# Kamino666/S2VT-video-caption

Measured on AMD Instinct MI355X. Metric: training frames/sec (whole node), higher is better.
Workload: dtype f32; 1 GPU; BASELINE configs[1]: S2VT train step, B=64 per GPU x 1 GPU, 80x4096 feats, hidden=embed=1000, vocab=12000, fp32, Adam; global_batch=64, frames=80, parallelism=dp1

## Files before the change

include/s2vt_hip.h:

```cpp
#ifndef S2VT_HIP_H
#define S2VT_HIP_H

#include <stddef.h>
#include <stdint.h>

#ifdef __cplusplus
extern "C" {
#endif

#define S2VT_ABI_VERSION 9

#define S2VT_ERR_ARG (-1)
#define S2VT_ERR_INDEX (-2)
#define S2VT_ERR_TIMEOUT (-3)

typedef struct s2vt_dims {
    int32_t B, L, F, H, E, V;
} s2vt_dims;

typedef struct s2vt_params {
    const float* vid_w_ih;
    const float* vid_w_hh;
    const float* vid_b_ih;
    const float* vid_b_hh;
// ... 127 lines not shown
                              float* dlogits, void* stream);

#define S2VT_CIDER_MAX_T 512
typedef struct s2vt_cider_table {
    const uint64_t* idf_keys; const double* idf_vals;
    const int32_t* clip_ref_off; const int32_t* ent_off;
    const uint64_t* ent_keys; const double* ent_w;
    const double* ref_norm; const int32_t* ref_len;
    const double* pen;
    double log_n;
    int64_t n_idf;
    int32_t n_clips, n_refs, n_pen;
} s2vt_cider_table;
int s2vt_cider_rewards(const s2vt_cider_table* table, const int32_t* clip_rows, const int64_t* ids, int32_t B, int32_t T, int64_t ld,
                       int32_t sos, int32_t eos, double* out, void* stream);
#define S2VT_CONSENSUS_MAX_K 64
size_t s2vt_cider_consensus_workspace_bytes(int32_t B, int32_t K, int32_t T);
int s2vt_cider_consensus(const s2vt_cider_table* table, const int64_t* ids, int32_t B, int32_t K, int32_t T, int64_t ld,
                         int32_t sos, int32_t eos, const uint8_t* valid, double* utility, int32_t* best,
                         void* workspace, size_t workspace_bytes, void* stream);
typedef struct s2vt_bleu_table {
    const int32_t* clip_key_off; const uint64_t* keys; const int32_t* max_count;
    const int32_t* clip_ref_off; const int32_t* ref_words;
    const double* bp;
    int64_t n_keys;
    int32_t n_clips, n_refs, n_rl;
} s2vt_bleu_table;
int s2vt_mixed_rewards(const s2vt_cider_table* table, const s2vt_bleu_table* bleu, const int32_t* clip_rows, const int64_t* ids,
                       int32_t B, int32_t T, int64_t ld, int32_t sos, int32_t eos, double w_cider, double w_bleu, double* out,
                       double* out_cider, double* out_bleu, void* stream);
size_t s2vt_mixed_consensus_workspace_bytes(int32_t B, int32_t K, int32_t T);
int s2vt_mixed_consensus(const s2vt_cider_table* table, const s2vt_bleu_table* bleu, const int64_t* ids, int32_t B, int32_t K, int32_t T,
                         int64_t ld, int32_t sos, int32_t eos, const uint8_t* valid, double w_cider, double w_bleu, double* utility,
                         int32_t* best, void* workspace, size_t workspace_bytes, void* stream);
int s2vt_sc_weights(const int64_t* sampled, const double* r_sample, const double* r_greedy, int32_t B, int32_t T, int32_t sos,
                    int32_t eos, int64_t* caps, float* weight, void* stream);
int s2vt_sc_weights_group(const int64_t* sampled, const double* r_sample, const double* r_greedy, int32_t B, int32_t K, int32_t T,
                          int32_t sos, int32_t eos, int64_t* caps, float* weight, double* baseline, void* stream);
#define S2VT_SWOR_MAX_K 8
int s2vt_sc_weights_swor(const int64_t* sampled, const float* logprob, const float* kappa, const double* r_sample,
                         const double* r_greedy, int32_t B, int32_t K, int32_t T, int32_t sos, int32_t eos, int64_t* caps,
                         float* weight, double* coef, double* baseline, void* stream);

int s2vt_mean_ce_backward_fused(const s2vt_dims* d, const float* logits, const int64_t* target, int64_t target_ld, const float* lse,
                                const float* gout, void* workspace, size_t workspace_bytes, void* stream);


int s2vt_gemm_f32(int32_t a_kmajor, int32_t b_kmajor, int32_t M, int32_t N, int32_t K, const float* A, int64_t lda,
                  const float* B, int64_t ldb, float* C, int64_t ldc, const float* bias, int32_t accumulate,
                  void* stream);

int s2vt_gemm_f32_splitk(int32_t a_kmajor, int32_t b_kmajor, int32_t M, int32_t N, int32_t K, const float* A,
                         int64_t lda, const float* B, int64_t ldb, float* C, int64_t ldc, const float* bias,
                         int32_t accumulate, float* ws, size_t ws_floats, void* stream);

int s2vt_split_planes(int32_t nplanes, int32_t transpose, const float* in, int64_t ld, int32_t rows, int32_t cols,
                      uint16_t* out, int64_t ldo, int32_t kpad, int32_t out_rows_pad, void* stream);
int s2vt_gemm_bf16_nt(int32_t nplanes, int32_t M, int32_t N, int32_t K, const uint16_t* A, int64_t lda, const uint16_t* B,
                      int64_t ldb, float* C, int64_t ldc, const float* bias, int32_t accumulate, float* ws,
                      size_t ws_floats, void* stream);
int s2vt_gemm_bf16_tt(int32_t nplanes, int32_t M, int32_t N, int32_t K, const uint16_t* A, int64_t lda, const uint16_t* B,
                      int64_t ldb, float* C, int64_t ldc, const float* bias, int32_t accumulate, float* ws, size_t ws_floats,
                      void* stream);

int s2vt_gemm_tune(int32_t nplanes, int32_t tile_rows, int32_t nsplit);

int s2vt_feat_proj_fwd(const s2vt_dims* d, const float* feats, const float* w, const float* bias, float* x1,
                       void* stream);
int s2vt_feat_proj_bwd(const s2vt_dims* d, const float* feats, const float* w, const float* dx1, float* dw,
                       float* dbias, float* dfeats, float* colsum_ws, void* stream);
size_t s2vt_colsum_ws_floats(int64_t rows, int32_t cols);


int s2vt_gemm_f32_mapped(int32_t a_kmajor, int32_t b_kmajor, int32_t M, int32_t N, int32_t K, const float* A, int64_t lda,
                         const int32_t* a_idx, int32_t a_inner, int32_t a_outer, const float* B, int64_t ldb, const int32_t* b_idx,
                         int32_t b_inner, int32_t b_outer, float* C, int64_t ldc, const int32_t* c_idx, int32_t c_inner,
                         int32_t c_outer, const float* bias, int32_t accumulate, float* ws, size_t ws_floats, int32_t splitk_cap,
                         void* stream);
size_t s2vt_embedding_grad_ws_ints(int64_t rows, int32_t V);
int s2vt_embedding_grad(const float* d_rows, int64_t rows, int32_t E, const int32_t* tok, int32_t V, float* d_emb, int32_t* ws,
                        size_t ws_ints, void* stream);
int s2vt_gather_rows(const float* src, int64_t ld, const int32_t* idx, int64_t rows, int32_t cols, float* out, void* stream);
int s2vt_group_sum_rows(const float* in, int64_t ld_in, float* out, int64_t ld_out, int64_t groups, int32_t K, int32_t cols, void* stream);
int s2vt_transpose_f32(const float* in, int32_t rows, int32_t cols, float* out, void* stream);
int s2vt_colsum(const float* x, int64_t rows, int32_t cols, int64_t ld, float* ws, size_t ws_floats, float* out, int32_t accumulate,
                void* stream);
int s2vt_colsum_finish(const float* partial, int32_t nchunks, int32_t cols, float* out, int32_t accumulate, void* stream);
int s2vt_split_planes_dual(int32_t nplanes, const float* in, int64_t ld, const int32_t* idx, int32_t inner, int32_t outer, int32_t rows,
                           int32_t cols, uint16_t* out_r, int64_t ldo_r, int32_t kpad_r, uint16_t* out_t, int64_t ldo_t, int32_t kpad_t,
                           float* colpart, const float* lse, const int64_t* target, int64_t target_ld, int32_t Lm1, const float* gout,
                           float* alpha_out, void* stream);

int s2vt_lstm_step_fwd(int32_t B, int32_t H, const float* gx, const float* bias, const float* w_hh,
                       const float* h_prev, const float* c_prev, float* h_out, float* c_out, float* stash,
                       void* stream);
int s2vt_lstm_step_fwd_token(int32_t B, int32_t H, int32_t E, int32_t V, const float* gx, const float* w_hh, const float* h_prev,
                             const float* c_prev, const float* emb, const float* w_e, int64_t ldw_e, const int32_t* tok,
                             const unsigned long long* tok_packed, int32_t tok_const, float* h_out, float* c_out, void* stream);

int s2vt_lstm_step_fwd_table(int32_t B, int32_t H, int32_t V, const float* gx, const int32_t* gx_idx, const float* bias, const float* gtab,
                             int64_t ldtab, const int32_t* tok, const unsigned long long* tok_packed, int32_t tok_const, const float* w_hh,
                             const float* h_prev, const float* c_prev, float* h_out, float* c_out, float* stash, uint16_t* h_planes,
                             int64_t ldhp, int32_t hp_rows, float* z_out, int64_t ldz, int32_t contract_only, void* stream);
int s2vt_lstm_cell_pointwise(int32_t B, int32_t H, int32_t V, const float* gx, const int32_t* gx_idx, const float* bias, const float* gtab,
                             int64_t ldtab, const int32_t* tok, const unsigned long long* tok_packed, int32_t tok_const, const float* z,
                             int64_t ldz, const float* c_prev, float* h_out, float* c_out, float* stash, uint16_t* h_planes, int64_t ldhp,
                             int32_t hp_rows, void* stream);
int s2vt_argmax_x3_planes(int32_t B, int32_t V, int32_t K, const uint16_t* W, int64_t ldw, int32_t w_rows, const uint16_t* Hp, int64_t ldh,
                          int32_t kpad_h, int32_t hp_rows, const float* bias, unsigned long long* packed, const uint16_t* W2, int64_t ldw2,
                          int32_t kpad_w2, int32_t w2_rows, int32_t M2, float* z, int64_t ldz, int32_t with_logits, int32_t sample,
                          float temperature, uint64_t seed, int32_t step, int32_t row0, void* stream);

int s2vt_lstm_step_bwd(int32_t B, int32_t H, const float* dg_next, const float* w_hh_t, const float* dh_out,
                       const float* stash, const float* c, const float* c_prev, float* dc, int32_t dc_is_zero,
                       float* dg, void* stream);

int s2vt_lstm_seq_fwd(int32_t T, int32_t B, int32_t H, const float* gx, int32_t n_gx, const float* bias,
                      const float* w_hh, float* h_all, float* c_all, float* stash, void* stream);
int s2vt_lstm_seq_bwd(int32_t T, int32_t B, int32_t H, const float* w_hh, const float* dh_out, int32_t dh_first,
                      const float* c_all, float* stash_dg, float* w_hh_t, float* dc, void* stream);

int s2vt_gru_step_fwd(int32_t B, int32_t H, const float* gx, const float* b_ih, const float* w_hh, const float* b_hh,
                      const float* h_prev, float* h_out, float* stash, void* stream);
int s2vt_gru_step_fwd_token(int32_t B, int32_t H, int32_t E, int32_t V, const float* gx, const float* w_hh, const float* b_hh,
                            const float* h_prev, const float* emb, const float* w_e, int64_t ldw_e, const int32_t* tok,
                            const unsigned long long* tok_packed, int32_t tok_const, float* h_out, void* stream);
int s2vt_gru_step_fwd_token_ss(int32_t B, int32_t H, int32_t E, int32_t V, const float* gx, const float* w_hh, const float* b_hh,
                               const float* h_prev, const float* emb, const float* w_e, int64_t ldw_e,
                               const unsigned long long* tok_packed, const int64_t* targets, int64_t targets_ld, float ss_prob,
                               uint64_t seed, int32_t step, int32_t row0, float* h_out, void* stream);
int s2vt_gru_step_bwd(int32_t B, int32_t H, const float* dgh_next, const float* w_hh_t, const float* stash_next, const float* dh_out,
                      const float* stash, const float* h_prev, float* dh, float* dgx, float* dgh, void* stream);
int s2vt_gru_seq_fwd(int32_t T, int32_t B, int32_t H, const float* gx, int32_t n_gx, const float* b_ih, const float* w_hh,
                     const float* b_hh, float* h_all, float* stash, void* stream);
int s2vt_gru_seq_bwd(int32_t T, int32_t B, int32_t H, const float* w_hh, const float* dh_out, int32_t dh_first, const float* h_all,
                     const float* stash, float* w_hh_t, float* dh, float* dgx, float* dgh, void* stream);
int s2vt_tokens_time_major(int32_t B, int32_t Lm1, int32_t V, const int64_t* targets, int64_t targets_ld, int32_t* tok, void* stream);

typedef struct s2vt_lstm_layer {
    const float* w_hh;
    const float* w_in;
    int64_t ldw_in;
    const float* x_in;
    const float* gx;
    int32_t gx_t0, n_gx;
    const float* bias;
    const float* h0; const float* c0;
    const float* mask;
    const float* emb; const float* w_e; int64_t ldw_e; int32_t E, V;
    const unsigned long long* tok_packed; int32_t tok_const;
    float* h; float* c;
    float* stash;
    float* hm;
    const float* dh_ext; int32_t dh_t0;
    float* dg;
    const int64_t* ss_targets; int64_t ss_ld; uint64_t ss_seed; float ss_prob; int32_t ss_step, ss_row0;
} s2vt_lstm_layer;
int s2vt_lstm_chain_fwd(int32_t T, int32_t B, int32_t H, int32_t n, const s2vt_lstm_layer* layers, void* stream);
size_t s2vt_lstm_chain_bwd_workspace_bytes(int32_t B, int32_t H, int32_t n);
int s2vt_lstm_chain_bwd(int32_t T, int32_t B, int32_t H, int32_t n, const s2vt_lstm_layer* layers, void* workspace,
                        size_t workspace_bytes, void* stream);

size_t s2vt_lstm_seq_bf16_workspace_bytes(int32_t T, int32_t B, int32_t H);
int s2vt_lstm_seq_fwd_bf16(int32_t T, int32_t B, int32_t H, float* gx_stash, int32_t n_gx, const float* bias,
                           const float* w_hh, float* h_all, float* c_all, void* workspace, size_t workspace_bytes,
                           int32_t persistent, int32_t block, void* stream);
// ... 174 lines not shown
```

s2vt-video-caption_amd/capi.py:

```python
import ctypes
import os
from ctypes import POINTER, c_char_p, c_double, c_float, c_int32, c_int64, c_size_t, c_uint64, c_void_p

_HERE = os.path.dirname(os.path.abspath(__file__))
LIB_PATH = os.environ.get("S2VT_LIB") or os.path.join(_HERE, "libs2vt_hip.so")


class Dims(ctypes.Structure):
    _fields_ = [(n, c_int32) for n in ("B", "L", "F", "H", "E", "V")]


PARAM_FIELDS = ("vid_w_ih", "vid_w_hh", "vid_b_ih", "vid_b_hh", "word_w_ih", "word_w_hh", "word_b_ih", "word_b_hh",
                "feat_w", "feat_b", "out_w", "out_b", "emb_w")
PARAM_KEYS = ("vid_rnn.weight_ih_l0", "vid_rnn.weight_hh_l0", "vid_rnn.bias_ih_l0", "vid_rnn.bias_hh_l0",
              "word_rnn.weight_ih_l0", "word_rnn.weight_hh_l0", "word_rnn.bias_ih_l0", "word_rnn.bias_hh_l0",
              "feat_linear.weight", "feat_linear.bias", "out_linear.weight", "out_linear.bias", "embedding.weight")


class Params(ctypes.Structure):
    _fields_ = [(n, c_void_p) for n in PARAM_FIELDS]


class Grads(ctypes.Structure):
    _fields_ = [(n, c_void_p) for n in PARAM_FIELDS]
# ... 59 lines not shown
                                      c_void_p, c_size_t, c_void_p]),
    "s2vt_backward_wait_grads": (c_int32, [c_int32, c_void_p]),
    "s2vt_backward_order": (c_int32, [POINTER(c_int32), POINTER(c_int32)]),
    "s2vt_beam_workspace_bytes": (c_size_t, [POINTER(Dims), c_int32]),
    "s2vt_beam_step": (c_int32, [POINTER(Dims), POINTER(Params), c_int32] + [c_void_p] * 14 + [c_size_t, c_void_p]),
    "s2vt_beam_step_cached": (c_int32, [POINTER(Dims), POINTER(Params), c_int32] + [c_void_p] * 14 + [c_size_t, c_void_p, c_size_t,
                                                                                                     c_void_p]),
    "s2vt_decode_workspace_bytes": (c_size_t, [POINTER(Dims)]),
    "s2vt_greedy_decode": (c_int32, [POINTER(Dims), POINTER(Params), c_void_p, c_int32, c_void_p, c_void_p, c_size_t,
                                     c_void_p]),
    "s2vt_decode_cache_bytes": (c_size_t, [POINTER(Dims)]),
    "s2vt_decode_uses_cache": (c_int32, [POINTER(Dims)]),
    "s2vt_greedy_decode_cached": (c_int32, [POINTER(Dims), POINTER(Params), c_void_p, c_int32, c_void_p, c_void_p, c_size_t,
                                            c_void_p, c_size_t, c_int32, c_void_p]),
    "s2vt_adam_step": (c_int32, [c_void_p, c_void_p, c_void_p, c_void_p, c_int64, c_double, c_double, c_double, c_double, c_int64, c_void_p]),
    "s2vt_grad_norm_workspace_bytes": (c_size_t, [c_int64]),
    "s2vt_grad_norm": (c_int32, [c_void_p, c_int64, c_double, c_int32, c_void_p, c_size_t, c_void_p, c_void_p]),
    "s2vt_adam_step_clipped": (c_int32, [c_void_p, c_void_p, c_void_p, c_void_p, c_int64, c_double, c_double, c_double, c_double, c_int64,
                                         c_double, c_int32, POINTER(c_int64), POINTER(c_int32), c_int32, c_int32, c_void_p, c_void_p]),
    "s2vt_mean_ce_forward": (c_int32, [c_int32, c_int32, c_int32, c_void_p, c_void_p, c_int64, c_void_p, c_void_p,
                                       c_void_p, c_void_p]),
    "s2vt_mean_ce_backward": (c_int32, [c_int32, c_int32, c_int32, c_void_p, c_void_p, c_int64, c_void_p, c_void_p,
                                        c_void_p, c_void_p]),
    "s2vt_mask_criterion_forward": (c_int32, [c_int32, c_int32, c_int32, c_void_p, c_void_p, c_int64, c_void_p, c_int64, c_void_p,
                                              c_void_p, c_void_p, c_void_p]),
    "s2vt_mask_criterion_backward": (c_int32, [c_int32, c_int32, c_void_p, c_int64, c_void_p, c_void_p, c_void_p, c_void_p]),
    "s2vt_gemm_f32": (c_int32, [c_int32, c_int32, c_int32, c_int32, c_int32, c_void_p, c_int64, c_void_p, c_int64,
                                c_void_p, c_int64, c_void_p, c_int32, c_void_p]),
    "s2vt_gemm_f32_splitk": (c_int32, [c_int32, c_int32, c_int32, c_int32, c_int32, c_void_p, c_int64, c_void_p, c_int64,
                                       c_void_p, c_int64, c_void_p, c_int32, c_void_p, c_size_t, c_void_p]),
    "s2vt_split_planes": (c_int32, [c_int32, c_int32, c_void_p, c_int64, c_int32, c_int32, c_void_p, c_int64, c_int32,
                                    c_int32, c_void_p]),
    "s2vt_gemm_bf16_nt": (c_int32, [c_int32, c_int32, c_int32, c_int32, c_void_p, c_int64, c_void_p, c_int64, c_void_p,
                                    c_int64, c_void_p, c_int32, c_void_p, c_size_t, c_void_p]),
    "s2vt_gemm_bf16_tt": (c_int32, [c_int32, c_int32, c_int32, c_int32, c_void_p, c_int64, c_void_p, c_int64, c_void_p,
                                    c_int64, c_void_p, c_int32, c_void_p, c_size_t, c_void_p]),
    "s2vt_gemm_tune": (c_int32, [c_int32, c_int32, c_int32]),
    "s2vt_beam_queue_bytes": (c_size_t, [c_int32, c_int32, c_int32]),
    "s2vt_beam_queue_step": (c_int32, [c_int32] * 6 + [c_void_p, c_size_t] + [c_void_p] * 6),
    "s2vt_beam_queue_result": (c_int32, [c_int32, c_int32, c_int32, c_void_p, c_size_t, c_void_p, c_int32, c_void_p, c_void_p]),
    "s2vt_beam_cum_bytes": (c_size_t, [c_int32, c_int32, c_int32]),
    "s2vt_beam_cum_step": (c_int32, [c_int32] * 5 + [c_double, c_int32, c_void_p, c_size_t] + [c_void_p] * 6),
    "s2vt_beam_cum_result": (c_int32, [c_int32] * 5 + [c_void_p, c_size_t] + [c_void_p] * 4),
    "s2vt_beam_cum_hist_bytes": (c_size_t, [c_int32, c_int32, c_int32]),
    "s2vt_beam_cum_hist_step": (c_int32, [c_int32] * 5 + [c_double, c_int32, c_void_p, c_size_t] + [c_void_p] * 5 +
                                [POINTER(c_void_p), POINTER(c_int64), c_void_p]),
    "s2vt_top20_logprob_constrained": (c_int32, [c_void_p, c_int64, c_int64, c_int32, c_void_p, c_int64, c_int32, POINTER(Constraints),
                                                 c_void_p, c_void_p, c_void_p]),
    "s2vt_beam_step_constrained": (c_int32, [POINTER(Dims), POINTER(Params), c_int32] + [c_void_p] * 15 + [c_size_t, c_void_p, c_size_t,
                                                                                                          POINTER(Constraints), c_void_p,
                                                                                                          c_int64, c_int32, c_void_p]),
    "s2vt_ensemble_top20": (c_int32, [c_void_p, c_int64, c_int64, c_int32, c_int64, c_int32, c_void_p, c_void_p, c_void_p, c_void_p]),
    "s2vt_ensemble_top20_constrained": (c_int32, [c_void_p, c_int64, c_int64, c_int32, c_int64, c_int32, c_void_p, c_void_p, c_int64,
                                                  c_int32, POINTER(Constraints), c_void_p, c_void_p, c_void_p]),
    "s2vt_beam_step_logits": (c_int32, [POINTER(Dims), POINTER(Params), c_int32] + [c_void_p] * 13 + [c_int64, c_void_p, c_size_t,
                                                                                                     c_void_p, c_size_t, c_void_p]),
    "s2vt_beam_div_bytes": (c_size_t, [c_int32] * 5),
    "s2vt_beam_div_step": (c_int32, [c_int32] * 6 + [c_double, c_double, c_int32, c_void_p, c_size_t] + [c_void_p] * 5 +
                           [POINTER(c_void_p), POINTER(c_int64), c_void_p]),
    "s2vt_beam_div_result": (c_int32, [c_int32] * 6 + [c_void_p, c_size_t] + [c_void_p] * 4),
    "s2vt_top20_gumbel": (c_int32, [c_void_p, c_int64, c_int64, c_int32, c_float, c_uint64, c_int32, c_int32, c_void_p, c_void_p, c_void_p,
                                    c_void_p]),
    "s2vt_beam_step_gumbel": (c_int32, [POINTER(Dims), POINTER(Params), c_int32] + [c_void_p] * 16 + [c_size_t, c_void_p, c_size_t, c_float,
                                                                                                     c_uint64, c_int32, c_void_p]),
    "s2vt_sbs_bytes": (c_size_t, [c_int32, c_int32, c_int32]),
    "s2vt_sbs_step": (c_int32, [c_int32] * 6 + [c_void_p, c_size_t] + [c_void_p] * 7),
    "s2vt_sbs_result": (c_int32, [c_int32] * 4 + [c_void_p, c_size_t] + [c_void_p] * 6),
    "s2vt_score_workspace_bytes": (c_size_t, [POINTER(Dims), c_int32, c_int32]),
    "s2vt_score_captions": (c_int32, [POINTER(Dims), POINTER(Params), c_void_p, c_void_p, c_int64, c_int64, c_int32, c_int32, c_int32,
                                      c_double, c_void_p, c_void_p, c_void_p, c_void_p, c_size_t, c_void_p, c_size_t, c_int32,
                                      c_void_p]),
    "s2vt_pick_logprob": (c_int32, [c_void_p, c_int64, c_int64, c_int32, c_void_p, c_void_p, c_void_p, c_void_p]),
    "s2vt_feat_proj_fwd": (c_int32, [POINTER(Dims), c_void_p, c_void_p, c_void_p, c_void_p, c_void_p]),
    "s2vt_feat_proj_bwd": (c_int32, [POINTER(Dims), c_void_p, c_void_p, c_void_p, c_void_p, c_void_p, c_void_p,
                                     c_void_p, c_void_p]),
    "s2vt_colsum_ws_floats": (c_size_t, [c_int64, c_int32]),
    "s2vt_gemm_f32_mapped": (c_int32, [c_int32] * 5 + [c_void_p, c_int64, c_void_p, c_int32, c_int32] * 3 +
                             [c_void_p, c_int32, c_void_p, c_size_t, c_int32, c_void_p]),
    "s2vt_embedding_grad_ws_ints": (c_size_t, [c_int64, c_int32]),
    "s2vt_embedding_grad": (c_int32, [c_void_p, c_int64, c_int32, c_void_p, c_int32, c_void_p, c_void_p, c_size_t, c_void_p]),
    "s2vt_gather_rows": (c_int32, [c_void_p, c_int64, c_void_p, c_int64, c_int32, c_void_p, c_void_p]),
    "s2vt_group_sum_rows": (c_int32, [c_void_p, c_int64, c_void_p, c_int64, c_int64, c_int32, c_int32, c_void_p]),
    "s2vt_transpose_f32": (c_int32, [c_void_p, c_int32, c_int32, c_void_p, c_void_p]),
    "s2vt_colsum": (c_int32, [c_void_p, c_int64, c_int32, c_int64, c_void_p, c_size_t, c_void_p, c_int32, c_void_p]),
    "s2vt_colsum_finish": (c_int32, [c_void_p, c_int32, c_int32, c_void_p, c_int32, c_void_p]),
    "s2vt_split_planes_dual": (c_int32, [c_int32, c_void_p, c_int64, c_void_p, c_int32, c_int32, c_int32, c_int32,
                                         c_void_p, c_int64, c_int32, c_void_p, c_int64, c_int32, c_void_p, c_void_p, c_void_p,
                                         c_int64, c_int32, c_void_p, c_void_p, c_void_p]),
    "s2vt_lstm_step_fwd": (c_int32, [c_int32, c_int32] + [c_void_p] * 9),
    "s2vt_lstm_step_fwd_token": (c_int32, [c_int32, c_int32, c_int32, c_int32] + [c_void_p] * 6 + [c_int64, c_void_p, c_void_p,
                                                                                            c_int32, c_void_p, c_void_p, c_void_p]),
    "s2vt_lstm_step_fwd_table": (c_int32, [c_int32] * 3 + [c_void_p] * 4 + [c_int64, c_void_p, c_void_p, c_int32] + [c_void_p] * 7 +
                                 [c_int64, c_int32, c_void_p, c_int64, c_int32, c_void_p]),
    "s2vt_lstm_cell_pointwise": (c_int32, [c_int32] * 3 + [c_void_p] * 4 + [c_int64, c_void_p, c_void_p, c_int32, c_void_p, c_int64] +
                                 [c_void_p] * 5 + [c_int64, c_int32, c_void_p]),
    "s2vt_argmax_x3_planes": (c_int32, [c_int32] * 3 + [c_void_p, c_int64, c_int32, c_void_p, c_int64, c_int32, c_int32, c_void_p, c_void_p,
                                                        c_void_p, c_int64, c_int32, c_int32, c_int32, c_void_p, c_int64, c_int32, c_int32,
                                                        c_float, c_uint64, c_int32, c_int32, c_void_p]),
    "s2vt_lstm_step_bwd": (c_int32, [c_int32, c_int32] + [c_void_p] * 7 + [c_int32, c_void_p, c_void_p]),
    "s2vt_lstm_seq_fwd": (c_int32, [c_int32, c_int32, c_int32, c_void_p, c_int32] + [c_void_p] * 6),
    "s2vt_lstm_seq_bwd": (c_int32, [c_int32, c_int32, c_int32, c_void_p, c_void_p, c_int32] + [c_void_p] * 5),
    "s2vt_gru_step_fwd": (c_int32, [c_int32, c_int32] + [c_void_p] * 8),
    "s2vt_gru_step_fwd_token": (c_int32, [c_int32, c_int32, c_int32, c_int32] + [c_void_p] * 6 + [c_int64, c_void_p, c_void_p,
                                                                                           c_int32, c_void_p, c_void_p]),
    "s2vt_gru_step_bwd": (c_int32, [c_int32, c_int32] + [c_void_p] * 10),
    "s2vt_lstm_chain_fwd": (c_int32, [c_int32, c_int32, c_int32, c_int32, POINTER(LstmLayer), c_void_p]),
    "s2vt_lstm_chain_bwd_workspace_bytes": (c_size_t, [c_int32, c_int32, c_int32]),
    "s2vt_lstm_chain_bwd": (c_int32, [c_int32, c_int32, c_int32, c_int32, POINTER(LstmLayer), c_void_p, c_size_t, c_void_p]),
    "s2vt_gru_seq_fwd": (c_int32, [c_int32, c_int32, c_int32, c_void_p, c_int32] + [c_void_p] * 6),
    "s2vt_gru_seq_bwd": (c_int32, [c_int32, c_int32, c_int32, c_void_p, c_void_p, c_int32] + [c_void_p] * 7),
    "s2vt_tokens_time_major": (c_int32, [c_int32, c_int32, c_int32, c_void_p, c_int64, c_void_p, c_void_p]),
    "s2vt_lstm_seq_bf16_workspace_bytes": (c_size_t, [c_int32, c_int32, c_int32]),
    "s2vt_lstm_seq_fwd_bf16": (c_int32, [c_int32, c_int32, c_int32, c_void_p, c_int32, c_void_p, c_void_p, c_void_p,
                                         c_void_p, c_void_p, c_size_t, c_int32, c_int32, c_void_p]),
    "s2vt_lstm_seq_fwd_bf16_pair": (c_int32, [c_int32, c_int32, c_int32, c_void_p, c_void_p, c_int32] + [c_void_p] * 9 +
                                    [c_size_t, c_int32, c_void_p]),
    "s2vt_lstm_seq_bwd_bf16_workspace_bytes": (c_size_t, [c_int32, c_int32, c_int32]),
    "s2vt_lstm_seq_bwd_bf16": (c_int32, [c_int32, c_int32, c_int32, c_void_p, c_void_p, c_int32, c_void_p, c_void_p, c_void_p,
                                         c_size_t, c_int32, c_int32, c_void_p]),
    "s2vt_lstm_seq_bwd_bf16_pair": (c_int32, [c_int32, c_int32, c_int32, c_void_p, c_void_p, c_void_p, c_void_p, c_int32,
                                              c_void_p, c_void_p, c_void_p, c_void_p, c_void_p, c_size_t, c_int32, c_void_p]),
    "s2vt_lstm_seq_bf16_layout": (c_int32, [c_int32, c_int32, c_int32, c_int32, c_void_p]),
    "s2vt_lstm_seq_x3_workspace_bytes": (c_size_t, [c_int32, c_int32, c_int32]),
    "s2vt_lstm_seq_fwd_x3_persist": (c_int32, [c_int32, c_int32, c_int32, c_void_p, c_void_p, c_int32] + [c_void_p] * 8 +
                                  [c_int32, c_void_p, c_size_t, c_void_p]),
    "s2vt_lstm_seq_bwd_x3_workspace_bytes": (c_size_t, [c_int32, c_int32, c_int32, c_int32]),
    "s2vt_lstm_seq_bwd_x3_persist": (c_int32, [c_int32, c_int32, c_int32, c_void_p, c_void_p, c_void_p, c_void_p, c_int32] +
                                     [c_void_p] * 4 + [c_int32, c_void_p, c_size_t, c_void_p]),
    "s2vt_lstm_seq_fwd_x3_persist_emit": (c_int32, [c_int32, c_int32, c_int32, c_void_p, c_void_p, c_int32] + [c_void_p] * 8 +
                                          [c_void_p, c_int64, c_void_p, c_int64, c_int32, c_int32, c_void_p, c_size_t, c_void_p]),
    "s2vt_lstm_seq_bwd_x3_persist_emit": (c_int32, [c_int32, c_int32, c_int32, c_void_p, c_void_p, c_void_p, c_void_p, c_int32] +
                                          [c_void_p] * 4 + [c_void_p, c_int64, c_void_p, c_int64, c_void_p, c_void_p, c_int32, c_int32,
                                                            c_void_p, c_size_t, c_void_p]),
    "s2vt_set_recurrence_mode": (c_int32, [c_int32]),
    "s2vt_recurrence_plan": (c_int32, [c_int32, c_int32, POINTER(c_int32), POINTER(c_int32)]),
    "s2vt_decode_plan": (c_int32, [POINTER(Dims), c_int32, POINTER(c_int32), POINTER(c_int32), POINTER(c_int32)]),
    "s2vt_decode_step_argmax": (c_int32, [c_int32, c_int32, c_int32] + [c_void_p] * 5),
    "s2vt_decode_step_argmax_x3_workspace_bytes": (c_size_t, [c_int32, c_int32, c_int32]),
    "s2vt_decode_step_argmax_x3": (c_int32, [c_int32, c_int32, c_int32] + [c_void_p] * 5 + [c_size_t, c_void_p]),
    "s2vt_decode_step_sample": (c_int32, [c_int32, c_int32, c_int32, c_void_p, c_void_p, c_void_p, c_float, c_uint64, c_int32, c_int32,
                                          c_void_p, c_void_p]),
    "s2vt_decode_step_sample_x3_workspace_bytes": (c_size_t, [c_int32, c_int32, c_int32]),
    "s2vt_decode_step_sample_x3": (c_int32, [c_int32, c_int32, c_int32, c_void_p, c_void_p, c_void_p, c_float, c_uint64, c_int32,
                                             c_int32, c_void_p, c_void_p, c_size_t, c_void_p]),
    "s2vt_sample_decode": (c_int32, [POINTER(Dims), POINTER(Params), c_void_p, c_int32, c_float, c_uint64, c_void_p, c_void_p,
                                     c_size_t, c_void_p]),
    "s2vt_sample_decode_cached": (c_int32, [POINTER(Dims), POINTER(Params), c_void_p, c_int32, c_float, c_uint64, c_void_p, c_void_p,
                                            c_size_t, c_void_p, c_size_t, c_int32, c_void_p]),
    "s2vt_sample_rows_workspace_bytes": (c_size_t, [POINTER(Dims), c_int32]),
    "s2vt_sample_decode_rows": (c_int32, [POINTER(Dims), POINTER(Params), c_void_p, c_int32, c_int32, c_float, c_uint64, c_void_p,
                                          c_void_p, c_size_t, c_void_p, c_size_t, c_int32, c_void_p]),
    "s2vt_truncated_draw": (c_int32, [c_void_p, c_int64, c_int64, c_int32, c_float, c_int32, c_float, c_uint64, c_int32, c_int32, c_void_p,
                                      c_void_p, c_void_p]),
    "s2vt_top20_logprob": (c_int32, [c_void_p, c_int64, c_int64, c_int32, c_void_p, c_void_p, c_void_p]),
    "s2vt_sample_rows_trunc_workspace_bytes": (c_size_t, [POINTER(Dims), c_int32]),
    "s2vt_sample_decode_rows_trunc": (c_int32, [POINTER(Dims), POINTER(Params), c_void_p, c_int32, c_int32, c_float, c_uint64, c_int32,
                                                c_float, c_void_p, c_void_p, c_size_t, c_void_p, c_size_t, c_int32, c_void_p]),
    "s2vt_constrained_draw": (c_int32, [c_void_p, c_int64, c_int64, c_int32, c_void_p, c_int64, c_int32, POINTER(Constraints), c_int32, c_float,
                                        c_int32, c_float, c_uint64, c_int32, c_int32, c_void_p, c_void_p, c_void_p]),
    "s2vt_decode_rows_constrained_workspace_bytes": (c_size_t, [POINTER(Dims), c_int32]),
    "s2vt_decode_rows_constrained": (c_int32, [POINTER(Dims), POINTER(Params), c_void_p, c_int32, c_int32, c_int32, c_float, c_uint64, c_int32,
                                               c_float, POINTER(Constraints), c_void_p, c_void_p, c_size_t, c_void_p, c_size_t, c_int32,
                                               c_void_p]),
    "s2vt_scheduled_decode": (c_int32, [POINTER(Dims), POINTER(Params), c_void_p, c_void_p, c_int64, c_float, c_int32, c_float, c_uint64,
                                        c_void_p, c_void_p, c_void_p, c_size_t, c_void_p]),
    "s2vt_scheduled_decode_cached": (c_int32, [POINTER(Dims), POINTER(Params), c_void_p, c_void_p, c_int64, c_float, c_int32, c_float,
# ... 119 lines not shown
```

s2vt-video-caption_amd/csrc/api_internal.h:

```cpp
#pragma once
#include <stdarg.h>
#include <stdlib.h>
#include <string.h>

#include <algorithm>
#include <functional>
#include <map>
#include <mutex>
#include <vector>

#include "../../include/s2vt_hip.h"
#include "common.h"
#include "kernels.h"

namespace s2vt {

#ifdef S2VT_EXPERIMENT_STAMPS
extern unsigned long long* g_xstamps;
extern int g_xstamp_block;
#endif
const char* last_error_text();

int poll_async_error(bool wait);
int post_async_error(hipStream_t st, const int* dev_flags, int kind = 0);
// ... 63 lines not shown
    const int m = option(O_PERSIST_X3_BWD);
    if (m == 0 || !persist_on()) return false;
    return m == 1 || lstm_seq_bwd_x3_persist_supported(B, H) == 1;
}
enum RecKind { REC_PER_STEP = 0, REC_BF16_PERSIST = 1, REC_X3_PERSIST = 3 };
struct RecurrencePlan { RecKind fwd, bwd; };
static inline RecurrencePlan train_recurrence_plan(int B, int H) {
    RecurrencePlan pl = {REC_PER_STEP, REC_PER_STEP};
    const int gm = gemm_mode();
    if (pipe_block() <= 0 || gm == 0 || B % 64 != 0) return pl;
    if (gm == 1) {
        if (persist_on() && lstm_seq_fwd_bf16_persist_supported(B, H, pad64(H))) pl.fwd = REC_BF16_PERSIST;
        if (persist_on() && lstm_seq_bwd_bf16_persist_supported(B, H, pad64(4 * H))) pl.bwd = REC_BF16_PERSIST;
    } else if (H <= 1024) {
        if (persist_x3_fwd_on() && lstm_seq_fwd_x3_persist_supported(B, H)) pl.fwd = REC_X3_PERSIST;
        if (persist_x3_bwd_on(B, H) && lstm_seq_bwd_x3_persist_supported(B, H)) pl.bwd = REC_X3_PERSIST;
    }
    return pl;
}
enum DecSchedule { DEC_PER_STEP = 0, DEC_TWO_CHAINS = 1, DEC_FUSED = 2 };
struct DecodePlan { bool padded; int B; bool planes, persist_encode; DecSchedule schedule; int nh; };
static inline DecodePlan decode_plan(const s2vt_dims& d, bool encode_only, bool device = true) {
    DecodePlan pl;
    pl.padded = encode_only ? (gemm_mode() != 0 && d.B % 64 != 0) : batch_pads(d.B, true);
    pl.B = pl.padded ? padded_dims(d).B : d.B;
    pl.planes = gemm_mode() != 0 && pl.B % 64 == 0;
    pl.persist_encode = pl.planes && d.H <= 1024 && pipe_block() > 0 && persist_x3_fwd_on() &&
                        (!device || lstm_seq_fwd_x3_persist_supported(pl.B, d.H));
    pl.schedule = !pl.persist_encode ? DEC_PER_STEP : option(O_DECODE_FUSED) == 1 ? DEC_FUSED : DEC_TWO_CHAINS;
    pl.nh = (pl.persist_encode && pl.B % 128 == 0) ? 2 : 1;
    return pl;
}
static inline int persist_bits() { return persist_mode() | (persist_x3_fwd_on() ? 2 : 0) | (option(O_PERSIST_X3_BWD) << 2); }

struct Lane {
    hipStream_t s;
    float* gws;
    size_t gws_floats;
    float* colsum;
};
int side_stream(hipStream_t caller, hipStream_t* out);
int side_stream_overlaps();
int get_event(size_t i, hipEvent_t* out);
int handoff(hipStream_t from, hipStream_t to, size_t ev_index);
int lgemm(const Lane& ln, bool ak, bool bk, int M, int N, int K, const float* A, int64_t lda, RowMap am, const float* B, int64_t ldb,
          RowMap bm, float* C, int64_t ldc, RowMap cm, const float* bias, bool acc);
struct Lanes {
    hipStream_t st = nullptr, sx = nullptr;
    Lane la{}, lb{};
    size_t ev = 0;
    int open(hipStream_t caller, float* gws_a, float* gws_b, size_t gws_floats, float* colsum_a, float* colsum_b);
    int hand(hipStream_t from, hipStream_t to) { return handoff(from, to, ev++); }
    int record(hipStream_t s, long* idx);
    int wait(hipStream_t s, long idx);
};

int seq_fwd(hipStream_t st, int t0, int t1, int B, int H, float* gx_stash, int n_gx, const float* bias, const float* w_hh, float* h_all,
            float* c_all, bool write_stash);
int seq_bwd(hipStream_t st, int T, int t0, int t1, int B, int H, const float* w_hh_t, const float* dh_out, int dh_first,
            const float* c_all, float* stash_dg, float* dc);
int balanced_block(int L, int blk);
std::vector<int> pipe_bounds(int T, int L, int blk);

struct PB { unsigned short* p = nullptr; int64_t ld = 0; int kpad = 0; int planes = 0; };
static constexpr size_t K16_HALF_ELEMS = 64 * 8;
static constexpr size_t K16_REC_ELEMS = 3 * 2 * K16_HALF_ELEMS;
static inline int64_t koff(const PB& b, int k0) { return b.planes == 3 ? (int64_t)k0 * 192 : (int64_t)k0 * b.planes; }
static inline size_t rows64(size_t r) { return (r + 63) / 64 * 64; }
static inline PB take_planes(Carver& c, size_t rows, size_t k, int planes) {
    const int kpad = pad64((int)k);
    return PB{c.take<unsigned short>(rows64(rows) * (size_t)planes * kpad), (int64_t)planes * kpad, kpad, planes};
}
int zero_k16_tail(hipStream_t st, const PB& img, int H, size_t rows);
int psplit(const Lane& ln, const PB& dst, int r0, const float* in, int64_t ld, RowMap imap, int rows, int cols);
int pdual(const Lane& ln, const float* in, int64_t ld, RowMap imap, int rows, int cols, const PB* r, int r0, const PB* t, int k0,
          float* colpart);
int pcolpart(const Lane& ln, int planes, const float* in, int64_t ld, RowMap imap, int rows, int cols, float* colpart);
int pgemm(const Lane& ln, int M, int N, int K, const PB& A, int a0, int ka, const PB& B, int b0, int kb, float* C, int64_t ldc,
          RowMap cm, const float* bias, bool acc);
int pgemm_tt(const Lane& ln, int M, int N, int K, const PB& A, int a_row0, const PB& B, int b_row0, float* C, int64_t ldc, RowMap cm,
             const float* bias, bool acc);
int lcolsum_finish(const Lane& ln, const float* partial, int nchunks, int cols, float* out, bool accumulate);
int bias_sums(hipStream_t st, const s2vt_params* p, int H, float* bsum1, float* bsum2);
int project_features_f32(const Lane& ln, const s2vt_dims& d, const s2vt_params* p, const float* feats, float* x1, float* gx1, const float* bsum1);
extern int g_lane_delay_lanes;
extern long long g_lane_delay_us;
struct LaneDelayScope {
    explicit LaneDelayScope(hipStream_t caller);
    ~LaneDelayScope();
};
int lane_delay(hipStream_t s);

int seq_fwd_bf16(hipStream_t st, int t0, int t1, int B, int H, float* gx_stash, int n_gx, const float* bias, const PB& wb, const PB& hb,
                 float* h_all, float* c_all);
int seq_bwd_bf16(hipStream_t st, int T, int t0, int t1, int B, int H, const PB& wt, const float* dh_out, int dh_first,
                 const float* c_all, float* stash_dg, const PB& dgb, float* dc);
SeqBwdX3Args persist_bwd_x3_args(int T, int t0, int t1, int B, int H, int64_t Kp, int64_t Hp, const unsigned short* wtp,
                                 const float* dh_out, int dh_first, const float* c_all, float* stash_dg, float* dc, float* part,
                                 int64_t part_slot, int nslots, unsigned int* sync, int* err);
SeqFwdX3Args persist_fwd_x3_args(int t0, int t1, int B, int H, int T, int64_t Kp, float* gx_stash, int n_gx, const float* bias,
                                 const unsigned short* wp, unsigned short* hp, float* h_all, float* c_all, unsigned int* sync, int* err);
bool persist_fwd_ok(int B, int H, const PB& wb, const PB& hb);
SeqFwdBf16Args persist_fwd_args(int t0, int t1, int B, int H, float* gx_stash, int n_gx, const float* bias, const PB& wb, const PB& hb,
                                float* h_all, float* c_all, unsigned int* sync, int* err);
SeqBwdBf16Args seq_bwd_bf16_args(int T, int t0, int t1, int B, int H, const PB& wt, const PB& dgb, const float* dh_out, int dh_first,
                                 const float* c_all, float* stash_dg, float* dc, unsigned int* sync, int* err);

int grads_ready(int group, hipStream_t s);
void backward_order_reset();
struct BackwardScope {
    BackwardScope() { backward_order_reset(); cu_reserve_window(false); }
    ~BackwardScope() { cu_reserve_window(false); }
};

template <typename Rec> class RecordTable {
    struct Slot { Rec rec; unsigned long long seq; };
    std::map<const void*, Slot> slots;
    std::mutex mutex;
    unsigned long long seq = 0;
public:
    void put(const void* ws, const Rec& rec) {
        std::lock_guard<std::mutex> lock(mutex);
        if (slots.size() >= 64 && !slots.count(ws)) {
            auto oldest = slots.begin();
            for (auto it = slots.begin(); it != slots.end(); ++it)
                if (it->second.seq < oldest->second.seq) oldest = it;
            slots.erase(oldest);
        }
        slots[ws] = Slot{rec, ++seq};
    }
    bool take(const void* ws, Rec* out) {
        std::lock_guard<std::mutex> lock(mutex);
        auto it = slots.find(ws);
        if (it == slots.end()) return false;
        *out = it->second.rec;
        slots.erase(it);
        return true;
    }
    template <typename F> bool with(const void* ws, F f) {
        std::lock_guard<std::mutex> lock(mutex);
        auto it = slots.find(ws);
        return it != slots.end() && f(it->second.rec);
    }
};

struct TrainBufs {
    float *bsum1, *bsum2, *x1, *s1, *h1, *c1, *s2, *h2, *c2;
    float *wt1, *wt2, *dh1, *dh2dec, *dx1, *de, *dc1, *dc2, *colsum_a, *colsum_b, *gws_a, *gws_b;
    size_t gws_floats;
    int32_t* tok;
    int* embws;
    int* err;
};

int train_forward_f32(const s2vt_dims* d, const s2vt_params* p, const float* feats, const int64_t* targets, int64_t targets_ld,
                      float* logits, const TrainBufs& w, hipStream_t st, const float* out_mask);
int train_backward_f32(const s2vt_dims* d, const s2vt_params* p, const float* feats, const float* dlogits, const s2vt_grads* g,
                       float* dfeats, const TrainBufs& w, hipStream_t st, const float* out_mask);

static inline bool temperature_ok(float t) { const float r = 1.0f / t; return t > 0.f && r > 0.f && r <= 3.4028234e38f; }
static inline GumbelArgs gumbel_args(float temperature, uint64_t seed, uint32_t step, uint32_t row0, uint32_t rows) {
    return GumbelArgs{1.0f / temperature, (uint32_t)(seed & 0xFFFFFFFFull), (uint32_t)(seed >> 32), step, row0, rows};
}

struct DecodeConst { PB wf, wih1, wv, wo; float* gtab; unsigned short *xw1, *xw2; PB whh; size_t bytes; };
DecodeConst carve_decode_const(const s2vt_dims& d, void* base);
// ... 18 lines not shown
```

s2vt-video-caption_amd/csrc/api_ops.hip:

```cpp
#include "api_internal.h"

using namespace s2vt;

extern "C" {

int s2vt_adam_step(float* params, const float* grads, float* exp_avg, float* exp_avg_sq, int64_t n, double lr, double beta1, double beta2,
                   double eps, int64_t step, void* stream) {
    return adam_flat((hipStream_t)stream, params, grads, exp_avg, exp_avg_sq, n, lr, beta1, beta2, eps, step);
}

size_t s2vt_grad_norm_workspace_bytes(int64_t n) { return grad_norm_workspace_bytes(n); }
int s2vt_grad_norm(const float* grads, int64_t n, double max_norm, int32_t skip_nonfinite, void* workspace, size_t workspace_bytes,
                   void* record, void* stream) {
    static_assert(sizeof(ClipRecord) == sizeof(s2vt_clip_record) && GN_CHUNK == S2VT_GRAD_NORM_CHUNK && ADAM_MAX_SEGS == S2VT_ADAM_MAX_SEGMENTS,
                  "kernels.h and s2vt_hip.h state the same record and constants");
    return grad_norm((hipStream_t)stream, grads, n, max_norm, skip_nonfinite, workspace, workspace_bytes, static_cast<ClipRecord*>(record));
}
int s2vt_adam_step_clipped(float* params, const float* grads, float* exp_avg, float* exp_avg_sq, int64_t n, double lr, double beta1,
                           double beta2, double eps, int64_t step, double weight_decay, int32_t decoupled, const int64_t* seg_end,
                           const int32_t* seg_decay, int32_t n_seg, int32_t skip_nonfinite, const void* record, void* stream) {
    return adam_flat_clipped((hipStream_t)stream, params, grads, exp_avg, exp_avg_sq, n, lr, beta1, beta2, eps, step, weight_decay, decoupled,
                             seg_end, seg_decay, n_seg, skip_nonfinite, static_cast<const ClipRecord*>(record));
}

// ... 74 lines not shown
                         int64_t lda, const float* B, int64_t ldb, float* C, int64_t ldc, const float* bias,
                         int32_t accumulate, float* ws, size_t ws_floats, void* stream) {
    GemmWsScope gscope(ws, ws_floats);
    return gemm((hipStream_t)stream, a_kmajor != 0, b_kmajor != 0, M, N, K, A, lda, ID, B, ldb, ID, C, ldc, ID, bias,
                accumulate != 0);
}

int s2vt_split_planes(int32_t nplanes, int32_t transpose, const float* in, int64_t ld, int32_t rows, int32_t cols,
                      uint16_t* out, int64_t ldo, int32_t kpad, int32_t out_rows_pad, void* stream) {
    return split_planes((hipStream_t)stream, nplanes, transpose != 0, in, ld, ID, rows, cols, out, ldo, kpad, out_rows_pad);
}

int s2vt_gemm_bf16_nt(int32_t nplanes, int32_t M, int32_t N, int32_t K, const uint16_t* A, int64_t lda, const uint16_t* B,
                      int64_t ldb, float* C, int64_t ldc, const float* bias, int32_t accumulate, float* ws,
                      size_t ws_floats, void* stream) {
    ProfScope ps((hipStream_t)stream, K_GEMM, 1);
    return gemm_bf16_nt((hipStream_t)stream, nplanes, M, N, K, A, lda, B, ldb, C, ldc, ID, bias, accumulate != 0, ws,
                        ws_floats);
}

int s2vt_gemm_bf16_tt(int32_t nplanes, int32_t M, int32_t N, int32_t K, const uint16_t* A, int64_t lda, const uint16_t* B,
                      int64_t ldb, float* C, int64_t ldc, const float* bias, int32_t accumulate, float* ws, size_t ws_floats,
                      void* stream) {
    S2VT_REQUIRE(nplanes == 3 || nplanes == 1, "s2vt_gemm_bf16_tt: planes must be 1 or 3");
    ProfScope ps((hipStream_t)stream, K_GEMM, 1);
    if (nplanes == 1) return gemm_b1_tt((hipStream_t)stream, M, N, K, A, lda, B, ldb, C, ldc, ID, bias, accumulate != 0, ws, ws_floats);
    return gemm_x3_tt((hipStream_t)stream, M, N, K, A, lda, B, ldb, C, ldc, ID, bias, accumulate != 0, ws, ws_floats);
}

int s2vt_feat_proj_fwd(const s2vt_dims* d, const float* feats, const float* w, const float* bias, float* x1,
                       void* stream) {
    S2VT_REQUIRE(dims_ok(d) && feats && w && x1, "s2vt_feat_proj_fwd: null/invalid argument");
    return gemm((hipStream_t)stream, true, true, d->B * d->L, d->H, d->F, feats, d->F, ID, w, d->F, ID, x1, d->H,
                perm(d->L, d->B), bias, false);
}

size_t s2vt_colsum_ws_floats(int64_t rows, int32_t cols) { return colsum_partial_floats(rows, cols); }

static bool rowmap_ok(const int32_t* idx, int32_t inner, int32_t outer, int64_t mapped_rows) {
    if (inner < 0 || outer < 0) return false;
    if (inner == 0) return outer == 0;
    return idx == nullptr && (int64_t)inner * outer == mapped_rows;
}
static RowMap rowmap(const int32_t* idx, int32_t inner, int32_t outer) { return RowMap{idx, inner, outer}; }

int s2vt_gemm_f32_mapped(int32_t a_kmajor, int32_t b_kmajor, int32_t M, int32_t N, int32_t K, const float* A, int64_t lda,
                         const int32_t* a_idx, int32_t a_inner, int32_t a_outer, const float* B, int64_t ldb, const int32_t* b_idx,
                         int32_t b_inner, int32_t b_outer, float* C, int64_t ldc, const int32_t* c_idx, int32_t c_inner,
                         int32_t c_outer, const float* bias, int32_t accumulate, float* ws, size_t ws_floats, int32_t splitk_cap,
                         void* stream) {
    S2VT_REQUIRE(M > 0 && N > 0 && K > 0 && A && B && C, "s2vt_gemm_f32_mapped: null operand or non-positive size (M=%d N=%d K=%d)", M, N, K);
    S2VT_REQUIRE(lda >= (a_kmajor ? K : M) && ldb >= (b_kmajor ? K : N) && ldc >= N,
                 "s2vt_gemm_f32_mapped: a row stride is shorter than the row it strides over");
    S2VT_REQUIRE(rowmap_ok(a_idx, a_inner, a_outer, a_kmajor ? M : K) && rowmap_ok(b_idx, b_inner, b_outer, b_kmajor ? N : K) &&
                     rowmap_ok(c_idx, c_inner, c_outer, M),
                 "s2vt_gemm_f32_mapped: bad row map (an index and a permutation together, or inner * outer != the mapped rows)");
    S2VT_REQUIRE(splitk_cap >= 0 && (ws != nullptr || ws_floats == 0), "s2vt_gemm_f32_mapped: bad split-K scratch or cap");
    size_t planned = ws ? ws_floats : 0;
    if (splitk_cap > 0 && (size_t)splitk_cap * M * N < planned) planned = (size_t)splitk_cap * M * N;
    ProfScope ps((hipStream_t)stream, K_GEMM, 1);
    return gemm_f32((hipStream_t)stream, a_kmajor != 0, b_kmajor != 0, M, N, K, A, lda, rowmap(a_idx, a_inner, a_outer), B, ldb,
                    rowmap(b_idx, b_inner, b_outer), C, ldc, rowmap(c_idx, c_inner, c_outer), bias, accumulate != 0, ws, planned);
}

size_t s2vt_embedding_grad_ws_ints(int64_t rows, int32_t V) {
    if (rows < 0 || V <= 0) return 0;
    return embedding_grad_ws_ints(rows, V);
}
int s2vt_embedding_grad(const float* d_rows, int64_t rows, int32_t E, const int32_t* tok, int32_t V, float* d_emb, int32_t* ws,
                        size_t ws_ints, void* stream) {
    S2VT_REQUIRE(rows >= 0 && rows <= 0x7fffffff && E > 0 && V > 0 && d_emb && ws && (rows == 0 || (d_rows && tok)),
                 "s2vt_embedding_grad: null argument or bad size (rows=%lld E=%d V=%d)", (long long)rows, E, V);
    S2VT_REQUIRE(ws_ints >= embedding_grad_ws_ints(rows, V), "s2vt_embedding_grad: scratch %zu < %zu ints", ws_ints,
                 embedding_grad_ws_ints(rows, V));
    return embedding_grad((hipStream_t)stream, d_rows, rows, E, tok, V, d_emb, ws);
}

int s2vt_gather_rows(const float* src, int64_t ld, const int32_t* idx, int64_t rows, int32_t cols, float* out, void* stream) {
    S2VT_REQUIRE(src && idx && out && rows > 0 && rows <= 65535 && cols > 0 && ld >= cols,
                 "s2vt_gather_rows: null argument or bad geometry (rows=%lld cols=%d ld=%lld)", (long long)rows, cols, (long long)ld);
    return gather_rows_f32((hipStream_t)stream, src, ld, idx, rows, cols, out);
}

int s2vt_transpose_f32(const float* in, int32_t rows, int32_t cols, float* out, void* stream) {
    S2VT_REQUIRE(in && out && in != out && rows > 0 && cols > 0 && (rows + 63) / 64 <= 65535,
                 "s2vt_transpose_f32: null argument or bad geometry (rows=%d cols=%d)", rows, cols);
    return transpose_f32((hipStream_t)stream, in, rows, cols, out);
}

int s2vt_colsum(const float* x, int64_t rows, int32_t cols, int64_t ld, float* ws, size_t ws_floats, float* out, int32_t accumulate,
                void* stream) {
    S2VT_REQUIRE(x && ws && out && rows > 0 && rows <= 64 * (int64_t)65535 && cols > 0 && ld >= cols,
                 "s2vt_colsum: null argument or bad geometry (rows=%lld cols=%d ld=%lld)", (long long)rows, cols, (long long)ld);
    S2VT_REQUIRE(ws_floats >= colsum_partial_floats(rows, cols), "s2vt_colsum: scratch %zu < %zu floats", ws_floats,
                 colsum_partial_floats(rows, cols));
    return colsum_f32((hipStream_t)stream, x, rows, cols, ld, ws, out, accumulate != 0);
}
int s2vt_colsum_finish(const float* partial, int32_t nchunks, int32_t cols, float* out, int32_t accumulate, void* stream) {
    S2VT_REQUIRE(partial && out && nchunks > 0 && cols > 0, "s2vt_colsum_finish: null argument or bad geometry (nchunks=%d cols=%d)",
                 nchunks, cols);
    return colsum_finish((hipStream_t)stream, partial, nchunks, cols, out, accumulate != 0);
}

int s2vt_split_planes_dual(int32_t nplanes, const float* in, int64_t ld, const int32_t* idx, int32_t inner, int32_t outer, int32_t rows,
                           int32_t cols, uint16_t* out_r, int64_t ldo_r, int32_t kpad_r, uint16_t* out_t, int64_t ldo_t, int32_t kpad_t,
                           float* colpart, const float* lse, const int64_t* target, int64_t target_ld, int32_t Lm1, const float* gout,
                           float* alpha_out, void* stream) {
    S2VT_REQUIRE((nplanes == 1 || nplanes == 3) && in && rows > 0 && cols > 0 && ld >= cols && (out_r || out_t || colpart),
                 "s2vt_split_planes_dual: null input, no output, or bad size (planes=%d rows=%d cols=%d)", nplanes, rows, cols);
    S2VT_REQUIRE(rowmap_ok(idx, inner, outer, rows), "s2vt_split_planes_dual: bad row map");
    auto image_ok = [&](const uint16_t* p, int64_t ldo, int kpad, int k) {
        return !p || (kpad % 64 == 0 && kpad >= k && kpad <= 64 * cdiv(k, 64) && ldo % 8 == 0 && ldo >= (int64_t)nplanes * kpad &&
                      (reinterpret_cast<uintptr_t>(p) & 15) == 0);
    };
    S2VT_REQUIRE(image_ok(out_r, ldo_r, kpad_r, cols) && image_ok(out_t, ldo_t, kpad_t, rows),
                 "s2vt_split_planes_dual: bad plane geometry (kpad = the k extent rounded up to 64, ldo >= planes * kpad, 16-byte aligned)");
    const bool with_ce = lse || target || gout || alpha_out;
    if (!with_ce) return split_planes_dual((hipStream_t)stream, nplanes, in, ld, rowmap(idx, inner, outer), rows, cols, out_r, ldo_r,
                                            kpad_r, out_t, ldo_t, kpad_t, colpart, nullptr);
    S2VT_REQUIRE(lse && target && gout && Lm1 > 0 && rows % Lm1 == 0 && target_ld >= Lm1 + 1 && !idx && inner == 0,
                 "s2vt_split_planes_dual: bad CE-gradient arguments (lse, target and gout together, rows = B * Lm1, no row map)");
    const CeGradArgs ce = {lse, target, gout, Lm1, target_ld, alpha_out};
    return split_planes_dual((hipStream_t)stream, nplanes, in, ld, ID, rows, cols, out_r, ldo_r, kpad_r, out_t, ldo_t, kpad_t, colpart, &ce);
}

int s2vt_feat_proj_bwd(const s2vt_dims* d, const float* feats, const float* w, const float* dx1, float* dw,
                       float* dbias, float* dfeats, float* colsum_ws, void* stream) {
    S2VT_REQUIRE(dims_ok(d) && feats && w && dx1 && dw && dbias && colsum_ws, "s2vt_feat_proj_bwd: null/invalid argument");
    hipStream_t st = (hipStream_t)stream;
    int rc;
    if ((rc = gemm(st, false, false, d->H, d->F, d->L * d->B, dx1, d->H, ID, feats, d->F, perm(d->B, d->L), dw, d->F, ID,
                   nullptr, false)))
        return rc;
    if ((rc = colsum_f32(st, dx1, (int64_t)d->L * d->B, d->H, d->H, colsum_ws, dbias, false))) return rc;
    if (dfeats)
        return gemm(st, true, false, d->L * d->B, d->F, d->H, dx1, d->H, ID, w, d->F, ID, dfeats, d->F, perm(d->B, d->L),
                    nullptr, false);
    return 0;
}

int s2vt_lstm_step_fwd(int32_t B, int32_t H, const float* gx, const float* bias, const float* w_hh,
                       const float* h_prev, const float* c_prev, float* h_out, float* c_out, float* stash,
                       void* stream) {
    StepFwdArgs a;
    memset(&a, 0, sizeof(a));
    a.B = B; a.H = H;
    a.h_prev = h_prev; a.ldh = H; a.w_hh = w_hh; a.ldw = H;
    a.gx = gx; a.ldgx = 4 * (int64_t)H; a.bias = bias;
    a.c_prev = c_prev; a.ldc = H;
    a.h_out = h_out; a.ldho = H; a.c_out = c_out; a.ldco = H;
    a.stash = stash; a.ldst = 4 * (int64_t)H;
    ProfScope ps((hipStream_t)stream, K_STEP_FWD, 1);
    return lstm_step_fwd((hipStream_t)stream, a);
}

int s2vt_lstm_step_fwd_token(int32_t B, int32_t H, int32_t E, int32_t V, const float* gx, const float* w_hh, const float* h_prev,
                             const float* c_prev, const float* emb, const float* w_e, int64_t ldw_e, const int32_t* tok,
                             const unsigned long long* tok_packed, int32_t tok_const, float* h_out, float* c_out, void* stream) {
    S2VT_REQUIRE(B > 0 && H > 0 && E > 0 && V > 0 && gx && w_hh && emb && w_e && h_out && c_out && ldw_e >= E,
                 "s2vt_lstm_step_fwd_token: null/invalid argument");
    hipStream_t st = (hipStream_t)stream;
    PostedFlags flags;
    int rc;
    if ((rc = flags.open(st))) return rc;
    StepFwdArgs a;
    memset(&a, 0, sizeof(a));
// ... 509 lines not shown
```

s2vt-video-caption_amd/csrc/api_shared.hip:

```cpp
#include "api_internal.h"

namespace s2vt {

int seq_fwd(hipStream_t st, int t0, int t1, int B, int H, float* gx_stash, int n_gx, const float* bias,
                   const float* w_hh, float* h_all, float* c_all, bool write_stash) {
    if (t1 <= t0) return 0;
    ProfScope ps(st, K_STEP_FWD, t1 - t0);
    const int64_t BH = (int64_t)B * H, B4H = 4 * BH;
    for (int t = t0; t < t1; ++t) {
        StepFwdArgs a;
        memset(&a, 0, sizeof(a));
        a.B = B; a.H = H;
        a.h_prev = t ? h_all + (t - 1) * BH : nullptr; a.ldh = H;
        a.w_hh = w_hh; a.ldw = H;
        a.gx = (t < n_gx) ? gx_stash + t * B4H : nullptr; a.ldgx = 4 * (int64_t)H;
        a.bias = bias;
        a.c_prev = t ? c_all + (t - 1) * BH : nullptr; a.ldc = H;
        a.h_out = h_all + t * BH; a.ldho = H;
        a.c_out = c_all + t * BH; a.ldco = H;
        a.stash = write_stash ? gx_stash + t * B4H : nullptr; a.ldst = 4 * (int64_t)H;
        int rc = lstm_step_fwd(st, a);
        if (rc) return rc;
    }
    return 0;
// ... 47 lines not shown
}
int Lanes::record(hipStream_t s, long* idx) {
    hipEvent_t e;
    *idx = (long)ev++;
    if (const int r = get_event((size_t)*idx, &e)) return r;
    S2VT_HIP(hipEventRecord(e, s));
    return 0;
}
int Lanes::wait(hipStream_t s, long idx) {
    hipEvent_t e;
    if (const int r = get_event((size_t)idx, &e)) return r;
    S2VT_HIP(hipStreamWaitEvent(s, e, 0));
    return 0;
}

int bias_sums(hipStream_t st, const s2vt_params* p, int H, float* bsum1, float* bsum2) {
    if (const int rc = add_vectors(st, p->vid_b_ih, p->vid_b_hh, bsum1, 4 * H)) return rc;
    return add_vectors(st, p->word_b_ih, p->word_b_hh, bsum2, 4 * H);
}
int project_features_f32(const Lane& ln, const s2vt_dims& d, const s2vt_params* p, const float* feats, float* x1, float* gx1, const float* bsum1) {
    const int B = d.B, L = d.L, F = d.F, H = d.H;
    if (const int rc = lgemm(ln, true, true, B * L, H, F, feats, F, ID, p->feat_w, F, ID, x1, H, perm(L, B), p->feat_b, false)) return rc;
    return lgemm(ln, true, true, L * B, 4 * H, H, x1, H, ID, p->vid_w_ih, H, ID, gx1, 4 * H, ID, bsum1, false);
}
int zero_k16_tail(hipStream_t st, const PB& img, int H, size_t rows) {
    const size_t kc0 = (size_t)cdiv(H, 16), kc1 = (size_t)(img.kpad / 16);
    if (kc1 <= kc0) return 0;
    S2VT_HIP(hipMemset2DAsync(img.p + kc0 * K16_REC_ELEMS, (size_t)64 * img.ld * 2, 0, (kc1 - kc0) * K16_REC_ELEMS * 2, rows / 64, st));
    return 0;
}

int g_lane_delay_lanes = 0;
long long g_lane_delay_us = 0;
static thread_local hipStream_t t_delay_caller = nullptr;
static thread_local bool t_delay_active = false;
LaneDelayScope::LaneDelayScope(hipStream_t caller) { t_delay_caller = caller; t_delay_active = true; }
LaneDelayScope::~LaneDelayScope() { t_delay_active = false; t_delay_caller = nullptr; }
int lane_delay(hipStream_t s) {
    if (g_lane_delay_us <= 0 || !t_delay_active) return 0;
    if (!(g_lane_delay_lanes & (s == t_delay_caller ? 1 : 2))) return 0;
    return occupy_cus(s, 1, 0, g_lane_delay_us);
}

int psplit(const Lane& ln, const PB& dst, int r0, const float* in, int64_t ld, RowMap imap, int rows, int cols) {
    if (int rc = lane_delay(ln.s)) return rc;
    return split_planes(ln.s, dst.planes, false, in, ld, imap, rows, cols, dst.p + (int64_t)r0 * dst.ld, dst.ld, dst.kpad, rows);
}
int pdual(const Lane& ln, const float* in, int64_t ld, RowMap imap, int rows, int cols, const PB* r, int r0,
                 const PB* t, int k0, float* colpart) {
    if (!r && !t && !colpart) return 0;
    S2VT_REQUIRE(r || t, "pdual: column sums alone name no plane count (pcolpart)");
    S2VT_REQUIRE(!r || !t || r->planes == t->planes, "pdual: row image of %d planes, transposed image of %d", r->planes, t->planes);
    if (int rc = lane_delay(ln.s)) return rc;
    return split_planes_dual(ln.s, (r ? r : t)->planes, in, ld, imap, rows, cols, r ? r->p + (int64_t)r0 * r->ld : nullptr, r ? r->ld : 0,
                             r ? r->kpad : 0, t ? t->p + koff(*t, k0) : nullptr, t ? t->ld : 0, t ? pad64(rows) : 0, colpart);
}
int pcolpart(const Lane& ln, int planes, const float* in, int64_t ld, RowMap imap, int rows, int cols, float* colpart) {
    if (int rc = lane_delay(ln.s)) return rc;
    return split_planes_dual(ln.s, planes, in, ld, imap, rows, cols, nullptr, 0, 0, nullptr, 0, 0, colpart);
}
int pgemm(const Lane& ln, int M, int N, int K, const PB& A, int a0, int ka, const PB& B, int b0, int kb, float* C,
                 int64_t ldc, RowMap cm, const float* bias, bool acc) {
    S2VT_REQUIRE(A.planes == B.planes, "pgemm: A of %d planes, B of %d", A.planes, B.planes);
    if (int rc = lane_delay(ln.s)) return rc;
    ProfScope ps(ln.s, cu_plan_cap_current() ? K_GEMM_CORUN : K_GEMM, 1);
    return gemm_bf16_nt(ln.s, A.planes, M, N, pad64(K), A.p + (int64_t)a0 * A.ld + koff(A, ka), A.ld,
                        B.p + (int64_t)b0 * B.ld + koff(B, kb), B.ld, C, ldc, cm, bias, acc, ln.gws, ln.gws_floats);
}

int pgemm_tt(const Lane& ln, int M, int N, int K, const PB& A, int a_row0, const PB& B, int b_row0, float* C, int64_t ldc,
                    RowMap cm, const float* bias, bool acc) {
    S2VT_REQUIRE(A.planes == B.planes, "pgemm_tt: A of %d planes, B of %d", A.planes, B.planes);
    if (int rc = lane_delay(ln.s)) return rc;
    ProfScope ps(ln.s, cu_plan_cap_current() ? K_GEMM_CORUN : K_GEMM, 1);
    if (A.planes == 1)
        return gemm_b1_tt(ln.s, M, N, K, A.p + (int64_t)a_row0 * A.ld, A.ld, B.p + (int64_t)b_row0 * B.ld, B.ld, C, ldc, cm, bias, acc,
                          ln.gws, ln.gws_floats);
    return gemm_x3_tt(ln.s, M, N, K, A.p + (int64_t)a_row0 * A.ld, A.ld, B.p + (int64_t)b_row0 * B.ld, B.ld, C, ldc, cm, bias, acc,
                      ln.gws, ln.gws_floats);
}
int lcolsum_finish(const Lane& ln, const float* partial, int nchunks, int cols, float* out, bool accumulate) {
    if (int rc = lane_delay(ln.s)) return rc;
    return colsum_finish(ln.s, partial, nchunks, cols, out, accumulate);
}

int seq_fwd_bf16(hipStream_t st, int t0, int t1, int B, int H, float* gx_stash, int n_gx, const float* bias,
                        const PB& wb, const PB& hb, float* h_all, float* c_all) {
    if (t1 <= t0) return 0;
    ProfScope ps(st, K_STEP_FWD, t1 - t0);
    const int64_t BH = (int64_t)B * H, B4H = 4 * BH;
    for (int t = t0; t < t1; ++t) {
        StepFwdBf16Args a;
        memset(&a, 0, sizeof(a));
        a.B = B; a.H = H; a.Kp = hb.kpad;
        a.hb_prev = t ? hb.p + (int64_t)(t - 1) * B * hb.ld : nullptr; a.ldhb = hb.ld;
        a.wb = wb.p; a.ldwb = wb.ld;
        a.gx = (t < n_gx) ? gx_stash + t * B4H : nullptr; a.ldgx = 4 * (int64_t)H;
        a.bias = bias;
        a.c_prev = t ? c_all + (t - 1) * BH : nullptr; a.ldc = H;
        a.h_out = h_all + t * BH; a.ldho = H;
        a.hb_out = hb.p + (int64_t)t * B * hb.ld; a.ldhbo = hb.ld;
        a.c_out = c_all + t * BH; a.ldco = H;
        a.stash = gx_stash + t * B4H; a.ldst = 4 * (int64_t)H;
        int rc = lstm_step_fwd_bf16(st, a);
        if (rc) return rc;
    }
    return 0;
}
int seq_bwd_bf16(hipStream_t st, int T, int t0, int t1, int B, int H, const PB& wt, const float* dh_out,
                        int dh_first, const float* c_all, float* stash_dg, const PB& dgb, float* dc) {
    if (t1 <= t0) return 0;
    ProfScope ps(st, K_STEP_BWD, t1 - t0);
    const int64_t BH = (int64_t)B * H, B4H = 4 * BH;
    for (int t = t1 - 1; t >= t0; --t) {
        StepBwdBf16Args a;
        memset(&a, 0, sizeof(a));
        a.B = B; a.H = H; a.Kp = dgb.kpad;
        a.dgb_next = (t < T - 1) ? dgb.p + (int64_t)(t + 1) * B * dgb.ld : nullptr; a.lddgb = dgb.ld;
        a.wtb = wt.p; a.ldwtb = wt.ld;
        a.dh_out = (dh_out && t >= dh_first) ? dh_out + (int64_t)(t - dh_first) * BH : nullptr; a.lddho = H;
        a.stash = stash_dg + t * B4H; a.ldst = 4 * (int64_t)H;
        a.c = c_all + t * BH; a.ldc = H;
        a.c_prev = t ? c_all + (t - 1) * BH : nullptr; a.ldcp = H;
        a.dc = dc; a.lddc = H;
        a.dc_is_zero = (t == T - 1) ? 1 : 0;
        a.dg = stash_dg + t * B4H; a.lddg = 4 * (int64_t)H;
        a.dgb = dgb.p + (int64_t)t * B * dgb.ld; a.lddgbo = dgb.ld;
        int rc = lstm_step_bwd_bf16(st, a);
        if (rc) return rc;
    }
    return 0;
}

SeqBwdX3Args persist_bwd_x3_args(int T, int t0, int t1, int B, int H, int64_t Kp, int64_t Hp, const unsigned short* wtp,
                                        const float* dh_out, int dh_first, const float* c_all, float* stash_dg, float* dc,
                                        float* part, int64_t part_slot, int nslots, unsigned int* sync, int* err) {
    SeqBwdX3Args a;
    memset(&a, 0, sizeof(a));
    a.B = B; a.H = H; a.Kp = (int)Kp; a.Hp = (int)Hp; a.T = T; a.t0 = t0; a.t1 = t1;
    a.wtp = wtp; a.wplane = Kp * 4 * Hp; a.ldw = 4 * Hp;
    a.dh_out = dh_out; a.dh_first = dh_first;
    a.stash_dg = stash_dg; a.c_all = c_all; a.dc = dc;
    a.part = part; a.part_slot = part_slot; a.nslots = nslots;
    a.sync = sync; a.err = err;
#ifdef S2VT_EXPERIMENT_STAMPS
    a.stamps = g_xstamps; a.stamp_block = g_xstamp_block;
#endif
    return a;
}
SeqFwdX3Args persist_fwd_x3_args(int t0, int t1, int B, int H, int T, int64_t Kp, float* gx_stash, int n_gx, const float* bias,
                                        const unsigned short* wp, unsigned short* hp, float* h_all, float* c_all,
                                        unsigned int* sync, int* err) {
    SeqFwdX3Args a;
    memset(&a, 0, sizeof(a));
    a.B = B; a.H = H; a.Kp = (int)Kp; a.t0 = t0; a.t1 = t1; a.n_gx = n_gx;
    a.wp = wp; a.wplane = 4 * (int64_t)H * Kp; a.ldw = Kp;
    a.hp = hp; a.hplane = (int64_t)T * B * Kp; a.ldh = Kp;
    a.h_all = h_all; a.gx_stash = gx_stash; a.bias = bias; a.c_all = c_all;
    a.sync = sync; a.err = err;
#ifdef S2VT_EXPERIMENT_STAMPS
    a.stamps = g_xstamps; a.stamp_block = g_xstamp_block;
#endif
    return a;
}
bool persist_fwd_ok(int B, int H, const PB& wb, const PB& hb) {
    return persist_on() && lstm_seq_fwd_bf16_persist_supported(B, H, hb.kpad) && hb.kpad == wb.kpad;
// ... 33 lines not shown
```

s2vt-video-caption_amd/csrc/api_train.hip:

```cpp
#include "api_internal.h"

namespace s2vt {

struct TrainWS : TrainBufs {
    float* colsum_c;
    float* ce_alpha;
    unsigned int *psync_a, *psync_b;
    unsigned short *xw1, *xw2, *xh1, *xh2;
    int64_t xkp;
    bool xfwd;
    unsigned short *xwt1, *xwt2;
    float *xpart1, *xpart2;
    int xnslots; int64_t xpslot, xhp;
    size_t bytes;
};

static TrainWS carve_train(const s2vt_dims& d, void* base) {
    const size_t B = d.B, L = d.L, H = d.H, E = d.E, V = d.V, T = 2 * L - 1;
    Carver c{reinterpret_cast<char*>(base), 0, 0};
    TrainWS w;
    w.bsum1 = c.take<float>(4 * H);
    w.bsum2 = c.take<float>(4 * H);
    w.x1 = c.take<float>(L * B * H);
    w.s1 = c.take<float>(T * B * 4 * H);
// ... 56 lines not shown
    if (group == 0) {
        g_bwd_group0_after = g_bwd_persist_launches;
        cu_reserve_window(true);
    }
    if (!g_grad_ev[group]) S2VT_HIP(hipEventCreateWithFlags(&g_grad_ev[group], hipEventDisableTiming));
    if (!graph_capturing()) S2VT_HIP(hipEventRecord(g_grad_ev[group], s));
    g_grad_ev_set[group] = true;
    return 0;
}

struct PlaneWS {
    PB feats, wf, x1, wih1, h1, we, wv, emb, h2r, wo, whh1, whh2;
    PB dlog, woT, wvT, weT, wih1T, dg2, dg1, whh1T, whh2T;
    PB h2decB;
    size_t bytes;
};

static PlaneWS carve_planes(const s2vt_dims& d, int planes, void* base) {
    const size_t B = d.B, L = d.L, F = d.F, H = d.H, E = d.E, V = d.V, T = 2 * L - 1, R = (L - 1) * B;
    Carver c{reinterpret_cast<char*>(base), 0, 0};
    auto mk = [&](size_t rows, size_t k) { return take_planes(c, rows, k, planes); };
    PlaneWS w;
    w.feats = mk(B * L, F);   w.wf = mk(H, F);       w.x1 = mk(L * B, H);    w.wih1 = mk(4 * H, H);
    w.h1 = mk(T * B, H);      w.we = mk(4 * H, E);   w.wv = mk(4 * H, H);    w.emb = mk(R, E);
    w.h2r = mk(T * B, H);     w.wo = mk(V, H);
    if (planes == 1) {
        w.whh1 = mk(4 * H, H); w.whh2 = mk(4 * H, H); w.whh1T = mk(H, 4 * H); w.whh2T = mk(H, 4 * H);
    }
    w.dlog = mk(R, V);        w.woT = mk(H, V);
    w.wvT = mk(H, 4 * H);     w.weT = mk(E, 4 * H);  w.wih1T = mk(H, 4 * H);
    w.dg2 = mk(T * B, 4 * H); w.dg1 = mk(T * B, 4 * H);
    w.h2decB = mk(R, H);
    w.bytes = align_up(c.off, 256);
    return w;
}

struct FwdRecord { s2vt_dims d; int gemm_mode, planes, persist, blk; bool dlog_ready; };
static RecordTable<FwdRecord> g_fwd_records;
static void record_forward(const void* ws, const s2vt_dims& d, bool planes) {
    g_fwd_records.put(ws, FwdRecord{d, gemm_mode(), planes ? train_planes() : 0, persist_bits(), pipe_block(), false});
}
static int check_forward_record(const void* ws, const s2vt_dims& d, bool planes, bool* dlog_ready = nullptr) {
    FwdRecord r;
    S2VT_REQUIRE(g_fwd_records.take(ws, &r), "s2vt_train_backward: no s2vt_train_forward has run on this workspace");
    if (dlog_ready) *dlog_ready = r.dlog_ready;
    S2VT_REQUIRE(memcmp(&r.d, &d, sizeof(d)) == 0, "s2vt_train_backward: dims differ from the forward that filled this workspace");
    S2VT_REQUIRE(r.gemm_mode == gemm_mode() && r.planes == (planes ? train_planes() : 0) && r.persist == persist_bits() && r.blk == pipe_block(),
                 "s2vt_train_backward: the forward ran with gemm mode %d / recurrence options %d / pipeline block %d, now %d / %d / %d: the "
                 "workspace layout differs (do not change gemm_mode / persist / persist_x3_fwd / persist_x3_bwd / pipe_block "
                 "between a forward and its backward)", r.gemm_mode, r.persist, r.blk, gemm_mode(), persist_bits(), pipe_block());
    return 0;
}

static void key_options(std::vector<uint64_t>& key) {
    for (int i = 0; i < O_COUNT; ++i) key.push_back((uint64_t)(uint32_t)option(i));
    key.push_back((uint64_t)(uint32_t)cu_plan_cap_current());
    key.push_back((uint64_t)g_lane_delay_lanes);
    key.push_back((uint64_t)g_lane_delay_us);
}

struct BpttDone {
    int bias_chunk = 64;
    int hh1_t0 = 0;
    long word_grads_ev = -1;
    long demb_ev = -1;
};

struct TrainDriver : Lanes {
    const s2vt_params* p; const s2vt_grads* g; const TrainWS& w; const PlaneWS& q;
    const float* out_mask; float* logits;
    const int B, L, F, H, E, V, T, R, blk;
    const int64_t BH, B4H;
    const bool bf;
    const bool emit;
    std::vector<int> bd;
    TrainDriver(const s2vt_dims* d, const s2vt_params* p_, const s2vt_grads* g_, const TrainWS& w_, const PlaneWS& q_,
                const float* out_mask_, float* logits_)
        : p(p_), g(g_), w(w_), q(q_), out_mask(out_mask_), logits(logits_), B(d->B), L(d->L), F(d->F), H(d->H), E(d->E), V(d->V),
          T(2 * d->L - 1), R((d->L - 1) * d->B), blk(pipe_block()), BH((int64_t)d->B * d->H), B4H(4 * (int64_t)d->B * d->H),
          bf(q_.h1.planes == 1), emit(d->H % 8 == 0) {}
    int open_lanes(hipStream_t caller) { return open(caller, w.gws_a, w.gws_b, w.gws_floats, w.colsum_a, w.colsum_b); }
    void set_bounds(bool persistent) { bd = pipe_bounds(T, L, persistent ? balanced_block(L, blk) : blk); }

    int zero_k16(const PB& img, size_t first, size_t elems) {
        S2VT_HIP(hipMemset2DAsync(img.p + first, (size_t)64 * img.ld * 2, 0, elems * 2, (size_t)(T * B / 64), st));
        return 0;
    }
    int vid_half_gemm(const Lane& ln, int t0, int t1) {
        const bool cap = t0 >= L;
        return pgemm(ln, (t1 - t0) * B, 4 * H, H, q.h1, t0 * B, 0, q.wv, 0, 0, w.s2 + t0 * B4H, 4 * H, ID, cap ? nullptr : w.bsum2, cap);
    }
    int logits_gemm(const Lane& ln, int first_step) {
        const PB* a = &q.h2r;
        int a0 = L * B, rc;
        if (out_mask) {
            if ((rc = mul_vectors(ln.s, w.h2 + (int64_t)L * B * H, out_mask, w.dh2dec, (int64_t)R * H))) return rc;
            a = &q.h2decB; a0 = 0;
            if ((rc = psplit(ln, *a, a0, w.dh2dec, H, ID, R, H))) return rc;
        }
        return pgemm(ln, R - first_step * B, V, H, *a, a0 + first_step * B, 0, q.wo, 0, 0, logits + (int64_t)first_step * V, V, perm(B, L - 1),
                     p->out_b, false);
    }
    int fwd_x3_persistent(int f_cus, int tenths, int gxe_c);
    int fwd_bf16_persistent();
    int fwd_two_lanes();

    int split_dg_block(const Lane& ln, int layer, int t0, int t1, bool want_planes) {
        const PB& dg = layer == 2 ? q.dg2 : q.dg1;
        const float* in = (layer == 2 ? w.s2 : w.s1) + t0 * B4H;
        float* colpart = (layer == 2 ? w.colsum_a : w.colsum_b) + (int64_t)(t0 * B / 64) * 4 * H;
        return want_planes ? pdual(ln, in, 4 * H, ID, (t1 - t0) * B, 4 * H, &dg, t0 * B, nullptr, t0 * B, colpart)
                           : pcolpart(ln, dg.planes, in, 4 * H, ID, (t1 - t0) * B, 4 * H, colpart);
    }
    int dh1_gemm(const Lane& ln, int t0, int t1) {
        return pgemm(ln, (t1 - t0) * B, H, 4 * H, q.dg2, t0 * B, 0, q.wvT, 0, 0, w.dh1 + t0 * BH, H, ID, nullptr, false);
    }
    int word_weight_grads(const Lane& ln) {
        int rc;
        if ((rc = pgemm_tt(ln, 4 * H, H, (T - 1) * B, q.dg2, B, q.h2r, 0, g->word_w_hh, H, ID, nullptr, false))) return rc;
        if ((rc = pgemm_tt(ln, 4 * H, H, T * B, q.dg2, 0, q.h1, 0, g->word_w_ih + E, E + H, ID, nullptr, false))) return rc;
        return pgemm_tt(ln, 4 * H, E, R, q.dg2, L * B, q.emb, 0, g->word_w_ih, E + H, ID, nullptr, false);
    }
    int demb_gemm(const Lane& ln) { return pgemm(ln, R, E, 4 * H, q.dg2, L * B, 0, q.weT, 0, 0, w.de, E, ID, nullptr, false); }
    SeqBwdX3Args bwd_x3_args(int layer, int t0, int t1) {
        const bool word = layer == 2;
        SeqBwdX3Args a = word ? persist_bwd_x3_args(T, t0, t1, B, H, w.xkp, w.xhp, w.xwt2, w.dh2dec, L, w.c2, w.s2, w.dc2, w.xpart2, w.xpslot,
                                                    w.xnslots, w.psync_a, w.err + 1)
                              : persist_bwd_x3_args(T, t0, t1, B, H, w.xkp, w.xhp, w.xwt1, w.dh1, 0, w.c1, w.s1, w.dc1, w.xpart1, w.xpslot,
                                                    w.xnslots, w.psync_b, w.err + 1);
        if (emit) {
            a.dgp = word ? q.dg2.p : q.dg1.p; a.lddgp = word ? q.dg2.ld : q.dg1.ld;
            a.colpart = word ? w.colsum_a : w.colsum_b; a.skip_dg = 1;
        }
        return a;
    }
    int x3_bptt_begin();
    int bptt_x3_one_layer(int corun_cus, int corun_k, BpttDone* done);
    int bptt_x3_two_layer(int corun_cus, int corun_k, BpttDone* done);
    int bptt_bf16_persistent();
    int bptt_two_lanes();
};

int TrainDriver::fwd_x3_persistent(int f_cus, int tenths, int gxe_c) {
    int rc;
    if ((rc = hand(sx, st))) return rc;
    const int nb = (int)bd.size() - 1;
    for (const PB* img : {&q.h1, &q.h2r})
        if ((rc = zero_k16_tail(st, *img, H, (size_t)T * B))) return rc;
    int lg_c = (nb >= 2 && !out_mask) ? (L - 1) * ((2 * tenths + 1) / 3) / 10 : 0;
    if (lg_c > bd[nb - 1] - L) lg_c = bd[nb - 1] - L > 0 ? bd[nb - 1] - L : 0;
    for (int k = 0; k <= nb; ++k) {
        const bool hv = k < nb, hw = k >= 1;
        const bool co_first = k == 0 && nb >= 2 && gxe_c > 0, co_last = k == nb && lg_c > 0;
        if ((co_first || co_last) && (rc = hand(st, sx))) return rc;
        {
        ProfScope ps(st, K_STEP_FWD, (hv ? bd[k + 1] - bd[k] : 0) + (hw ? bd[k] - bd[k - 1] : 0));
        SeqFwdX3Args av, aw;
        if (hv) av = persist_fwd_x3_args(bd[k], bd[k + 1], B, H, T, w.xkp, w.s1, L, w.bsum1, w.xw1, w.xh1, w.h1, w.c1, w.psync_a, w.err + 1);
        if (hw) aw = persist_fwd_x3_args(bd[k - 1], bd[k], B, H, T, w.xkp, w.s2, T, w.bsum2, w.xw2, w.xh2, w.h2, w.c2, w.psync_b, w.err + 1);
        av.hblk = q.h1.p; av.ldhblk = q.h1.ld;
        aw.hblk = q.h2r.p; aw.ldhblk = q.h2r.ld;
        if (hv && hw) rc = lstm_seq_fwd_x3_persist2(st, av, &aw);
        else rc = lstm_seq_fwd_x3_persist2(st, hv ? av : aw, nullptr);
        }
        if (rc) return rc;
        if (co_first || co_last) {
            {
                CuPlanCap cap(f_cus);
                if (co_first)
                    rc = pgemm(lb, gxe_c, 4 * H, E, q.emb, R - gxe_c, 0, q.we, 0, 0, w.s2 + (int64_t)L * B4H + (int64_t)(R - gxe_c) * 4 * H, 4 * H,
                               ID, w.bsum2, false);
                else
                    rc = pgemm(lb, lg_c * B, V, H, q.h2r, L * B, 0, q.wo, 0, 0, logits, V, perm(B, L - 1), p->out_b, false);
            }
            if (rc || (rc = hand(sx, st))) return rc;
        }
        if (hv && (rc = vid_half_gemm(la, bd[k], bd[k + 1]))) return rc;
    }
    return logits_gemm(la, lg_c);
}

int TrainDriver::fwd_bf16_persistent() {
    int rc;
    if ((rc = hand(sx, st))) return rc;
    const int nb = (int)bd.size() - 1;
    for (int k = 0; k <= nb; ++k) {
        const bool hv = k < nb, hw = k >= 1;
        SeqFwdBf16Args av, aw;
        if (hv) av = persist_fwd_args(bd[k], bd[k + 1], B, H, w.s1, L, w.bsum1, q.whh1, q.h1, w.h1, w.c1, w.psync_a, w.err + 1);
        if (hw) aw = persist_fwd_args(bd[k - 1], bd[k], B, H, w.s2, T, w.bsum2, q.whh2, q.h2r, w.h2, w.c2, w.psync_b, w.err + 1);
        {
            ProfScope ps(st, K_STEP_FWD, (hv ? bd[k + 1] - bd[k] : 0) + (hw ? bd[k] - bd[k - 1] : 0));
            if (hv && hw) rc = lstm_seq_fwd_bf16_persist2(st, av, &aw);
            else rc = lstm_seq_fwd_bf16_persist2(st, hv ? av : aw, nullptr);
            if (rc) return rc;
        }
        if (hv && (rc = vid_half_gemm(la, bd[k], bd[k + 1]))) return rc;
    }
    return logits_gemm(la, 0);
}

int TrainDriver::fwd_two_lanes() {
    int rc;
    for (size_t k = 0; k + 1 < bd.size(); ++k) {
        const int t0 = bd[k], t1 = bd[k + 1];
        rc = bf ? seq_fwd_bf16(st, t0, t1, B, H, w.s1, L, w.bsum1, q.whh1, q.h1, w.h1, w.c1)
                : seq_fwd(st, t0, t1, B, H, w.s1, L, w.bsum1, p->vid_w_hh, w.h1, w.c1, true);
        if (rc) return rc;
        if ((rc = hand(st, sx))) return rc;
        if ((rc = pdual(lb, w.h1 + t0 * BH, H, ID, (t1 - t0) * B, H, bf ? nullptr : &q.h1, t0 * B, nullptr, t0 * B, nullptr))) return rc;
        if ((rc = vid_half_gemm(lb, t0, t1))) return rc;
        rc = bf ? seq_fwd_bf16(sx, t0, t1, B, H, w.s2, T, w.bsum2, q.whh2, q.h2r, w.h2, w.c2)
                : seq_fwd(sx, t0, t1, B, H, w.s2, T, w.bsum2, p->word_w_hh, w.h2, w.c2, true);
        if (rc) return rc;
        if ((rc = pdual(lb, w.h2 + t0 * BH, H, ID, (t1 - t0) * B, H, bf ? nullptr : &q.h2r, t0 * B, nullptr, t0 * B, nullptr))) return rc;
    }
    if ((rc = logits_gemm(lb, 0))) return rc;
    return hand(sx, st);
}

static int train_forward_x3(const s2vt_dims* d, const s2vt_params* p, const float* feats, const int64_t* targets,
                            int64_t targets_ld, float* logits, const TrainWS& w, const PlaneWS& q, hipStream_t st,
                            const float* out_mask) {
    TrainDriver x(d, p, nullptr, w, q, out_mask, logits);
    const int B = x.B, L = x.L, F = x.F, H = x.H, E = x.E, V = x.V, T = x.T, R = x.R;
    const int64_t B4H = x.B4H;
    int rc;
    if ((rc = x.open_lanes(st))) return rc;
    const hipStream_t sx = x.sx;
    const Lane &la = x.la, &lb = x.lb;
    const bool bf = x.bf;
    if ((rc = bias_sums(st, p, H, w.bsum1, w.bsum2))) return rc;
    if ((rc = fill_zero(st, w.err, 4 * sizeof(int)))) return rc;
    if ((rc = targets_to_time_major(st, targets, B, L - 1, targets_ld, V, w.tok, w.err))) return rc;
    if (bf) {
        if ((rc = zero_pad_cols_u16(st, q.h1.p, (int64_t)T * B, q.h1.ld, H, q.h1.kpad))) return rc;
        if ((rc = zero_pad_cols_u16(st, q.h2r.p, (int64_t)T * B, q.h2r.ld, H, q.h2r.kpad))) return rc;
        if ((rc = pdual(la, p->vid_w_hh, H, ID, 4 * H, H, &q.whh1, 0, &q.whh1T, 0, nullptr))) return rc;
    }
    if ((rc = x.hand(st, sx))) return rc;
    if (bf && (rc = pdual(lb, p->word_w_hh, H, ID, 4 * H, H, &q.whh2, 0, &q.whh2T, 0, nullptr))) return rc;
    RecKind kind = train_recurrence_plan(B, H).fwd;
    if (kind == REC_X3_PERSIST && !w.xfwd) kind = REC_PER_STEP;
    if (kind == REC_BF16_PERSIST && !persist_fwd_ok(B, H, q.whh1, q.h1)) kind = REC_PER_STEP;
    const bool px3_fwd = kind == REC_X3_PERSIST;
    if (px3_fwd) {
        if ((rc = split3_rows(sx, p->vid_w_hh, H, 4 * H, H, (int)w.xkp, w.xw1, 4 * (int64_t)H * w.xkp))) return rc;
        if ((rc = split3_rows(sx, p->word_w_hh, H, 4 * H, H, (int)w.xkp, w.xw2, 4 * (int64_t)H * w.xkp))) return rc;
    }
    if ((rc = pdual(lb, p->word_w_ih, E + H, ID, 4 * H, E, &q.we, 0, &q.weT, 0, nullptr))) return rc;
    if ((rc = pdual(lb, p->word_w_ih + E, E + H, ID, 4 * H, H, &q.wv, 0, &q.wvT, 0, nullptr))) return rc;
    if ((rc = pdual(lb, p->out_w, H, ID, V, H, &q.wo, 0, &q.woT, 0, nullptr))) return rc;
    if ((rc = pdual(lb, p->emb_w, E, gather(w.tok), R, E, &q.emb, 0, nullptr, 0, nullptr))) return rc;
    const int f_wgs = px3_fwd ? lstm_seq_fwd_x3_persist_single_workgroups(B, H) : 0;
    const int f_cus = f_wgs > 0 ? (planned_compute_units() - f_wgs - 2) / 8 * 8 : 0;
    const bool stages3 = px3_fwd && pipe_bounds(T, L, balanced_block(L, x.blk)).size() >= 3;
    const int tenths = (stages3 && sx != st && f_cus >= 64 && R >= 2560 && B % 64 == 0) ? option(O_CORUN) : 0;
    const int gxe_c = (R / 64 * (2 * tenths < 8 ? 2 * tenths : 8) / 10) * 64;
    if ((rc = pgemm(lb, R - gxe_c, 4 * H, E, q.emb, 0, 0, q.we, 0, 0, w.s2 + (int64_t)L * B4H, 4 * H, ID, w.bsum2, false))) return rc;
    if ((rc = psplit(la, q.feats, 0, feats, F, ID, B * L, F))) return rc;
    if ((rc = psplit(la, q.wf, 0, p->feat_w, F, ID, H, F))) return rc;
    if ((rc = pdual(la, p->vid_w_ih, H, ID, 4 * H, H, &q.wih1, 0, &q.wih1T, 0, nullptr))) return rc;
    if ((rc = pgemm(la, B * L, H, F, q.feats, 0, 0, q.wf, 0, 0, w.x1, H, perm(L, B), p->feat_b, false))) return rc;
    if ((rc = pdual(la, w.x1, H, ID, L * B, H, &q.x1, 0, nullptr, 0, nullptr))) return rc;
    if ((rc = pgemm(la, L * B, 4 * H, H, q.x1, 0, 0, q.wih1, 0, 0, w.s1, 4 * H, ID, w.bsum1, false))) return rc;
    x.set_bounds(kind != REC_PER_STEP);
    switch (kind) {
    case REC_X3_PERSIST: return x.fwd_x3_persistent(f_cus, tenths, gxe_c);
    case REC_BF16_PERSIST: return x.fwd_bf16_persistent();
    default: return x.fwd_two_lanes();
    }
}

int TrainDriver::x3_bptt_begin() {
    int rc;
    if ((rc = split3_wt(st, w.wt2, H, (int)w.xkp, (int)w.xhp, w.xwt2, w.xkp * 4 * w.xhp))) return rc;
    if ((rc = split3_wt(sx, w.wt1, H, (int)w.xkp, (int)w.xhp, w.xwt1, w.xkp * 4 * w.xhp))) return rc;
    if ((rc = hand(sx, st))) return rc;
    if (emit && q.dg2.kpad > 4 * H) {
        const size_t kc0 = (size_t)(4 * H / 16);
        for (const PB* img : {&q.dg2, &q.dg1}) {
            if ((rc = zero_k16_tail(st, *img, 4 * H, (size_t)T * B))) return rc;
            if (4 * H % 16)
                for (int pl = 0; pl < 3; ++pl)
                    if ((rc = zero_k16(*img, kc0 * K16_REC_ELEMS + (pl * 2 + 1) * K16_HALF_ELEMS, K16_HALF_ELEMS))) return rc;
        }
    }
    return 0;
}

int TrainDriver::bptt_x3_one_layer(int corun_cus, int corun_k, BpttDone* done) {
    int rc;
    const int nb = (int)bd.size() - 1;
    if ((rc = hand(st, sx))) return rc;
    int wo_r = 0;
    auto wo_part = [&]() -> int {
        if (wo_r >= R) return 0;
        int kk = corun_k < R - wo_r ? corun_k : R - wo_r;
        if (R - wo_r - kk < 512) kk = R - wo_r;
        const int r = pgemm_tt(lb, V, H, kk, q.dlog, wo_r, q.h2decB, wo_r, g->out_w, H, ID, nullptr, wo_r > 0);
        wo_r += kk;
        return r;
    };
    std::vector<long> dh1_done((size_t)nb);
    long wo_done = 0;
    {
        CuPlanCap cap(corun_cus);
        for (int k = nb - 1; k >= 0; --k) {
            const int t0 = bd[k], t1 = bd[k + 1];
            {
                ProfScope ps(st, K_STEP_BWD, t1 - t0);
                if ((rc = lstm_seq_bwd_x3_persist2(st, bwd_x3_args(2, t0, t1), nullptr))) return rc;
                ++g_bwd_persist_launches;
            }
            if ((rc = wo_part())) return rc;
            if ((rc = hand(st, sx))) return rc;
            if (!emit && (rc = split_dg_block(lb, 2, t0, t1, true))) return rc;
            if ((rc = dh1_gemm(lb, t0, t1))) return rc;
            if ((rc = record(sx, &dh1_done[(size_t)k]))) return rc;
        }
        while (wo_r < R)
            if ((rc = wo_part())) return rc;
        if ((rc = record(sx, &wo_done))) return rc;
        if ((rc = word_weight_grads(lb))) return rc;
        if ((rc = record(sx, &done->word_grads_ev))) return rc;
        if ((rc = demb_gemm(lb))) return rc;
        if ((rc = record(sx, &done->demb_ev))) return rc;
    }
    const int kc = nb / 2;
    const int hh1_t0 = nb >= 4 ? bd[kc] : 0;
    for (int k = nb - 1; k >= 0; --k) {
        const int t0 = bd[k], t1 = bd[k + 1];
        if ((rc = wait(st, dh1_done[(size_t)k]))) return rc;
        ProfScope ps(st, K_STEP_BWD, t1 - t0);
        if ((rc = lstm_seq_bwd_x3_persist2(st, bwd_x3_args(1, t0, t1), nullptr))) return rc;
        ++g_bwd_persist_launches;
        if (!emit && (rc = split_dg_block(la, 1, t0, t1, true))) return rc;
        if (hh1_t0 > 0 && k == kc) {
            if ((rc = hand(st, sx))) return rc;
            CuPlanCap cap(corun_cus);
            if ((rc = pgemm_tt(lb, 4 * H, H, (T - hh1_t0) * B, q.dg1, hh1_t0 * B, q.h1, (hh1_t0 - 1) * B, g->vid_w_hh, H, ID, nullptr, false))) return rc;
        }
    }
    done->bias_chunk = emit ? 32 : 64;
    done->hh1_t0 = hh1_t0;
    if ((rc = wait(st, wo_done))) return rc;
    if ((rc = grads_ready(0, st))) return rc;
    return hand(st, sx);
}

int TrainDriver::bptt_x3_two_layer(int corun_cus, int corun_k, BpttDone* done) {
    int rc;
    const int nb = (int)bd.size() - 1;
    for (int k = nb - 1; k >= -1; --k) {
        const bool hw = k >= 0, hv = k + 1 <= nb - 1;
        const bool solo = corun_k && nb >= 2 && (k == nb - 1 || k == -1);
        if (solo && (rc = hand(st, sx))) return rc;
        {
            ProfScope ps(st, K_STEP_BWD, (hw ? bd[k + 1] - bd[k] : 0) + (hv ? bd[k + 2] - bd[k + 1] : 0));
            SeqBwdX3Args aw, av;
            if (hw) aw = bwd_x3_args(2, bd[k], bd[k + 1]);
            if (hv) av = bwd_x3_args(1, bd[k + 1], bd[k + 2]);
            if (hw && hv) rc = lstm_seq_bwd_x3_persist2(st, aw, &av);
            else rc = lstm_seq_bwd_x3_persist2(st, hw ? aw : av, nullptr);
            ++g_bwd_persist_launches;
            if (rc) return rc;
        }
        if (solo) {
            const int r0 = (k == nb - 1) ? 0 : corun_k;
            {
                CuPlanCap cap(corun_cus);
                if ((rc = pgemm_tt(lb, V, H, corun_k, q.dlog, r0, q.h2decB, r0, g->out_w, H, ID, nullptr, r0 > 0))) return rc;
            }
            if ((rc = hand(sx, st))) return rc;
        }
        if (hw) {
            if (!emit && (rc = split_dg_block(la, 2, bd[k], bd[k + 1], true))) return rc;
            if ((rc = dh1_gemm(la, bd[k], bd[k + 1]))) return rc;
        }
        if (hv && !emit && (rc = split_dg_block(la, 1, bd[k + 1], bd[k + 2], true))) return rc;
    }
    done->bias_chunk = emit ? 32 : 64;
    if (!corun_k && (rc = grads_ready(0, st))) return rc;
    if ((rc = hand(st, sx))) return rc;
    if (corun_k) {
        const bool two = nb >= 2;
        const int r0 = two ? 2 * corun_k : 0;
        if ((rc = pgemm_tt(lb, V, H, R - r0, q.dlog, r0, q.h2decB, r0, g->out_w, H, ID, nullptr, two))) return rc;
        if ((rc = grads_ready(0, sx))) return rc;
    }
    return 0;
}

int TrainDriver::bptt_bf16_persistent() {
    int rc;
    if ((rc = hand(sx, st))) return rc;
    const int nb = (int)bd.size() - 1;
    for (int k = nb - 1; k >= -1; --k) {
        const bool hw = k >= 0, hv = k + 1 <= nb - 1;
        SeqBwdBf16Args aw, av;
        if (hw) aw = seq_bwd_bf16_args(T, bd[k], bd[k + 1], B, H, q.whh2T, q.dg2, w.dh2dec, L, w.c2, w.s2, w.dc2, w.psync_a, w.err + 1);
        if (hv) av = seq_bwd_bf16_args(T, bd[k + 1], bd[k + 2], B, H, q.whh1T, q.dg1, w.dh1, 0, w.c1, w.s1, w.dc1, w.psync_b, w.err + 1);
        {
            ProfScope ps(st, K_STEP_BWD, (hw ? bd[k + 1] - bd[k] : 0) + (hv ? bd[k + 2] - bd[k + 1] : 0));
            if (hw && hv) rc = lstm_seq_bwd_bf16_persist2(st, aw, &av);
            else rc = lstm_seq_bwd_bf16_persist2(st, hw ? aw : av, nullptr);
            ++g_bwd_persist_launches;
            if (rc) return rc;
        }
        if (hw) {
            if ((rc = split_dg_block(la, 2, bd[k], bd[k + 1], false))) return rc;
            if ((rc = dh1_gemm(la, bd[k], bd[k + 1]))) return rc;
        }
        if (hv && (rc = split_dg_block(la, 1, bd[k + 1], bd[k + 2], false))) return rc;
    }
    if ((rc = grads_ready(0, st))) return rc;
    return hand(st, sx);
}

int TrainDriver::bptt_two_lanes() {
    int rc;
    for (size_t k = bd.size() - 1; k >= 1; --k) {
        const int t0 = bd[k - 1], t1 = bd[k];
        rc = bf ? seq_bwd_bf16(st, T, t0, t1, B, H, q.whh2T, w.dh2dec, L, w.c2, w.s2, q.dg2, w.dc2)
                : seq_bwd(st, T, t0, t1, B, H, w.wt2, w.dh2dec, L, w.c2, w.s2, w.dc2);
        if (rc) return rc;
        if ((rc = split_dg_block(la, 2, t0, t1, !bf))) return rc;
        if ((rc = dh1_gemm(la, t0, t1))) return rc;
        if ((rc = hand(st, sx))) return rc;
        rc = bf ? seq_bwd_bf16(sx, T, t0, t1, B, H, q.whh1T, w.dh1, 0, w.c1, w.s1, q.dg1, w.dc1)
                : seq_bwd(sx, T, t0, t1, B, H, w.wt1, w.dh1, 0, w.c1, w.s1, w.dc1);
        if (rc) return rc;
        if ((rc = split_dg_block(lb, 1, t0, t1, !bf))) return rc;
    }
    return 0;
}

static int train_backward_x3(const s2vt_dims* d, const s2vt_params* p, const float* feats, const float* dlogits,
                             const s2vt_grads* g, float* dfeats, const TrainWS& w, const PlaneWS& q, hipStream_t st,
                             const float* out_mask, bool dlog_ready) {
    TrainDriver x(d, p, g, w, q, out_mask, nullptr);
    const int B = x.B, L = x.L, F = x.F, H = x.H, E = x.E, V = x.V, T = x.T, R = x.R;
    const int64_t BH = x.BH;
    int rc;
    if ((rc = x.open_lanes(st))) return rc;
    const hipStream_t sx = x.sx;
    const Lane &la = x.la, &lb = x.lb;
    const bool bf = x.bf;
    if (bf) {
        if ((rc = zero_pad_cols_u16(st, q.dg2.p, (int64_t)T * B, q.dg2.ld, 4 * H, q.dg2.kpad))) return rc;
        if ((rc = zero_pad_cols_u16(st, q.dg1.p, (int64_t)T * B, q.dg1.ld, 4 * H, q.dg1.kpad))) return rc;
    }
    if ((rc = x.hand(st, sx))) return rc;
    if (!dlog_ready && (rc = pdual(la, dlogits, V, ID, R, V, &q.dlog, 0, nullptr, 0, w.colsum_c))) return rc;
    if ((rc = x.hand(st, sx))) return rc;
    if ((rc = pgemm(la, R, H, V, q.dlog, 0, 0, q.woT, 0, 0, w.dh2dec, H, perm(L - 1, B), nullptr, false))) return rc;
    const bool ce_pow2 = dlog_ready && bf;
    if (ce_pow2 && (rc = scale_by_device_scalar(st, w.dh2dec, (int64_t)R * H, w.ce_alpha))) return rc;
    if (out_mask && (rc = mul_vectors(st, w.dh2dec, out_mask, w.dh2dec, (int64_t)R * H))) return rc;
    if (!bf && (rc = transpose_f32(st, p->word_w_hh, 4 * H, H, w.wt2))) return rc;
    RecKind kind = train_recurrence_plan(B, H).bwd;
    if (kind == REC_BF16_PERSIST && q.dg2.kpad != q.whh2T.kpad) kind = REC_PER_STEP;
    if (kind == REC_X3_PERSIST && !(w.xnslots > (x.blk < T ? x.blk : T))) kind = REC_PER_STEP;
    const bool px3_bwd = kind == REC_X3_PERSIST;
    const int x3_ns = px3_bwd ? lstm_seq_bwd_x3_persist_supported(B, H) : 0;
    const int one_layer_wgs = x3_ns > 0 ? (B / (32 * x3_ns)) * cdiv(H, 16) : 1 << 20;
    const int corun_cus = (planned_compute_units() - one_layer_wgs - 2) / 8 * 8;
    const int corun_k = (px3_bwd && option(O_CORUN) && sx != st && corun_cus >= 64 && R >= 2560) ? (R / 64 * option(O_CORUN) / 10) * 64 : 0;
    {
        const float* h2dec = w.h2 + L * BH;
        if (out_mask) {
            if ((rc = mul_vectors(sx, w.h2 + L * BH, out_mask, w.dx1, (int64_t)R * H))) return rc;
            h2dec = w.dx1;
        }
        if ((rc = psplit(lb, q.h2decB, 0, h2dec, H, perm(L - 1, B), R, H))) return rc;
        if (!corun_k && (rc = pgemm_tt(lb, V, H, R, q.dlog, 0, q.h2decB, 0, g->out_w, H, ID, nullptr, false))) return rc;
        if (!corun_k && ce_pow2 && (rc = scale_by_device_scalar(sx, g->out_w, (int64_t)V * H, w.ce_alpha))) return rc;
    }
    if ((rc = lcolsum_finish(lb, w.colsum_c, cdiv(R, 64), V, g->out_b, false))) return rc;
    if (kind == REC_PER_STEP && (rc = grads_ready(0, sx))) return rc;
    if (!bf && (rc = transpose_f32(sx, p->vid_w_hh, 4 * H, H, w.wt1))) return rc;
    x.set_bounds(kind != REC_PER_STEP);
    BpttDone done;
    switch (kind) {
    case REC_X3_PERSIST:
        if ((rc = x.x3_bptt_begin())) return rc;
        if (corun_k > 0 && x.bd.size() >= 3 && option(O_BPTT_SOLO) != 0) rc = x.bptt_x3_one_layer(corun_cus, corun_k, &done);
        else rc = x.bptt_x3_two_layer(corun_cus, corun_k, &done);
        break;
    case REC_BF16_PERSIST: rc = x.bptt_bf16_persistent(); break;
    default: rc = x.bptt_two_lanes(); break;
    }
    if (rc) return rc;
    if (done.word_grads_ev < 0 && (rc = x.word_weight_grads(la))) return rc;
    if ((rc = lcolsum_finish(la, w.colsum_a, T * B / done.bias_chunk, 4 * H, g->word_b_ih, false))) return rc;
    S2VT_HIP(hipMemcpyAsync(g->word_b_hh, g->word_b_ih, sizeof(float) * 4 * H, hipMemcpyDeviceToDevice, st));
    if ((rc = done.demb_ev >= 0 ? x.wait(st, done.demb_ev) : x.demb_gemm(la))) return rc;
    if ((rc = embedding_grad(st, w.de, R, E, w.tok, V, g->emb_w, w.embws))) return rc;
    if (done.word_grads_ev >= 0 && (rc = x.wait(st, done.word_grads_ev))) return rc;
    if ((rc = grads_ready(1, st))) return rc;
    const int hh1_rows = ((done.hh1_t0 > 0 ? done.hh1_t0 : T) - 1) * B;
    if ((rc = pgemm_tt(lb, 4 * H, H, hh1_rows, q.dg1, B, q.h1, 0, g->vid_w_hh, H, ID, nullptr, done.hh1_t0 > 0))) return rc;
    if ((rc = pgemm_tt(lb, 4 * H, H, L * B, q.dg1, 0, q.x1, 0, g->vid_w_ih, H, ID, nullptr, false))) return rc;
    if ((rc = lcolsum_finish(lb, w.colsum_b, T * B / done.bias_chunk, 4 * H, g->vid_b_ih, false))) return rc;
    S2VT_HIP(hipMemcpyAsync(g->vid_b_hh, g->vid_b_ih, sizeof(float) * 4 * H, hipMemcpyDeviceToDevice, sx));
    if ((rc = pgemm(lb, L * B, H, 4 * H, q.dg1, 0, 0, q.wih1T, 0, 0, w.dx1, H, perm(B, L), nullptr, false))) return rc;
    if ((rc = pdual(lb, w.dx1, H, ID, L * B, H, &q.x1, 0, nullptr, 0, w.colsum_b))) return rc;
    if ((rc = pgemm_tt(lb, H, F, L * B, q.x1, 0, q.feats, 0, g->feat_w, F, ID, nullptr, false))) return rc;
    if ((rc = lcolsum_finish(lb, w.colsum_b, L * B / 64, H, g->feat_b, false))) return rc;
    if (dfeats && (rc = lgemm(lb, true, false, L * B, F, H, w.dx1, H, ID, p->feat_w, F, ID, dfeats, F, ID, nullptr, false))) return rc;
    return x.hand(sx, st);
}

}

using namespace s2vt;

extern "C" {

struct PadWS { float* feats; int64_t* targets; float* logits; float* mask; float* dfeats; size_t bytes; };
static PadWS carve_pad(const s2vt_dims& d, const s2vt_dims& dp, void* base) {
    const size_t Bp = dp.B, L = d.L, F = d.F, H = d.H, V = d.V;
    Carver c{reinterpret_cast<char*>(base), 0, 0};
    PadWS w;
    w.feats = c.take<float>(Bp * L * F);
    w.targets = c.take<int64_t>(Bp * (L - 1));
    w.logits = c.take<float>(Bp * (L - 1) * V);
    w.mask = c.take<float>((L - 1) * Bp * H);
    w.dfeats = c.take<float>(Bp * L * F);
    w.bytes = align_up(c.off, 256);
    return w;
}
static size_t train_core_bytes(const s2vt_dims& d) {
    size_t n = carve_train(d, nullptr).bytes;
    if (planes_ok(d)) n += carve_planes(d, train_planes(), nullptr).bytes;
    return n;
}

int32_t s2vt_padded_batch(int32_t B) {
    if (B <= 0) return 0;
    s2vt_dims d = {B, 2, 1, 1, 1, 1};
    return batch_padded(d) ? padded_dims(d).B : B;
}

size_t s2vt_train_workspace_bytes(const s2vt_dims* d) {
    if (!dims_ok(d)) return 0;
    if (batch_padded(*d)) {
        const s2vt_dims dp = padded_dims(*d);
        return align_up(train_core_bytes(dp), 256) + carve_pad(*d, dp, nullptr).bytes;
    }
    return train_core_bytes(*d);
}

static inline uint64_t kw(const void* p) { return (uint64_t)(uintptr_t)p; }
static std::vector<uint64_t> graph_key(uint64_t tag, const s2vt_dims* d, const s2vt_params* p, const s2vt_grads* g, std::initializer_list<uint64_t> words) {
    std::vector<uint64_t> key;
    if (!graph_on()) return key;
    key.reserve(80);
    key.push_back(tag);
    for (int v : {d->B, d->L, d->F, d->H, d->E, d->V}) key.push_back((uint64_t)v);
    key_options(key);
    const float* const* pp = reinterpret_cast<const float* const*>(p);
    for (size_t i = 0; i < sizeof(s2vt_params) / sizeof(void*); ++i) key_ptr(key, pp[i]);
    float* const* gp = reinterpret_cast<float* const*>(g);
    for (size_t i = 0; g && i < sizeof(s2vt_grads) / sizeof(void*); ++i) key_ptr(key, gp[i]);
    key.insert(key.end(), words);
    return key;
}

static int train_forward_core(const s2vt_dims* d, const s2vt_params* p, const float* feats, const int64_t* targets,
                              int64_t targets_ld, float* logits, void* workspace, size_t workspace_bytes, void* stream,
                              const float* out_mask) {
    const TrainWS w = carve_train(*d, workspace);
    S2VT_REQUIRE(workspace_bytes >= w.bytes, "s2vt_train_forward: workspace %zu < %zu bytes", workspace_bytes, w.bytes);
    hipStream_t st = (hipStream_t)stream;
    int rc0 = poll_async_error(false);
    if (rc0) return rc0;
    record_forward(workspace, *d, planes_ok(*d));
    if (planes_ok(*d)) {
        const PlaneWS q = carve_planes(*d, train_planes(), reinterpret_cast<char*>(workspace) + w.bytes);
        S2VT_REQUIRE(workspace_bytes >= w.bytes + q.bytes, "s2vt_train_forward: workspace %zu < %zu bytes", workspace_bytes, w.bytes + q.bytes);
        const std::vector<uint64_t> key = graph_key(0xF0, d, p, nullptr, {kw(feats), kw(targets), (uint64_t)targets_ld, kw(logits), kw(workspace),
                                                                           kw(out_mask), kw(st)});
        rc0 = run_graphed(st, key, [&](hipStream_t s_) { return train_forward_x3(d, p, feats, targets, targets_ld, logits, w, q, s_, out_mask); });
    } else {
        rc0 = train_forward_f32(d, p, feats, targets, targets_ld, logits, w, st, out_mask);
    }
    return rc0 ? rc0 : post_async_error(st, w.err);
}
static int train_forward_impl(const s2vt_dims* d, const s2vt_params* p, const float* feats, const int64_t* targets,
                              int64_t targets_ld, float* logits, void* workspace, size_t workspace_bytes, void* stream,
                              const float* out_mask) {
    S2VT_REQUIRE(dims_ok(d) && p && feats && targets && logits && workspace, "s2vt_train_forward: null/invalid argument");
    if (!batch_padded(*d)) return train_forward_core(d, p, feats, targets, targets_ld, logits, workspace, workspace_bytes, stream, out_mask);
    const s2vt_dims dp = padded_dims(*d);
    const size_t core = align_up(train_core_bytes(dp), 256);
    const PadWS s = carve_pad(*d, dp, reinterpret_cast<char*>(workspace) + core);
    S2VT_REQUIRE(workspace_bytes >= core + s.bytes, "s2vt_train_forward: workspace %zu < %zu bytes", workspace_bytes, core + s.bytes);
    hipStream_t st = (hipStream_t)stream;
    const size_t B = d->B, Bp = dp.B, L = d->L, F = d->F, H = d->H, V = d->V;
    int rc;
    S2VT_HIP(hipMemcpyAsync(s.feats, feats, B * L * F * sizeof(float), hipMemcpyDeviceToDevice, st));
    if ((rc = fill_zero(st, s.feats + B * L * F, (Bp - B) * L * F * sizeof(float)))) return rc;
    if ((rc = fill_zero(st, s.targets, Bp * (L - 1) * sizeof(int64_t)))) return rc;
    S2VT_HIP(hipMemcpy2DAsync(s.targets, (L - 1) * sizeof(int64_t), targets, (size_t)targets_ld * sizeof(int64_t), (L - 1) * sizeof(int64_t), B,
                              hipMemcpyDeviceToDevice, st));
    if (out_mask) {
        if ((rc = fill_zero(st, s.mask, (L - 1) * Bp * H * sizeof(float)))) return rc;
        S2VT_HIP(hipMemcpy2DAsync(s.mask, Bp * H * sizeof(float), out_mask, B * H * sizeof(float), B * H * sizeof(float), L - 1,
                                  hipMemcpyDeviceToDevice, st));
    }
    if ((rc = train_forward_core(&dp, p, s.feats, s.targets, (int64_t)(L - 1), s.logits, workspace, core, stream, out_mask ? s.mask : nullptr))) return rc;
    S2VT_HIP(hipMemcpyAsync(logits, s.logits, B * (L - 1) * V * sizeof(float), hipMemcpyDeviceToDevice, st));
    return 0;
}

int s2vt_train_forward(const s2vt_dims* d, const s2vt_params* p, const float* feats, const int64_t* targets,
                       int64_t targets_ld, float* logits, void* workspace, size_t workspace_bytes, void* stream) {
    return train_forward_impl(d, p, feats, targets, targets_ld, logits, workspace, workspace_bytes, stream, nullptr);
}
int s2vt_train_forward_dropout(const s2vt_dims* d, const s2vt_params* p, const float* feats, const int64_t* targets,
                               int64_t targets_ld, const float* out_mask, float* logits, void* workspace,
                               size_t workspace_bytes, void* stream) {
    return train_forward_impl(d, p, feats, targets, targets_ld, logits, workspace, workspace_bytes, stream, out_mask);
}

static int train_backward_core(const s2vt_dims* d, const s2vt_params* p, const float* feats, const float* dlogits,
                               const s2vt_grads* g, float* dfeats, void* workspace, size_t workspace_bytes, void* stream,
                               const float* out_mask) {
    BackwardScope scope;
    const TrainWS w = carve_train(*d, workspace);
    S2VT_REQUIRE(workspace_bytes >= w.bytes, "s2vt_train_backward: workspace %zu < %zu bytes", workspace_bytes, w.bytes);
    hipStream_t st = (hipStream_t)stream;
    bool dlog_ready = false;
    int rc0 = poll_async_error(false);
    if (rc0 || (rc0 = check_forward_record(workspace, *d, planes_ok(*d), &dlog_ready))) return rc0;
    S2VT_REQUIRE(dlogits || dlog_ready, "s2vt_train_backward: dlogits is null and s2vt_mean_ce_backward_fused has not run on this workspace");
    if (planes_ok(*d)) {
        const PlaneWS q = carve_planes(*d, train_planes(), reinterpret_cast<char*>(workspace) + w.bytes);
        S2VT_REQUIRE(workspace_bytes >= w.bytes + q.bytes, "s2vt_train_backward: workspace %zu < %zu bytes", workspace_bytes, w.bytes + q.bytes);
        const std::vector<uint64_t> key = graph_key(0xB0 + (dlog_ready ? 1 : 0), d, p, g, {kw(feats), kw(dlogits), kw(dfeats), kw(workspace),
                                                                                            kw(out_mask), kw(st)});
        bool graphed = false;
        rc0 = run_graphed(st, key, [&](hipStream_t s_) {
                LaneDelayScope delay(s_);
                return train_backward_x3(d, p, feats, dlogits, g, dfeats, w, q, s_, out_mask, dlog_ready);
            }, &graphed);
        if (!rc0 && graphed) {
            if ((rc0 = grads_ready(0, st))) return rc0;
            if ((rc0 = grads_ready(1, st))) return rc0;
        }
        return rc0 ? rc0 : post_async_error(st, w.err, 1);
    }
    return train_backward_f32(d, p, feats, dlogits, g, dfeats, w, st, out_mask);
}
static int train_backward_impl(const s2vt_dims* d, const s2vt_params* p, const float* feats, const float* dlogits,
                               const s2vt_grads* g, float* dfeats, void* workspace, size_t workspace_bytes, void* stream,
                               const float* out_mask) {
    S2VT_REQUIRE(dims_ok(d) && p && feats && g && workspace, "s2vt_train_backward: null/invalid argument");
    if (!batch_padded(*d)) return train_backward_core(d, p, feats, dlogits, g, dfeats, workspace, workspace_bytes, stream, out_mask);
    S2VT_REQUIRE(dlogits, "s2vt_train_backward: dlogits is null (the fused criterion backward needs a batch that is a multiple of 64)");
    const s2vt_dims dp = padded_dims(*d);
    const size_t core = align_up(train_core_bytes(dp), 256);
    const PadWS s = carve_pad(*d, dp, reinterpret_cast<char*>(workspace) + core);
    S2VT_REQUIRE(workspace_bytes >= core + s.bytes, "s2vt_train_backward: workspace %zu < %zu bytes", workspace_bytes, core + s.bytes);
    hipStream_t st = (hipStream_t)stream;
    const size_t B = d->B, Bp = dp.B, L = d->L, F = d->F, V = d->V;
// ... 58 lines not shown
```

s2vt-video-caption_amd/csrc/kernels.h:

```cpp
#pragma once
#include "common.h"
#include "philox.h"

namespace s2vt {

int gemm_f32(hipStream_t stream, bool a_kmajor, bool b_kmajor, int M, int N, int K,
             const float* A, int64_t lda, RowMap amap, const float* B, int64_t ldb, RowMap bmap,
             float* C, int64_t ldc, RowMap cmap, const float* bias, bool accumulate,
             float* splitk_ws = nullptr, size_t splitk_ws_floats = 0);

int gemm_bf16_nt(hipStream_t stream, int nplanes, int M, int N, int K, const unsigned short* A, int64_t lda,
                 const unsigned short* B, int64_t ldb, float* C, int64_t ldc, RowMap cmap, const float* bias,
                 bool accumulate, float* splitk_ws, size_t splitk_ws_floats);
int gemm_x3(hipStream_t stream, int M, int N, int K, const unsigned short* A, int64_t lda, const unsigned short* B,
            int64_t ldb, float* C, int64_t ldc, RowMap cmap, const float* bias, bool accumulate, float* splitk_ws,
            size_t splitk_ws_floats);
int gemm_x3_tt(hipStream_t stream, int M, int N, int K, const unsigned short* A, int64_t lda, const unsigned short* B,
               int64_t ldb, float* C, int64_t ldc, RowMap cmap, const float* bias, bool accumulate, float* splitk_ws,
               size_t splitk_ws_floats);
int gemm_b1(hipStream_t stream, int M, int N, int K, const unsigned short* A, int64_t lda, const unsigned short* B,
            int64_t ldb, float* C, int64_t ldc, RowMap cmap, const float* bias, bool accumulate, float* splitk_ws,
            size_t splitk_ws_floats);
int gemm_b1_tt(hipStream_t stream, int M, int N, int K, const unsigned short* A, int64_t lda, const unsigned short* B,
               int64_t ldb, float* C, int64_t ldc, RowMap cmap, const float* bias, bool accumulate, float* splitk_ws,
// ... 115 lines not shown
struct ChainBwdLaunch { int B, H, n, tiles; ChainBwdStep s[CHAIN_MAX]; };
int lstm_chain_fwd_launch(hipStream_t stream, const ChainFwdLaunch& a);
int lstm_chain_bwd_launch(hipStream_t stream, const ChainBwdLaunch& a);

struct StepFwdBf16Args {
    int B, H, Kp;
    const unsigned short* hb_prev; int64_t ldhb;
    const unsigned short* wb; int64_t ldwb;
    const float* gx; int64_t ldgx;
    const float* bias;
    const float* c_prev; int64_t ldc;
    float* h_out; int64_t ldho;
    unsigned short* hb_out; int64_t ldhbo;
    float* c_out; int64_t ldco;
    float* stash; int64_t ldst;
};
int lstm_step_fwd_bf16(hipStream_t stream, const StepFwdBf16Args& a);

struct StepBwdBf16Args {
    int B, H, Kp;
    const unsigned short* dgb_next; int64_t lddgb;
    const unsigned short* wtb; int64_t ldwtb;
    const float* dh_out; int64_t lddho;
    const float* stash; int64_t ldst;
    const float* c; int64_t ldc;
    const float* c_prev; int64_t ldcp;
    float* dc; int64_t lddc;
    int dc_is_zero;
    float* dg; int64_t lddg;
    unsigned short* dgb; int64_t lddgbo;
};
int lstm_step_bwd_bf16(hipStream_t stream, const StepBwdBf16Args& a);

struct SeqFwdBf16Args {
    int B, H, Kp;
    int t0, t1, n_gx;
    const unsigned short* wb; int64_t ldwb;
    unsigned short* hb; int64_t ldhb;
    float* gx_stash;
    const float* bias;
    float* h_all;
    float* c_all;
    unsigned int* sync;
    int* err;
    int RB, NS;
    unsigned long long* stamps; int stamp_block;
};
int lstm_seq_fwd_bf16_persist_supported(int B, int H, int Kp);
size_t lstm_persist_sync_bytes();
int lstm_seq_fwd_bf16_persist(hipStream_t stream, SeqFwdBf16Args a);
int lstm_seq_fwd_bf16_persist2(hipStream_t stream, SeqFwdBf16Args a, const SeqFwdBf16Args* b);

struct SeqBwdBf16Args {
    int B, H, Kp;
    int T, t0, t1;
    const unsigned short* wtb; int64_t ldwtb;
    unsigned short* dgb; int64_t lddgb;
    const float* dh_out; int dh_first;
    float* stash_dg;
    const float* c_all;
    float* dc;
    unsigned int* sync; int* err;
    int RB, NS;
    unsigned long long* stamps; int stamp_block;
};
int lstm_seq_bwd_bf16_persist_supported(int B, int H, int Kp4);
int lstm_seq_bwd_bf16_persist2(hipStream_t stream, SeqBwdBf16Args a, const SeqBwdBf16Args* b);

struct SeqFwdX3Args {
    int B, H, Kp;
    int t0, t1, n_gx;
    const unsigned short* wp; int64_t wplane, ldw;
    unsigned short* hp; int64_t hplane, ldh;
    float* h_all;
    float* gx_stash; const float* bias; float* c_all;
    int no_stash;
    unsigned int* sync; int* err;
    unsigned short* hblk; int64_t ldhblk;
    int RB, NS;
    unsigned long long* stamps; int stamp_block;
};
int lstm_seq_fwd_x3_persist_supported(int B, int H);
int lstm_seq_fwd_x3_persist_single_workgroups(int B, int H);
int lstm_seq_fwd_x3_persist2(hipStream_t stream, SeqFwdX3Args a, const SeqFwdX3Args* b);
int split3_rows(hipStream_t stream, const float* src, int64_t ld, int R, int C, int Cp, unsigned short* dst, int64_t plane);
struct SeqBwdX3Args {
    int B, H, Kp, Hp;
    int T, t0, t1;
    const unsigned short* wtp; int64_t wplane, ldw;
    const float* dh_out; int dh_first;
    float* stash_dg;
    const float* c_all;
    float* dc;
    float* part; int64_t part_slot; int nslots;
    unsigned int* sync; int* err;
    unsigned short* dgp; int64_t lddgp;
    float* colpart;
    int skip_dg;
    int RB, NS;
    unsigned long long* stamps; int stamp_block;
};
int lstm_seq_bwd_x3_persist_supported(int B, int H);
size_t lstm_seq_bwd_x3_part_slot_floats(int B, int H);
int lstm_seq_bwd_x3_persist2(hipStream_t stream, SeqBwdX3Args a, const SeqBwdX3Args* b);
int split3_wt(hipStream_t stream, const float* wt, int H, int Kp, int Hp, unsigned short* dst, int64_t plane);

struct LogitsArgmaxArgs {
    int B, H, V;
    const float* h; int64_t ldh;
    const float* w_out; int64_t ldw;
    const float* b_out;
    unsigned long long* packed;
    unsigned long long* stamps;
};
int logits_argmax(hipStream_t stream, const LogitsArgmaxArgs& a, const GumbelArgs* sample = nullptr);

struct ArgmaxX3Args {
    int B, V, K;
    const unsigned short* W; int64_t ldw;
    const unsigned short* Hp; int64_t ldh;
    const float* bias;
    unsigned long long* packed;
    const unsigned short* W2; int64_t ldw2; int M2;
    float* z; int64_t ldz;
    int v_off;
    int dbg;
    unsigned long long* stamps;
};
int logits_argmax_x3(hipStream_t stream, const ArgmaxX3Args& a, const GumbelArgs* sample = nullptr);

int add_vectors(hipStream_t s, const float* a, const float* b, float* out, int n);
int adam_flat(hipStream_t s, float* p, const float* g, float* m, float* v, int64_t n, double lr, double beta1, double beta2, double eps,
              int64_t step);
constexpr int GN_CHUNK = 16384;
constexpr int ADAM_MAX_SEGS = 16;
struct ClipRecord {
    float grad_norm, scale;
    int32_t nonfinite, pad;
    int64_t skipped_total;
};
size_t grad_norm_workspace_bytes(int64_t n);
int grad_norm(hipStream_t s, const float* g, int64_t n, double max_norm, int skip_nonfinite, void* workspace, size_t workspace_bytes,
              ClipRecord* rec);
int adam_flat_clipped(hipStream_t s, float* p, const float* g, float* m, float* v, int64_t n, double lr, double beta1, double beta2,
                      double eps, int64_t step, double weight_decay, int decoupled, const int64_t* seg_end, const int32_t* seg_decay,
                      int n_seg, int skip_nonfinite, const ClipRecord* rec);
int mul_vectors(hipStream_t s, const float* a, const float* b, float* out, int64_t n);
int transpose_f32(hipStream_t s, const float* in, int rows, int cols, float* out);
int colsum_f32(hipStream_t s, const float* x, int64_t rows, int cols, int64_t ld, float* partial, float* out,
               bool accumulate);
size_t colsum_partial_floats(int64_t rows, int cols);
int targets_to_time_major(hipStream_t s, const int64_t* targets, int B, int Lm1, int64_t ld, int V, int32_t* out,
                          int* err_flag);
int top20_logprob(hipStream_t s, const float* logits, int64_t ld, int64_t rows, int V, int32_t* top_ix, float* top_lp);
int top20_gumbel(hipStream_t s, const float* logits, int64_t ld, int64_t rows, int V, const GumbelArgs& ga, int32_t* top_ix,
                 float* top_lp, float* top_g);
int gather_rows_f32(hipStream_t s, const float* src, int64_t ld, const int32_t* idx, int64_t rows, int cols, float* out);
size_t embedding_grad_ws_ints(int64_t rows, int V);
int embedding_grad(hipStream_t s, const float* d_rows, int64_t rows, int E, const int32_t* tok, int V, float* d_emb, int* ws);
int unpack_tokens(hipStream_t s, const unsigned long long* packed, int steps, int B, int64_t* out_ids);
int rows_clip(hipStream_t s, int R, int K, int Rp, int32_t* row_b);
int unpack_rows(hipStream_t s, const unsigned long long* packed, int steps, int ldp, int R, int64_t* out_ids);
int unpack_scheduled(hipStream_t s, const unsigned long long* packed, int steps, int ldp, int B, const SsArgs& ss, int64_t* used,
                     int64_t* draws);
int ss_mix(hipStream_t s, const int64_t* draw_tokens, int B, const SsArgs& ss, int64_t* out);
int fill_zero(hipStream_t s, void* p, size_t bytes);
int occupy_cus(hipStream_t s, int workgroups, int lds_bytes, long long microseconds);
int zero_pad_cols_u16(hipStream_t s, unsigned short* p, int64_t rows, int64_t ld, int col0, int col1);

int group_sum_rows(hipStream_t s, const float* in, int64_t ld_in, float* out, int64_t ld_out, int64_t groups, int K, int cols);
int group_expand_rows(hipStream_t s, const float* in, int64_t ld_in, float* out, int64_t ld_out, int64_t groups, int K, int cols,
                      bool accumulate);
int group_tokens(hipStream_t s, const int64_t* caps, int64_t stride_b, int64_t stride_k, int B, int K, int S, int V, int32_t* tok,
                 int* err_flag);

int mean_ce_fwd(hipStream_t s, const float* logits, int64_t rows, int V, const int64_t* target, int Lm1, int64_t ldt,
                float* lse, float* rowloss, float* loss_out, int* err_flag);
int mean_ce_bwd(hipStream_t s, const float* logits, int64_t rows, int V, const int64_t* target, int Lm1, int64_t ldt,
                const float* lse, const float* gout, float* dlogits);
int mask_criterion_fwd(hipStream_t s, const float* logits, int64_t rows, int V, const int64_t* target, int Lm1, int64_t ldt,
                       const float* mask, int64_t ldm, float* lse, float* rowloss, float* out3, int* err_flag);
int mask_criterion_bwd(hipStream_t s, const float* mask, int64_t ldm, int64_t rows, int Lm1, const float* fwd_out, const float* gout,
                       float* g_ce);
int weighted_ce_fwd(hipStream_t s, const float* logits, int64_t rows, int V, const int64_t* target, int Lm1, int64_t ldt,
                    const float* weight, int64_t ldw, float* lse, float* rowloss, float* out2, int* err_flag);
int weighted_ce_bwd(hipStream_t s, const float* logits, int64_t rows, int V, const int64_t* target, int Lm1, int64_t ldt,
                    const float* weight, int64_t ldw, const float* lse, const float* fwd_out, const float* gout, float* dlogits);

// ... 32 lines not shown
```

s2vt-video-caption_amd/csrc/lstm_persist_frame.h:

```cpp
#pragma once
#include <mutex>

#include "common.h"
#include "kernels.h"

namespace s2vt {

constexpr int PF_SR = 32;
constexpr int PF_MAXNS = 4;
constexpr unsigned long long PF_SPIN_TICKS = 100000000ull;

typedef short bf16x8 __attribute__((ext_vector_type(8)));
typedef float f32x2 __attribute__((ext_vector_type(2)));
typedef unsigned int u32x4 __attribute__((ext_vector_type(4)));
typedef __attribute__((address_space(1))) unsigned int gu32;

__device__ __forceinline__ unsigned short f2bf_rn(float x) {
    unsigned int u = __float_as_uint(x);
    if ((u & 0x7fffffffu) > 0x7f800000u) return (unsigned short)((u >> 16) | 0x40);
    u += 0x7fffu + ((u >> 16) & 1u);
    return (unsigned short)(u >> 16);
}

#ifdef S2VT_EXPERIMENT_PLAIN_LOADS
// ... 68 lines not shown
};

struct ActFast {
    static __device__ __forceinline__ float sigmoid(float x) { return __builtin_amdgcn_rcpf(1.0f + __expf(-x)); }
    static __device__ __forceinline__ float tanh(float x) { return 2.0f * __builtin_amdgcn_rcpf(1.0f + __expf(-2.0f * x)) - 1.0f; }
};
struct ActExact {
    static __device__ __forceinline__ float sigmoid(float x) { return sigmoidf_(x); }
    static __device__ __forceinline__ float tanh(float x) { return tanhf_(x); }
};

template <class Act>
__device__ __forceinline__ void cell_forward(float pi, float pf, float pg, float po, float cprev, bool ok, float (&gate)[4], float& c, float& h) {
    gate[0] = Act::sigmoid(pi);
    gate[1] = Act::sigmoid(pf);
    gate[2] = Act::tanh(pg);
    gate[3] = Act::sigmoid(po);
    c = ok ? gate[1] * cprev + gate[0] * gate[2] : 0.f;
    h = gate[3] * Act::tanh(c);
}
template <class Act>
__device__ __forceinline__ void cell_backward(float dh, float ig, float fg, float gg, float og, float c, float cprev, float dcin,
                                              float (&dg)[4], float& dcn) {
    const float tc = Act::tanh(c);
    const float dc = dh * og * (1.0f - tc * tc) + dcin;
    const float d_o = dh * tc;
    dg[0] = dc * gg * ig * (1.0f - ig);
    dg[1] = dc * cprev * fg * (1.0f - fg);
    dg[2] = dc * ig * (1.0f - gg * gg);
    dg[3] = d_o * og * (1.0f - og);
    dcn = dc * fg;
}

inline int coresident_capacity(const void* kernel, int block) {
    struct Entry { int dev; const void* k; int cap; };
    static Entry cache[32];
    static int n = 0;
    static std::mutex mu;
    std::lock_guard<std::mutex> lock(mu);
    int dev = 0;
    if (hipGetDevice(&dev) != hipSuccess) return 0;
    for (int i = 0; i < n; ++i)
        if (cache[i].dev == dev && cache[i].k == kernel) return cache[i].cap;
    int cus = 0, occ = 0;
    if (hipDeviceGetAttribute(&cus, hipDeviceAttributeMultiprocessorCount, dev) != hipSuccess) cus = 0;
    if (hipOccupancyMaxActiveBlocksPerMultiprocessor(&occ, kernel, block, 0) != hipSuccess) occ = 0;
    (void)hipGetLastError();
    const int cap = (cus > 0 && occ > 0) ? cus * occ : 0;
    if (n < 32) cache[n++] = Entry{dev, kernel, cap};
    return cap;
}
template <class Kernel>
static int persist_capacity_of(Kernel* kernel, int block, int design) {
    const int cap = coresident_capacity(reinterpret_cast<const void*>(kernel), block);
    return cap < design ? cap : design;
}

static inline int plan_chains(int B, int nC, int lim, bool rg_bound) {
    int R = B / PF_SR, ns = 1;
    while (R * nC > lim && ns < PF_MAXNS && R % 2 == 0) { R /= 2; ns *= 2; }
    return (R * nC <= lim && (!rg_bound || R <= 64)) ? ns : 0;
}

enum XcdPolicy { XCD_NONE, XCD_EXACT, XCD_PADDED };
struct XcdPlan { int xg, grid; };
static inline XcdPlan plan_xcd(XcdPolicy policy, int na, int nb, int nC, bool same_shape, int cap) {
    XcdPlan plan = {0, na + nb};
    if (policy == XCD_NONE || !same_shape || nC <= 0) return plan;
    const int G = (na + nb) / nC;
    if (!(G > 0 && G <= 8 && 8 % G == 0)) return plan;
    if (policy == XCD_EXACT) {
        if (na % nC == 0 && nb % nC == 0 && (!nb || nb == na) && (na + nb) % 8 == 0) plan.xg = G;
    } else {
        const int padded = 8 * cdiv(nC, 8 / G);
        if (padded <= cap) { plan.xg = G; plan.grid = padded; }
    }
    return plan;
}

struct PersistLayer { int un, cap; };

template <bool BPTT, class Args, class Prep, class Pair, class Launch>
static int launch_persistent_layers(hipStream_t stream, Args a, const Args* b, XcdPolicy policy, const char* who, const char* counters_msg,
                                    const char* kernel_name, Prep prep, Pair pair, Launch launch) {
    int rc;
    PersistLayer la, lb;
    if ((rc = prep(a, b == nullptr, &la))) return rc;
    Args bb = b ? *b : a;
    lb = la;
    if (b) {
        if ((rc = prep(bb, false, &lb))) return rc;
        const char* why = (bb.sync == a.sync) ? counters_msg : pair(a, bb, la, lb);
        S2VT_REQUIRE(!why, "%s", why);
    }
    const int nC = cdiv(a.H, la.un);
    const int na = (a.B / a.RB) * nC, nb = b ? (bb.B / bb.RB) * cdiv(bb.H, lb.un) : 0;
    S2VT_REQUIRE(na + nb <= la.cap, "%s: %d workgroups would not be co-resident (device capacity %d)", who, na + nb, la.cap);
    auto first = [](const Args& x) {
        if constexpr (BPTT) return x.t1 == x.T;
        else return x.t0 == 0;
    };
    if (first(a)) S2VT_HIP(hipMemsetAsync(a.sync, 0, lstm_persist_sync_bytes(), stream));
    if (b && first(bb)) S2VT_HIP(hipMemsetAsync(bb.sync, 0, lstm_persist_sync_bytes(), stream));
    const XcdPlan x = plan_xcd(policy, na, nb, nC, !b || (bb.B == a.B && bb.H == a.H), la.cap);
    launch(dim3(x.grid), a, bb, na, x.xg, la);
    S2VT_LAUNCH_CHECK(kernel_name);
    return 0;
}

}
```

s2vt-video-caption_amd/csrc/lstm_persist_x3.hip:

```cpp
#include <stdlib.h>
#include "common.h"
#include "experiment.h"
#include "kernels.h"
#include "lstm_persist_frame.h"

namespace s2vt {

constexpr int X_UN = 16;
constexpr int X_NT = 256;
constexpr int X_PLANE = PF_SR * 128;
constexpr int X_CHUNK = 3 * X_PLANE;
constexpr int X_RING = 3 * X_CHUNK;
constexpr int X_RLD = 72;
constexpr int X_HSM = 4 * X_RING;
constexpr int X_CST = X_HSM + 3 * PF_SR * X_UN * 2;
constexpr int X_LDS = X_CST + PF_MAXNS * PF_SR * X_UN * 4;
constexpr int X_MAX_WG = 256;
__device__ __forceinline__ void seq_fwd_x3_body(const SeqFwdX3Args& p, const int bid, unsigned char* smem, int& s_flag) {
    const unsigned lbase = (unsigned)(uintptr_t)(__attribute__((address_space(3))) unsigned char*)smem;
    const int tid = threadIdx.x, lane = tid & 63;
    const int kq = __builtin_amdgcn_readfirstlane(tid >> 6);
    const int li = lane & 31, lh = lane >> 5;
    const int H = p.H, B = p.B, Kp = p.Kp;
    const int nC = (H + X_UN - 1) / X_UN;
// ... 192 lines not shown
                        for (int c = u0 + X_UN; c < Kp; c += X_UN) {
                            zd += X_UN;
#pragma unroll
                            for (int pl = 0; pl < 3; ++pl)
                                asm volatile("global_store_dwordx4 %0, %1, off sc1\n\ts_nop 1" ::"v"(zd + pl * p.hplane), "v"(z) : "memory");
                        }
                    }
                }
            }
            if (kq == 1 && p.hblk) {
                const int rl = lane >> 1, part = lane & 1;
                const int64_t r = (int64_t)t * B + rbase + rl;
                if (rbase + rl < B) {
                    unsigned short* dst = p.hblk + (r >> 6) * (64 * p.ldhblk) + (int64_t)(u0 >> 4) * 3072 + part * 512 + (r & 63) * 8;
#pragma unroll
                    for (int pl = 0; pl < 3; ++pl)
                        *reinterpret_cast<u32x4*>(dst + pl * 1024) = *reinterpret_cast<const u32x4*>(hsm + pl * (PF_SR * X_UN) + rl * X_UN + part * 8);
                }
            }
            XSTAMP(p.stamps, xrec, 7);
            if (kq == 0) {
                asm volatile("s_waitcnt vmcnt(0)" ::: "memory");
                XSTAMP(p.stamps, xrec, 8);
                if (lane == 0) __hip_atomic_fetch_add((gu32*)cnt, 1u, __ATOMIC_RELAXED, __HIP_MEMORY_SCOPE_AGENT);
            }
            XSTAMP(p.stamps, xrec, 9);
            if (rok) {
                const int64_t rowi = (int64_t)t * B + eb;
                float* cdst = p.c_all + rowi * H + e.unit;
                float* hdst = p.h_all + rowi * H + e.unit;
                float* st = p.gx_stash + rowi * H4 + e.unit;
                const bool stash = p.no_stash == 0;
                e.store(cdst, cv);
                e.store(hdst, hv);
                if (stash) {
#pragma unroll
                    for (int g = 0; g < 4; ++g) e.store(st + (int64_t)g * H, gate[g]);
                }
            }
            PF_BARRIER();
        }
    }
}

__global__ __launch_bounds__(X_NT, 1) void lstm_seq_fwd_x3_persist_kernel(SeqFwdX3Args pa, SeqFwdX3Args pb, int na, int xg) {
    __shared__ __attribute__((aligned(1024))) unsigned char smem[X_LDS];
    __shared__ int s_flag;
    bool lb;
    const int vb = persist_role((int)blockIdx.x, na, (pa.H + X_UN - 1) / X_UN, xg, lb);
    if (vb < 0) return;
    seq_fwd_x3_body(lb ? pb : pa, vb, smem, s_flag);
}

static int fwd_x3_capacity() { return persist_capacity_of(&lstm_seq_fwd_x3_persist_kernel, X_NT, X_MAX_WG); }
int lstm_seq_fwd_x3_persist_supported(int B, int H) {
    if (!(B > 0 && B % PF_SR == 0 && H >= 8 && H <= 1024)) return 0;
    return plan_chains(B, cdiv(H, X_UN), fwd_x3_capacity() / 2, true);
}

static int fwd_x3_single_ns(int B, int H) {
    if (!lstm_seq_fwd_x3_persist_supported(B, H)) return 0;
    return plan_chains(B, cdiv(H, X_UN), fwd_x3_capacity(), false);
}
int lstm_seq_fwd_x3_persist_single_workgroups(int B, int H) {
    const int ns = fwd_x3_single_ns(B, H);
    return ns > 0 ? (B / (ns * PF_SR)) * cdiv(H, X_UN) : 0;
}
static int prep_x(SeqFwdX3Args& a, bool single = false) {
    const int ns = single ? fwd_x3_single_ns(a.B, a.H) : lstm_seq_fwd_x3_persist_supported(a.B, a.H);
    S2VT_REQUIRE(ns > 0, "lstm_seq_fwd_x3_persist: unsupported shape (B %% 32, H <= 1024) or it does not fit the device's resident capacity");
    S2VT_REQUIRE(a.t1 > a.t0 && a.t0 >= 0 && a.wp && a.hp && a.h_all && a.gx_stash && a.c_all && a.sync && a.err && (a.bias || a.n_gx >= a.t1),
                 "lstm_seq_fwd_x3_persist: bad arguments");
    S2VT_REQUIRE(!a.hblk || (a.B % 64 == 0 && a.ldhblk >= 3 * (int64_t)a.Kp && a.ldhblk % 8 == 0 && (reinterpret_cast<uintptr_t>(a.hblk) & 15) == 0),
                 "lstm_seq_fwd_x3_persist: the h row image needs B %% 64 == 0 and rows of 3 * pad64(H) elements");
    S2VT_REQUIRE(a.Kp == (a.H + 63) / 64 * 64 && a.ldw >= a.Kp && a.ldh >= a.Kp && a.ldw % 8 == 0 && a.ldh % 8 == 0 &&
                     a.wplane % 8 == 0 && a.hplane % 8 == 0 && (reinterpret_cast<uintptr_t>(a.wp) & 15) == 0 &&
                     (reinterpret_cast<uintptr_t>(a.hp) & 15) == 0,
                 "lstm_seq_fwd_x3_persist: plane images must be 16-byte aligned with rows of Kp = H rounded up to 64");
    a.NS = ns;
    a.RB = ns * PF_SR;
    return 0;
}

int lstm_seq_fwd_x3_persist2(hipStream_t stream, SeqFwdX3Args a, const SeqFwdX3Args* b) {
    return launch_persistent_layers<false>(
        stream, a, b, XCD_PADDED, "lstm_seq_fwd_x3_persist", "lstm_seq_fwd_x3_persist: paired layers need their own counters",
        "lstm_seq_fwd_x3_persist_kernel",
        [](SeqFwdX3Args& x, bool single, PersistLayer* l) {
            *l = PersistLayer{X_UN, fwd_x3_capacity()};
            return prep_x(x, single);
        },
        [](const SeqFwdX3Args&, const SeqFwdX3Args&, const PersistLayer&, const PersistLayer&) -> const char* { return nullptr; },
        [&](dim3 grid, const SeqFwdX3Args& pa, const SeqFwdX3Args& pb, int na, int xg, const PersistLayer&) {
            hipLaunchKernelGGL(lstm_seq_fwd_x3_persist_kernel, grid, dim3(X_NT), 0, stream, pa, pb, na, xg);
        });
}

__global__ __launch_bounds__(256) void split3_rows_kernel(const float* __restrict__ src, int64_t ld, int R, int C, int Cp,
                                                          unsigned short* __restrict__ dst, int64_t plane) {
    const int64_t n = (int64_t)R * (Cp / 2);
    for (int64_t i = (int64_t)blockIdx.x * blockDim.x + threadIdx.x; i < n; i += (int64_t)gridDim.x * blockDim.x) {
        const int r = (int)(i / (Cp / 2)), c = (int)(i % (Cp / 2)) * 2;
        unsigned short a[3] = {0, 0, 0}, b[3] = {0, 0, 0};
        if (c < C) split3_bits(src[(int64_t)r * ld + c], a);
        if (c + 1 < C) split3_bits(src[(int64_t)r * ld + c + 1], b);
#pragma unroll
        for (int pl = 0; pl < 3; ++pl)
            *reinterpret_cast<unsigned int*>(dst + pl * plane + (int64_t)r * Cp + c) = (unsigned int)a[pl] | ((unsigned int)b[pl] << 16);
    }
}
int split3_rows(hipStream_t stream, const float* src, int64_t ld, int R, int C, int Cp, unsigned short* dst, int64_t plane) {
    S2VT_REQUIRE(src && dst && R > 0 && C > 0 && Cp >= C && Cp % 2 == 0 && plane >= (int64_t)R * Cp, "split3_rows: bad arguments");
    const int64_t n = (int64_t)R * (Cp / 2);
    const int grid = (int)((n + 255) / 256 < 2048 ? (n + 255) / 256 : 2048);
    hipLaunchKernelGGL(split3_rows_kernel, dim3(grid), dim3(256), 0, stream, src, ld, R, C, Cp, dst, plane);
    S2VT_LAUNCH_CHECK("split3_rows_kernel");
    return 0;
}


constexpr int Y_GBUF = 64 * 2048;
constexpr int Y_TILE = Y_GBUF;
constexpr int Y_DCST = Y_TILE + 3 * X_PLANE;
constexpr int Y_CSUM = Y_DCST + PF_MAXNS * PF_SR * X_UN * 4;
constexpr int Y_LDS = Y_CSUM + 4 * 64 * 4;

__device__ __forceinline__ void seq_bwd_x3_body(const SeqBwdX3Args& p, const int bid, unsigned char* smem, int& s_flag) {
    const unsigned lbase = (unsigned)(uintptr_t)(__attribute__((address_space(3))) unsigned char*)smem;
    const int tid = threadIdx.x, lane = tid & 63;
    const int kw = __builtin_amdgcn_readfirstlane(tid >> 6);
    const int li = lane & 31, lh = lane >> 5;
    const int H = p.H, B = p.B;
    const int nC = (H + X_UN - 1) / X_UN;
    const int cs = bid % nC, rg = bid / nC;
    const int u0 = cs * X_UN, row0 = rg * p.RB;
    const unsigned short* zero = reinterpret_cast<const unsigned short*>(g_zero4);

    const int l16 = lane & 15, kg = lane >> 4;
    bf16x8 wreg[96];
    {
#pragma unroll
        for (int pl = 0; pl < 3; ++pl)
#pragma unroll
            for (int ks = 0; ks < 2; ++ks)
#pragma unroll
                for (int jt = 0; jt < 16; ++jt) {
                    const int j = 256 * kw + 16 * jt + l16;
                    const unsigned short* q = (j < p.Kp) ? p.wtp + pl * p.wplane + (int64_t)j * p.ldw + (2 * ks + (kg >> 1)) * p.Hp + u0 + (kg & 1) * 8 : zero;
                    wreg[(pl * 2 + ks) * 16 + jt] = *reinterpret_cast<const bf16x8*>(q);
                }
#pragma unroll
        for (int i = 0; i < 32; ++i) asm volatile("" : "+v"(wreg[i]));
#pragma unroll
        for (int i = 32; i < 96; ++i) asm volatile("" : "+a"(wreg[i]));
    }
    unsigned fa[2][2];
#pragma unroll
    for (int bt = 0; bt < 2; ++bt)
#pragma unroll
        for (int ks = 0; ks < 2; ++ks) {
            const int b = 16 * bt + l16;
            fa[bt][ks] = lbase + (unsigned)(Y_TILE + b * 128 + (((4 * ks + kg) ^ ((b >> 1) & 7)) * 16));
        }

    const CellLane<X_UN> e(tid, u0, H);
    float* dcst = reinterpret_cast<float*>(smem + Y_DCST);
    const bool last_block = (p.t1 == p.T);
    for (int s = 0; s < p.NS; ++s) {
        const int b = row0 + s * PF_SR + e.row;
        f32x2 d0 = {0.f, 0.f};
        if (!last_block && b < B) d0 = e.carry(p.dc + (int64_t)b * H + e.unit);
        *reinterpret_cast<f32x2*>(dcst + (s * PF_SR + e.row) * X_UN + e.ul) = d0;
    }
    const int64_t H4 = 4 * (int64_t)H;
    const float* gbuf = reinterpret_cast<const float*>(smem);
    unsigned char* tile = smem + Y_TILE;
    unsigned tw[4];
#pragma unroll
// ... 138 lines not shown
                        for (int ks = 0; ks < 2; ++ks) asm volatile("" : "+v"(gfr[pl][bt][ks]));
#define Y_MF(W, G, ACC) ACC = __builtin_amdgcn_mfma_f32_16x16x32_bf16(W, G, ACC, 0, 0, 0);
#pragma unroll
                for (int jp = 0; jp < 8; ++jp) {
                    f32x4 acc[2][2];
#pragma unroll
                    for (int x = 0; x < 2; ++x)
#pragma unroll
                        for (int bt = 0; bt < 2; ++bt) acc[x][bt] = f32x4{0.f, 0.f, 0.f, 0.f};
#define Y_PROD(WP, GP)                                                                                          \
                    _Pragma("unroll") for (int ks = 0; ks < 2; ++ks)                                            \
                        _Pragma("unroll") for (int x = 0; x < 2; ++x)                                           \
                            _Pragma("unroll") for (int bt = 0; bt < 2; ++bt)                                    \
                                Y_MF(wreg[((WP) * 2 + ks) * 16 + 2 * jp + x], gfr[GP][bt][ks], acc[x][bt])
                    Y_PROD(2, 0) Y_PROD(0, 2) Y_PROD(1, 1) Y_PROD(1, 0) Y_PROD(0, 1) Y_PROD(0, 0)
#undef Y_PROD
#pragma unroll
                    for (int x = 0; x < 2; ++x) {
                        const int cons = 16 * kw + 2 * jp + x;
                        if (cons < nC) {
#pragma unroll
                            for (int bt = 0; bt < 2; ++bt) {
                                float* dst = pslot + cons * cstride + bt * (16 * X_UN);
                                asm volatile("global_store_dwordx4 %0, %1, off sc1\n\ts_nop 1" ::"v"(dst), "a"(acc[x][bt]) : "memory");
                            }
                        }
                    }
                }
#undef Y_MF
                XSTAMP(p.stamps, xrec, 6);
                asm volatile("s_waitcnt vmcnt(0)" ::: "memory");
                XSTAMP(p.stamps, xrec, 7);
                PF_BARRIER();
                if (tid == 0) __hip_atomic_fetch_add((gu32*)cnt, 1u, __ATOMIC_RELAXED, __HIP_MEMORY_SCOPE_AGENT);
                XSTAMP(p.stamps, xrec, 8);
                emit_planes();
                if (p.dgp || p.colpart) PF_BARRIER();
            } else {
                emit_planes();
                PF_BARRIER();
            }
        }
    }
}

__global__ __launch_bounds__(X_NT, 1) void lstm_seq_bwd_x3_persist_kernel(SeqBwdX3Args pa, SeqBwdX3Args pb, int na, int xg) {
    __shared__ __attribute__((aligned(1024))) unsigned char smem[Y_LDS];
    __shared__ int s_flag;
    bool lb;
    const int vb = persist_role((int)blockIdx.x, na, (pa.H + X_UN - 1) / X_UN, xg, lb);
    if (vb < 0) return;
    seq_bwd_x3_body(lb ? pb : pa, vb, smem, s_flag);
}

static int bwd_x3_capacity() { return persist_capacity_of(&lstm_seq_bwd_x3_persist_kernel, X_NT, X_MAX_WG); }
int lstm_seq_bwd_x3_persist_supported(int B, int H) {
    if (!(B > 0 && B % PF_SR == 0 && H >= 8 && H <= 1024)) return 0;
    return plan_chains(B, cdiv(H, X_UN), bwd_x3_capacity() / 2, true);
}
size_t lstm_seq_bwd_x3_part_slot_floats(int B, int H) {
    const size_t nC = (size_t)cdiv(H, X_UN);
    return (size_t)(B / PF_SR) * nC * nC * PF_SR * X_UN;
}

static int prep_y(SeqBwdX3Args& a) {
    const int ns = lstm_seq_bwd_x3_persist_supported(a.B, a.H);
    S2VT_REQUIRE(ns > 0, "lstm_seq_bwd_x3_persist: unsupported shape (B %% 32, H <= 1024) or it does not fit the device's resident capacity");
    S2VT_REQUIRE(a.t1 > a.t0 && a.t0 >= 0 && a.t1 <= a.T && a.wtp && a.stash_dg && a.c_all && a.dc && a.part && a.sync && a.err &&
                     a.dh_first >= 0, "lstm_seq_bwd_x3_persist: bad arguments");
    S2VT_REQUIRE(a.Kp == (a.H + 63) / 64 * 64 && a.Hp == cdiv(a.H, X_UN) * X_UN && a.ldw >= 4 * (int64_t)a.Hp && a.ldw % 8 == 0 &&
                     a.wplane % 8 == 0 && (reinterpret_cast<uintptr_t>(a.wtp) & 15) == 0 && (reinterpret_cast<uintptr_t>(a.part) & 15) == 0,
                 "lstm_seq_bwd_x3_persist: W_hh^T planes must be [3][Kp][4 Hp], 16-byte aligned");
    S2VT_REQUIRE(a.nslots > a.t1 - a.t0 && (size_t)a.part_slot >= lstm_seq_bwd_x3_part_slot_floats(a.B, a.H) && a.part_slot % 4 == 0,
                 "lstm_seq_bwd_x3_persist: the partial-sum ring needs more slots than the launch has timesteps");
    S2VT_REQUIRE(!a.dgp || (a.H % 8 == 0 && a.B % 64 == 0 && a.lddgp >= 3 * (int64_t)((4 * a.H + 63) / 64 * 64) && a.lddgp % 8 == 0 &&
                            (reinterpret_cast<uintptr_t>(a.dgp) & 15) == 0),
                 "lstm_seq_bwd_x3_persist: the dG row image needs H %% 8 == 0, B %% 64 == 0 and rows of 3 * pad64(4H) elements");
    S2VT_REQUIRE(!a.skip_dg || a.dgp, "lstm_seq_bwd_x3_persist: skip_dg without a plane image");
    a.NS = ns;
    a.RB = ns * PF_SR;
    return 0;
}

int lstm_seq_bwd_x3_persist2(hipStream_t stream, SeqBwdX3Args a, const SeqBwdX3Args* b) {
    static const char pair_msg[] = "lstm_seq_bwd_x3_persist: paired layers need their own counters and partial sums";
    return launch_persistent_layers<true>(
        stream, a, b, XCD_PADDED, "lstm_seq_bwd_x3_persist", pair_msg, "lstm_seq_bwd_x3_persist_kernel",
        [](SeqBwdX3Args& x, bool, PersistLayer* l) {
            *l = PersistLayer{X_UN, bwd_x3_capacity()};
            return prep_y(x);
        },
        [](const SeqBwdX3Args& pa, const SeqBwdX3Args& pb, const PersistLayer&, const PersistLayer&) -> const char* {
            return pb.part != pa.part ? nullptr : pair_msg;
        },
        [&](dim3 grid, const SeqBwdX3Args& pa, const SeqBwdX3Args& pb, int na, int xg, const PersistLayer&) {
            hipLaunchKernelGGL(lstm_seq_bwd_x3_persist_kernel, grid, dim3(X_NT), 0, stream, pa, pb, na, xg);
        });
}

__global__ __launch_bounds__(256) void split3_wt_kernel(const float* __restrict__ wt, int H, int Kp, int Hp,
                                                        unsigned short* __restrict__ dst, int64_t plane) {
    const int64_t n = (int64_t)Kp * (2 * Hp);
    for (int64_t i = (int64_t)blockIdx.x * blockDim.x + threadIdx.x; i < n; i += (int64_t)gridDim.x * blockDim.x) {
        const int j = (int)(i / (2 * Hp)), kp = (int)(i % (2 * Hp)) * 2;
        const int g = kp / Hp, u = kp % Hp;
        unsigned short a[3] = {0, 0, 0}, b[3] = {0, 0, 0};
        if (j < H && u < H) split3_bits(wt[(int64_t)j * 4 * H + (int64_t)g * H + u], a);
        if (j < H && u + 1 < H) split3_bits(wt[(int64_t)j * 4 * H + (int64_t)g * H + u + 1], b);
#pragma unroll
        for (int pl = 0; pl < 3; ++pl)
            *reinterpret_cast<unsigned int*>(dst + pl * plane + (int64_t)j * 4 * Hp + kp) = (unsigned int)a[pl] | ((unsigned int)b[pl] << 16);
    }
}
int split3_wt(hipStream_t stream, const float* wt, int H, int Kp, int Hp, unsigned short* dst, int64_t plane) {
    S2VT_REQUIRE(wt && dst && H > 0 && Kp >= H && Hp >= H && Hp % 2 == 0 && plane >= (int64_t)Kp * 4 * Hp, "split3_wt: bad arguments");
    const int64_t n = (int64_t)Kp * (2 * Hp);
    const int grid = (int)((n + 255) / 256 < 2048 ? (n + 255) / 256 : 2048);
    hipLaunchKernelGGL(split3_wt_kernel, dim3(grid), dim3(256), 0, stream, wt, H, Kp, Hp, dst, plane);
    S2VT_LAUNCH_CHECK("split3_wt_kernel");
    return 0;
}

}
```

Baseline: 517,400 frames/s.

## Fuse W_hh split3 images, move forward prep onto side lane, prezero counters

```diff
diff --git a/include/s2vt_hip.h b/include/s2vt_hip.h
--- a/include/s2vt_hip.h
+++ b/include/s2vt_hip.h
@@ -233,6 +233,7 @@
                         size_t ws_ints, void* stream);
 int s2vt_gather_rows(const float* src, int64_t ld, const int32_t* idx, int64_t rows, int32_t cols, float* out, void* stream);
 int s2vt_group_sum_rows(const float* in, int64_t ld_in, float* out, int64_t ld_out, int64_t groups, int32_t K, int32_t cols, void* stream);
+int s2vt_split3_whh(const float* w_hh, int32_t H, uint16_t* rows_out, uint16_t* wt_out, void* stream);
 int s2vt_transpose_f32(const float* in, int32_t rows, int32_t cols, float* out, void* stream);
 int s2vt_colsum(const float* x, int64_t rows, int32_t cols, int64_t ld, float* ws, size_t ws_floats, float* out, int32_t accumulate,
                 void* stream);
diff --git a/s2vt-video-caption_amd/capi.py b/s2vt-video-caption_amd/capi.py
--- a/s2vt-video-caption_amd/capi.py
+++ b/s2vt-video-caption_amd/capi.py
@@ -165,6 +165,7 @@
     "s2vt_gather_rows": (c_int32, [c_void_p, c_int64, c_void_p, c_int64, c_int32, c_void_p, c_void_p]),
     "s2vt_group_sum_rows": (c_int32, [c_void_p, c_int64, c_void_p, c_int64, c_int64, c_int32, c_int32, c_void_p]),
     "s2vt_transpose_f32": (c_int32, [c_void_p, c_int32, c_int32, c_void_p, c_void_p]),
+    "s2vt_split3_whh": (c_int32, [c_void_p, c_int32, c_void_p, c_void_p, c_void_p]),
     "s2vt_colsum": (c_int32, [c_void_p, c_int64, c_int32, c_int64, c_void_p, c_size_t, c_void_p, c_int32, c_void_p]),
     "s2vt_colsum_finish": (c_int32, [c_void_p, c_int32, c_int32, c_void_p, c_int32, c_void_p]),
     "s2vt_split_planes_dual": (c_int32, [c_int32, c_void_p, c_int64, c_void_p, c_int32, c_int32, c_int32, c_int32,
diff --git a/s2vt-video-caption_amd/csrc/api_internal.h b/s2vt-video-caption_amd/csrc/api_internal.h
--- a/s2vt-video-caption_amd/csrc/api_internal.h
+++ b/s2vt-video-caption_amd/csrc/api_internal.h
@@ -169,6 +169,11 @@
              const float* bias, bool acc);
 int lcolsum_finish(const Lane& ln, const float* partial, int nchunks, int cols, float* out, bool accumulate);
 int bias_sums(hipStream_t st, const s2vt_params* p, int H, float* bsum1, float* bsum2);
+int lfill_zero(const Lane& ln, void* p, size_t bytes);
+int lzero_k16_tail(const Lane& ln, const PB& img, int H, size_t rows);
+int lsplit3_whh(const Lane& ln, const float* w_hh, int H, int64_t Kp, int64_t Hp, unsigned short* rows_dst, unsigned short* wt_dst);
+int lbias_sums(const Lane& ln, const s2vt_params* p, int H, float* bsum1, float* bsum2);
+int ltargets_to_time_major(const Lane& ln, const int64_t* targets, int B, int Lm1, int64_t ld, int V, int32_t* out, int* err);
 int project_features_f32(const Lane& ln, const s2vt_dims& d, const s2vt_params* p, const float* feats, float* x1, float* gx1, const float* bsum1);
 extern int g_lane_delay_lanes;
 extern long long g_lane_delay_us;
diff --git a/s2vt-video-caption_amd/csrc/api_ops.hip b/s2vt-video-caption_amd/csrc/api_ops.hip
--- a/s2vt-video-caption_amd/csrc/api_ops.hip
+++ b/s2vt-video-caption_amd/csrc/api_ops.hip
@@ -180,6 +180,12 @@
     return gather_rows_f32((hipStream_t)stream, src, ld, idx, rows, cols, out);
 }
 
+int s2vt_split3_whh(const float* w_hh, int32_t H, uint16_t* rows_out, uint16_t* wt_out, void* stream) {
+    S2VT_REQUIRE(w_hh && wt_out && H >= 8 && H <= 1024, "s2vt_split3_whh: null argument or H = %d outside 8..1024", H);
+    S2VT_REQUIRE((reinterpret_cast<uintptr_t>(rows_out) & 15) == 0 && (reinterpret_cast<uintptr_t>(wt_out) & 15) == 0,
+                 "s2vt_split3_whh: the images must be 16-byte aligned");
+    return split3_whh((hipStream_t)stream, w_hh, H, (H + 63) / 64 * 64, (H + 15) / 16 * 16, rows_out, wt_out);
+}
 int s2vt_transpose_f32(const float* in, int32_t rows, int32_t cols, float* out, void* stream) {
     S2VT_REQUIRE(in && out && in != out && rows > 0 && cols > 0 && (rows + 63) / 64 <= 65535,
                  "s2vt_transpose_f32: null argument or bad geometry (rows=%d cols=%d)", rows, cols);
diff --git a/s2vt-video-caption_amd/csrc/api_shared.hip b/s2vt-video-caption_amd/csrc/api_shared.hip
--- a/s2vt-video-caption_amd/csrc/api_shared.hip
+++ b/s2vt-video-caption_amd/csrc/api_shared.hip
@@ -153,6 +153,26 @@
 int lcolsum_finish(const Lane& ln, const float* partial, int nchunks, int cols, float* out, bool accumulate) {
     if (int rc = lane_delay(ln.s)) return rc;
     return colsum_finish(ln.s, partial, nchunks, cols, out, accumulate);
+}
+int lfill_zero(const Lane& ln, void* p, size_t bytes) {
+    if (int rc = lane_delay(ln.s)) return rc;
+    return fill_zero(ln.s, p, bytes);
+}
+int lzero_k16_tail(const Lane& ln, const PB& img, int H, size_t rows) {
+    if (int rc = lane_delay(ln.s)) return rc;
+    return zero_k16_tail(ln.s, img, H, rows);
+}
+int lsplit3_whh(const Lane& ln, const float* w_hh, int H, int64_t Kp, int64_t Hp, unsigned short* rows_dst, unsigned short* wt_dst) {
+    if (int rc = lane_delay(ln.s)) return rc;
+    return split3_whh(ln.s, w_hh, H, (int)Kp, (int)Hp, rows_dst, wt_dst);
+}
+int lbias_sums(const Lane& ln, const s2vt_params* p, int H, float* bsum1, float* bsum2) {
+    if (int rc = lane_delay(ln.s)) return rc;
+    return bias_sums(ln.s, p, H, bsum1, bsum2);
+}
+int ltargets_to_time_major(const Lane& ln, const int64_t* targets, int B, int Lm1, int64_t ld, int V, int32_t* out, int* err) {
+    if (int rc = lane_delay(ln.s)) return rc;
+    return targets_to_time_major(ln.s, targets, B, Lm1, ld, V, out, err);
 }
 
 int seq_fwd_bf16(hipStream_t st, int t0, int t1, int B, int H, float* gx_stash, int n_gx, const float* bias,
diff --git a/s2vt-video-caption_amd/csrc/api_train.hip b/s2vt-video-caption_amd/csrc/api_train.hip
--- a/s2vt-video-caption_amd/csrc/api_train.hip
+++ b/s2vt-video-caption_amd/csrc/api_train.hip
@@ -162,9 +162,10 @@
     int open_lanes(hipStream_t caller) { return open(caller, w.gws_a, w.gws_b, w.gws_floats, w.colsum_a, w.colsum_b); }
     void set_bounds(bool persistent) { bd = pipe_bounds(T, L, persistent ? balanced_block(L, blk) : blk); }
 
-    int zero_k16(const PB& img, size_t first, size_t elems) {
-        S2VT_HIP(hipMemset2DAsync(img.p + first, (size_t)64 * img.ld * 2, 0, elems * 2, (size_t)(T * B / 64), st));
-        return 0;
+    bool x3_bwd_planned() const { return train_recurrence_plan(B, H).bwd == REC_X3_PERSIST && w.xnslots > (blk < T ? blk : T); }
+    int zero_counters(const Lane& ln) {
+        const size_t span = (size_t)(reinterpret_cast<char*>(w.psync_b) - reinterpret_cast<char*>(w.psync_a)) + lstm_persist_sync_bytes();
+        return lfill_zero(ln, w.psync_a, span);
     }
     int vid_half_gemm(const Lane& ln, int t0, int t1) {
         const bool cap = t0 >= L;
@@ -214,7 +215,8 @@
         }
         return a;
     }
-    int x3_bptt_begin();
+    int x3_bptt_prep(long* ev);
+    int x3_bptt_begin(long prep_ev, bool one_layer);
     int bptt_x3_one_layer(int corun_cus, int corun_k, BpttDone* done);
     int bptt_x3_two_layer(int corun_cus, int corun_k, BpttDone* done);
     int bptt_bf16_persistent();
@@ -225,8 +227,6 @@
     int rc;
     if ((rc = hand(sx, st))) return rc;
     const int nb = (int)bd.size() - 1;
-    for (const PB* img : {&q.h1, &q.h2r})
-        if ((rc = zero_k16_tail(st, *img, H, (size_t)T * B))) return rc;
     int lg_c = (nb >= 2 && !out_mask) ? (L - 1) * ((2 * tenths + 1) / 3) / 10 : 0;
     if (lg_c > bd[nb - 1] - L) lg_c = bd[nb - 1] - L > 0 ? bd[nb - 1] - L : 0;
     for (int k = 0; k <= nb; ++k) {
@@ -240,8 +240,8 @@
         if (hw) aw = persist_fwd_x3_args(bd[k - 1], bd[k], B, H, T, w.xkp, w.s2, T, w.bsum2, w.xw2, w.xh2, w.h2, w.c2, w.psync_b, w.err + 1);
         av.hblk = q.h1.p; av.ldhblk = q.h1.ld;
         aw.hblk = q.h2r.p; aw.ldhblk = q.h2r.ld;
-        if (hv && hw) rc = lstm_seq_fwd_x3_persist2(st, av, &aw);
-        else rc = lstm_seq_fwd_x3_persist2(st, hv ? av : aw, nullptr);
+        if (hv && hw) rc = lstm_seq_fwd_x3_persist2(st, av, &aw, true);
+        else rc = lstm_seq_fwd_x3_persist2(st, hv ? av : aw, nullptr, true);
         }
         if (rc) return rc;
         if (co_first || co_last) {
@@ -310,39 +310,51 @@
     const hipStream_t sx = x.sx;
     const Lane &la = x.la, &lb = x.lb;
     const bool bf = x.bf;
-    if ((rc = bias_sums(st, p, H, w.bsum1, w.bsum2))) return rc;
-    if ((rc = fill_zero(st, w.err, 4 * sizeof(int)))) return rc;
-    if ((rc = targets_to_time_major(st, targets, B, L - 1, targets_ld, V, w.tok, w.err))) return rc;
     if (bf) {
         if ((rc = zero_pad_cols_u16(st, q.h1.p, (int64_t)T * B, q.h1.ld, H, q.h1.kpad))) return rc;
         if ((rc = zero_pad_cols_u16(st, q.h2r.p, (int64_t)T * B, q.h2r.ld, H, q.h2r.kpad))) return rc;
         if ((rc = pdual(la, p->vid_w_hh, H, ID, 4 * H, H, &q.whh1, 0, &q.whh1T, 0, nullptr))) return rc;
     }
     if ((rc = x.hand(st, sx))) return rc;
-    if (bf && (rc = pdual(lb, p->word_w_hh, H, ID, 4 * H, H, &q.whh2, 0, &q.whh2T, 0, nullptr))) return rc;
     RecKind kind = train_recurrence_plan(B, H).fwd;
     if (kind == REC_X3_PERSIST && !w.xfwd) kind = REC_PER_STEP;
     if (kind == REC_BF16_PERSIST && !persist_fwd_ok(B, H, q.whh1, q.h1)) kind = REC_PER_STEP;
     const bool px3_fwd = kind == REC_X3_PERSIST;
+    const bool px3_bwd = x.x3_bwd_planned();
+    long head_ev = -1;
+    if ((rc = lfill_zero(lb, w.err, 4 * sizeof(int)))) return rc;
+    if ((rc = ltargets_to_time_major(lb, targets, B, L - 1, targets_ld, V, w.tok, w.err))) return rc;
+    if ((rc = lbias_sums(lb, p, H, w.bsum1, w.bsum2))) return rc;
+    if ((rc = pdual(lb, p->vid_w_ih, H, ID, 4 * H, H, &q.wih1, 0, &q.wih1T, 0, nullptr))) return rc;
+    if ((rc = x.record(sx, &head_ev))) return rc;
+    if (bf && (rc = pdual(lb, p->word_w_hh, H, ID, 4 * H, H, &q.whh2, 0, &q.whh2T, 0, nullptr))) return rc;
     if (px3_fwd) {
-        if ((rc = split3_rows(sx, p->vid_w_hh, H, 4 * H, H, (int)w.xkp, w.xw1, 4 * (int64_t)H * w.xkp))) return rc;
-        if ((rc = split3_rows(sx, p->word_w_hh, H, 4 * H, H, (int)w.xkp, w.xw2, 4 * (int64_t)H * w.xkp))) return rc;
-    }
-    if ((rc = pdual(lb, p->word_w_ih, E + H, ID, 4 * H, E, &q.we, 0, &q.weT, 0, nullptr))) return rc;
-    if ((rc = pdual(lb, p->word_w_ih + E, E + H, ID, 4 * H, H, &q.wv, 0, &q.wvT, 0, nullptr))) return rc;
-    if ((rc = pdual(lb, p->out_w, H, ID, V, H, &q.wo, 0, &q.woT, 0, nullptr))) return rc;
-    if ((rc = pdual(lb, p->emb_w, E, gather(w.tok), R, E, &q.emb, 0, nullptr, 0, nullptr))) return rc;
+        if ((rc = x.zero_counters(lb))) return rc;
+        for (const PB* img : {&q.h1, &q.h2r})
+            if ((rc = lzero_k16_tail(lb, *img, H, (size_t)T * B))) return rc;
+    }
+    if (px3_bwd) {
+        if ((rc = lsplit3_whh(lb, p->vid_w_hh, H, w.xkp, w.xhp, px3_fwd ? w.xw1 : nullptr, w.xwt1))) return rc;
+        if ((rc = lsplit3_whh(lb, p->word_w_hh, H, w.xkp, w.xhp, px3_fwd ? w.xw2 : nullptr, w.xwt2))) return rc;
+    } else if (px3_fwd) {
+        if ((rc = lane_delay(sx)) || (rc = split3_rows(sx, p->vid_w_hh, H, 4 * H, H, (int)w.xkp, w.xw1, 4 * (int64_t)H * w.xkp))) return rc;
+        if ((rc = lane_delay(sx)) || (rc = split3_rows(sx, p->word_w_hh, H, 4 * H, H, (int)w.xkp, w.xw2, 4 * (int64_t)H * w.xkp))) return rc;
+    }
     const int f_wgs = px3_fwd ? lstm_seq_fwd_x3_persist_single_workgroups(B, H) : 0;
     const int f_cus = f_wgs > 0 ? (planned_compute_units() - f_wgs - 2) / 8 * 8 : 0;
     const bool stages3 = px3_fwd && pipe_bounds(T, L, balanced_block(L, x.blk)).size() >= 3;
     const int tenths = (stages3 && sx != st && f_cus >= 64 && R >= 2560 && B % 64 == 0) ? option(O_CORUN) : 0;
     const int gxe_c = (R / 64 * (2 * tenths < 8 ? 2 * tenths : 8) / 10) * 64;
+    if ((rc = pdual(lb, p->word_w_ih, E + H, ID, 4 * H, E, &q.we, 0, &q.weT, 0, nullptr))) return rc;
+    if ((rc = pdual(lb, p->word_w_ih + E, E + H, ID, 4 * H, H, &q.wv, 0, &q.wvT, 0, nullptr))) return rc;
+    if ((rc = pdual(lb, p->out_w, H, ID, V, H, &q.wo, 0, &q.woT, 0, nullptr))) return rc;
+    if ((rc = pdual(lb, p->emb_w, E, gather(w.tok), R, E, &q.emb, 0, nullptr, 0, nullptr))) return rc;
     if ((rc = pgemm(lb, R - gxe_c, 4 * H, E, q.emb, 0, 0, q.we, 0, 0, w.s2 + (int64_t)L * B4H, 4 * H, ID, w.bsum2, false))) return rc;
     if ((rc = psplit(la, q.feats, 0, feats, F, ID, B * L, F))) return rc;
     if ((rc = psplit(la, q.wf, 0, p->feat_w, F, ID, H, F))) return rc;
-    if ((rc = pdual(la, p->vid_w_ih, H, ID, 4 * H, H, &q.wih1, 0, &q.wih1T, 0, nullptr))) return rc;
     if ((rc = pgemm(la, B * L, H, F, q.feats, 0, 0, q.wf, 0, 0, w.x1, H, perm(L, B), p->feat_b, false))) return rc;
     if ((rc = pdual(la, w.x1, H, ID, L * B, H, &q.x1, 0, nullptr, 0, nullptr))) return rc;
+    if ((rc = x.wait(st, head_ev))) return rc;
     if ((rc = pgemm(la, L * B, 4 * H, H, q.x1, 0, 0, q.wih1, 0, 0, w.s1, 4 * H, ID, w.bsum1, false))) return rc;
     x.set_bounds(kind != REC_PER_STEP);
     switch (kind) {
@@ -352,22 +364,15 @@
     }
 }
 
-int TrainDriver::x3_bptt_begin() {
-    int rc;
-    if ((rc = split3_wt(st, w.wt2, H, (int)w.xkp, (int)w.xhp, w.xwt2, w.xkp * 4 * w.xhp))) return rc;
-    if ((rc = split3_wt(sx, w.wt1, H, (int)w.xkp, (int)w.xhp, w.xwt1, w.xkp * 4 * w.xhp))) return rc;
-    if ((rc = hand(sx, st))) return rc;
-    if (emit && q.dg2.kpad > 4 * H) {
-        const size_t kc0 = (size_t)(4 * H / 16);
-        for (const PB* img : {&q.dg2, &q.dg1}) {
-            if ((rc = zero_k16_tail(st, *img, 4 * H, (size_t)T * B))) return rc;
-            if (4 * H % 16)
-                for (int pl = 0; pl < 3; ++pl)
-                    if ((rc = zero_k16(*img, kc0 * K16_REC_ELEMS + (pl * 2 + 1) * K16_HALF_ELEMS, K16_HALF_ELEMS))) return rc;
-        }
-    }
-    return 0;
-}
+int TrainDriver::x3_bptt_prep(long* ev) {
+    int rc;
+    if ((rc = zero_counters(lb))) return rc;
+    if (emit)
+        for (const PB* img : {&q.dg2, &q.dg1})
+            if ((rc = lzero_k16_tail(lb, *img, 4 * H, (size_t)T * B))) return rc;
+    return record(sx, ev);
+}
+int TrainDriver::x3_bptt_begin(long prep_ev, bool one_layer) { return one_layer ? wait(st, prep_ev) : hand(sx, st); }
 
 int TrainDriver::bptt_x3_one_layer(int corun_cus, int corun_k, BpttDone* done) {
     int rc;
@@ -390,7 +395,7 @@
             const int t0 = bd[k], t1 = bd[k + 1];
             {
                 ProfScope ps(st, K_STEP_BWD, t1 - t0);
-                if ((rc = lstm_seq_bwd_x3_persist2(st, bwd_x3_args(2, t0, t1), nullptr))) return rc;
+                if ((rc = lstm_seq_bwd_x3_persist2(st, bwd_x3_args(2, t0, t1), nullptr, true))) return rc;
                 ++g_bwd_persist_launches;
             }
             if ((rc = wo_part())) return rc;
@@ -413,7 +418,7 @@
         const int t0 = bd[k], t1 = bd[k + 1];
         if ((rc = wait(st, dh1_done[(size_t)k]))) return rc;
         ProfScope ps(st, K_STEP_BWD, t1 - t0);
-        if ((rc = lstm_seq_bwd_x3_persist2(st, bwd_x3_args(1, t0, t1), nullptr))) return rc;
+        if ((rc = lstm_seq_bwd_x3_persist2(st, bwd_x3_args(1, t0, t1), nullptr, true))) return rc;
         ++g_bwd_persist_launches;
         if (!emit && (rc = split_dg_block(la, 1, t0, t1, true))) return rc;
         if (hh1_t0 > 0 && k == kc) {
@@ -441,8 +446,8 @@
             SeqBwdX3Args aw, av;
             if (hw) aw = bwd_x3_args(2, bd[k], bd[k + 1]);
             if (hv) av = bwd_x3_args(1, bd[k + 1], bd[k + 2]);
-            if (hw && hv) rc = lstm_seq_bwd_x3_persist2(st, aw, &av);
-            else rc = lstm_seq_bwd_x3_persist2(st, hw ? aw : av, nullptr);
+            if (hw && hv) rc = lstm_seq_bwd_x3_persist2(st, aw, &av, true);
+            else rc = lstm_seq_bwd_x3_persist2(st, hw ? aw : av, nullptr, true);
             ++g_bwd_persist_launches;
             if (rc) return rc;
         }
@@ -532,17 +537,20 @@
         if ((rc = zero_pad_cols_u16(st, q.dg1.p, (int64_t)T * B, q.dg1.ld, 4 * H, q.dg1.kpad))) return rc;
     }
     if ((rc = x.hand(st, sx))) return rc;
+    RecKind kind = train_recurrence_plan(B, H).bwd;
+    if (kind == REC_BF16_PERSIST && q.dg2.kpad != q.whh2T.kpad) kind = REC_PER_STEP;
+    if (kind == REC_X3_PERSIST && !x.x3_bwd_planned()) kind = REC_PER_STEP;
+    const bool px3_bwd = kind == REC_X3_PERSIST;
+    long prep_ev = -1;
+    if (px3_bwd && (rc = x.x3_bptt_prep(&prep_ev))) return rc;
     if (!dlog_ready && (rc = pdual(la, dlogits, V, ID, R, V, &q.dlog, 0, nullptr, 0, w.colsum_c))) return rc;
     if ((rc = x.hand(st, sx))) return rc;
     if ((rc = pgemm(la, R, H, V, q.dlog, 0, 0, q.woT, 0, 0, w.dh2dec, H, perm(L - 1, B), nullptr, false))) return rc;
     const bool ce_pow2 = dlog_ready && bf;
     if (ce_pow2 && (rc = scale_by_device_scalar(st, w.dh2dec, (int64_t)R * H, w.ce_alpha))) return rc;
     if (out_mask && (rc = mul_vectors(st, w.dh2dec, out_mask, w.dh2dec, (int64_t)R * H))) return rc;
-    if (!bf && (rc = transpose_f32(st, p->word_w_hh, 4 * H, H, w.wt2))) return rc;
-    RecKind kind = train_recurrence_plan(B, H).bwd;
-    if (kind == REC_BF16_PERSIST && q.dg2.kpad != q.whh2T.kpad) kind = REC_PER_STEP;
-    if (kind == REC_X3_PERSIST && !(w.xnslots > (x.blk < T ? x.blk : T))) kind = REC_PER_STEP;
-    const bool px3_bwd = kind == REC_X3_PERSIST;
+    const bool want_wt = !bf && !px3_bwd;
+    if (want_wt && (rc = transpose_f32(st, p->word_w_hh, 4 * H, H, w.wt2))) return rc;
     const int x3_ns = px3_bwd ? lstm_seq_bwd_x3_persist_supported(B, H) : 0;
     const int one_layer_wgs = x3_ns > 0 ? (B / (32 * x3_ns)) * cdiv(H, 16) : 1 << 20;
     const int corun_cus = (planned_compute_units() - one_layer_wgs - 2) / 8 * 8;
@@ -559,15 +567,16 @@
     }
     if ((rc = lcolsum_finish(lb, w.colsum_c, cdiv(R, 64), V, g->out_b, false))) return rc;
     if (kind == REC_PER_STEP && (rc = grads_ready(0, sx))) return rc;
-    if (!bf && (rc = transpose_f32(sx, p->vid_w_hh, 4 * H, H, w.wt1))) return rc;
+    if (want_wt && (rc = transpose_f32(sx, p->vid_w_hh, 4 * H, H, w.wt1))) return rc;
     x.set_bounds(kind != REC_PER_STEP);
     BpttDone done;
     switch (kind) {
-    case REC_X3_PERSIST:
-        if ((rc = x.x3_bptt_begin())) return rc;
-        if (corun_k > 0 && x.bd.size() >= 3 && option(O_BPTT_SOLO) != 0) rc = x.bptt_x3_one_layer(corun_cus, corun_k, &done);
-        else rc = x.bptt_x3_two_layer(corun_cus, corun_k, &done);
+    case REC_X3_PERSIST: {
+        const bool one_layer = corun_k > 0 && x.bd.size() >= 3 && option(O_BPTT_SOLO) != 0;
+        if ((rc = x.x3_bptt_begin(prep_ev, one_layer))) return rc;
+        rc = one_layer ? x.bptt_x3_one_layer(corun_cus, corun_k, &done) : x.bptt_x3_two_layer(corun_cus, corun_k, &done);
         break;
+    }
     case REC_BF16_PERSIST: rc = x.bptt_bf16_persistent(); break;
     default: rc = x.bptt_two_lanes(); break;
     }
@@ -586,8 +595,8 @@
     S2VT_HIP(hipMemcpyAsync(g->vid_b_hh, g->vid_b_ih, sizeof(float) * 4 * H, hipMemcpyDeviceToDevice, sx));
     if ((rc = pgemm(lb, L * B, H, 4 * H, q.dg1, 0, 0, q.wih1T, 0, 0, w.dx1, H, perm(B, L), nullptr, false))) return rc;
     if ((rc = pdual(lb, w.dx1, H, ID, L * B, H, &q.x1, 0, nullptr, 0, w.colsum_b))) return rc;
+    if ((rc = lcolsum_finish(lb, w.colsum_b, L * B / 64, H, g->feat_b, false))) return rc;
     if ((rc = pgemm_tt(lb, H, F, L * B, q.x1, 0, q.feats, 0, g->feat_w, F, ID, nullptr, false))) return rc;
-    if ((rc = lcolsum_finish(lb, w.colsum_b, L * B / 64, H, g->feat_b, false))) return rc;
     if (dfeats && (rc = lgemm(lb, true, false, L * B, F, H, w.dx1, H, ID, p->feat_w, F, ID, dfeats, F, ID, nullptr, false))) return rc;
     return x.hand(sx, st);
 }
@@ -662,7 +671,10 @@
         S2VT_REQUIRE(workspace_bytes >= w.bytes + q.bytes, "s2vt_train_forward: workspace %zu < %zu bytes", workspace_bytes, w.bytes + q.bytes);
         const std::vector<uint64_t> key = graph_key(0xF0, d, p, nullptr, {kw(feats), kw(targets), (uint64_t)targets_ld, kw(logits), kw(workspace),
                                                                            kw(out_mask), kw(st)});
-        rc0 = run_graphed(st, key, [&](hipStream_t s_) { return train_forward_x3(d, p, feats, targets, targets_ld, logits, w, q, s_, out_mask); });
+        rc0 = run_graphed(st, key, [&](hipStream_t s_) {
+                LaneDelayScope delay(s_);
+                return train_forward_x3(d, p, feats, targets, targets_ld, logits, w, q, s_, out_mask);
+            });
     } else {
         rc0 = train_forward_f32(d, p, feats, targets, targets_ld, logits, w, st, out_mask);
     }
diff --git a/s2vt-video-caption_amd/csrc/kernels.h b/s2vt-video-caption_amd/csrc/kernels.h
--- a/s2vt-video-caption_amd/csrc/kernels.h
+++ b/s2vt-video-caption_amd/csrc/kernels.h
@@ -221,7 +221,7 @@
 };
 int lstm_seq_fwd_x3_persist_supported(int B, int H);
 int lstm_seq_fwd_x3_persist_single_workgroups(int B, int H);
-int lstm_seq_fwd_x3_persist2(hipStream_t stream, SeqFwdX3Args a, const SeqFwdX3Args* b);
+int lstm_seq_fwd_x3_persist2(hipStream_t stream, SeqFwdX3Args a, const SeqFwdX3Args* b, bool counters_zeroed = false);
 int split3_rows(hipStream_t stream, const float* src, int64_t ld, int R, int C, int Cp, unsigned short* dst, int64_t plane);
 struct SeqBwdX3Args {
     int B, H, Kp, Hp;
@@ -241,8 +241,9 @@
 };
 int lstm_seq_bwd_x3_persist_supported(int B, int H);
 size_t lstm_seq_bwd_x3_part_slot_floats(int B, int H);
-int lstm_seq_bwd_x3_persist2(hipStream_t stream, SeqBwdX3Args a, const SeqBwdX3Args* b);
+int lstm_seq_bwd_x3_persist2(hipStream_t stream, SeqBwdX3Args a, const SeqBwdX3Args* b, bool counters_zeroed = false);
 int split3_wt(hipStream_t stream, const float* wt, int H, int Kp, int Hp, unsigned short* dst, int64_t plane);
+int split3_whh(hipStream_t stream, const float* w_hh, int H, int Kp, int Hp, unsigned short* rows_dst, unsigned short* wt_dst);
 
 struct LogitsArgmaxArgs {
     int B, H, V;
diff --git a/s2vt-video-caption_amd/csrc/lstm_persist_frame.h b/s2vt-video-caption_amd/csrc/lstm_persist_frame.h
--- a/s2vt-video-caption_amd/csrc/lstm_persist_frame.h
+++ b/s2vt-video-caption_amd/csrc/lstm_persist_frame.h
@@ -174,7 +174,7 @@
 
 template <bool BPTT, class Args, class Prep, class Pair, class Launch>
 static int launch_persistent_layers(hipStream_t stream, Args a, const Args* b, XcdPolicy policy, const char* who, const char* counters_msg,
-                                    const char* kernel_name, Prep prep, Pair pair, Launch launch) {
+                                    const char* kernel_name, Prep prep, Pair pair, Launch launch, bool counters_zeroed = false) {
     int rc;
     PersistLayer la, lb;
     if ((rc = prep(a, b == nullptr, &la))) return rc;
@@ -192,8 +192,8 @@
         if constexpr (BPTT) return x.t1 == x.T;
         else return x.t0 == 0;
     };
-    if (first(a)) S2VT_HIP(hipMemsetAsync(a.sync, 0, lstm_persist_sync_bytes(), stream));
-    if (b && first(bb)) S2VT_HIP(hipMemsetAsync(bb.sync, 0, lstm_persist_sync_bytes(), stream));
+    if (!counters_zeroed && first(a)) S2VT_HIP(hipMemsetAsync(a.sync, 0, lstm_persist_sync_bytes(), stream));
+    if (!counters_zeroed && b && first(bb)) S2VT_HIP(hipMemsetAsync(bb.sync, 0, lstm_persist_sync_bytes(), stream));
     const XcdPlan x = plan_xcd(policy, na, nb, nC, !b || (bb.B == a.B && bb.H == a.H), la.cap);
     launch(dim3(x.grid), a, bb, na, x.xg, la);
     S2VT_LAUNCH_CHECK(kernel_name);
diff --git a/s2vt-video-caption_amd/csrc/lstm_persist_x3.hip b/s2vt-video-caption_amd/csrc/lstm_persist_x3.hip
--- a/s2vt-video-caption_amd/csrc/lstm_persist_x3.hip
+++ b/s2vt-video-caption_amd/csrc/lstm_persist_x3.hip
@@ -298,7 +298,7 @@
     return 0;
 }
 
-int lstm_seq_fwd_x3_persist2(hipStream_t stream, SeqFwdX3Args a, const SeqFwdX3Args* b) {
+int lstm_seq_fwd_x3_persist2(hipStream_t stream, SeqFwdX3Args a, const SeqFwdX3Args* b, bool counters_zeroed) {
     return launch_persistent_layers<false>(
         stream, a, b, XCD_PADDED, "lstm_seq_fwd_x3_persist", "lstm_seq_fwd_x3_persist: paired layers need their own counters",
         "lstm_seq_fwd_x3_persist_kernel",
@@ -309,7 +309,7 @@
         [](const SeqFwdX3Args&, const SeqFwdX3Args&, const PersistLayer&, const PersistLayer&) -> const char* { return nullptr; },
         [&](dim3 grid, const SeqFwdX3Args& pa, const SeqFwdX3Args& pb, int na, int xg, const PersistLayer&) {
             hipLaunchKernelGGL(lstm_seq_fwd_x3_persist_kernel, grid, dim3(X_NT), 0, stream, pa, pb, na, xg);
-        });
+        }, counters_zeroed);
 }
 
 __global__ __launch_bounds__(256) void split3_rows_kernel(const float* __restrict__ src, int64_t ld, int R, int C, int Cp,
@@ -614,7 +614,7 @@
     return 0;
 }
 
-int lstm_seq_bwd_x3_persist2(hipStream_t stream, SeqBwdX3Args a, const SeqBwdX3Args* b) {
+int lstm_seq_bwd_x3_persist2(hipStream_t stream, SeqBwdX3Args a, const SeqBwdX3Args* b, bool counters_zeroed) {
     static const char pair_msg[] = "lstm_seq_bwd_x3_persist: paired layers need their own counters and partial sums";
     return launch_persistent_layers<true>(
         stream, a, b, XCD_PADDED, "lstm_seq_bwd_x3_persist", pair_msg, "lstm_seq_bwd_x3_persist_kernel",
@@ -627,7 +627,7 @@
         },
         [&](dim3 grid, const SeqBwdX3Args& pa, const SeqBwdX3Args& pb, int na, int xg, const PersistLayer&) {
             hipLaunchKernelGGL(lstm_seq_bwd_x3_persist_kernel, grid, dim3(X_NT), 0, stream, pa, pb, na, xg);
-        });
+        }, counters_zeroed);
 }
 
 __global__ __launch_bounds__(256) void split3_wt_kernel(const float* __restrict__ wt, int H, int Kp, int Hp,
@@ -653,4 +653,48 @@
     return 0;
 }
 
-}
+static constexpr int W3_TU = 32, W3_TC = 64;
+__global__ __launch_bounds__(256) void split3_whh_kernel(const float* __restrict__ w, int H, int Kp, int Hp,
+                                                         unsigned short* __restrict__ rows, unsigned short* __restrict__ wt) {
+    __shared__ unsigned short tile[3][W3_TC][W3_TU + 2];
+    const int g = blockIdx.z, u0 = blockIdx.y * W3_TU, c0 = blockIdx.x * W3_TC;
+    const int64_t rplane = 4 * (int64_t)H * Kp, tplane = (int64_t)Kp * 4 * Hp;
+    {
+        const int cl = (threadIdx.x % 32) * 2, c = c0 + cl;
+        for (int ul = threadIdx.x / 32; ul < W3_TU; ul += 8) {
+            const int u = u0 + ul;
+            unsigned short a[3] = {0, 0, 0}, b[3] = {0, 0, 0};
+            if (u < H) {
+                const float* src = w + ((int64_t)g * H + u) * H;
+                if (c < H) split3_bits(src[c], a);
+                if (c + 1 < H) split3_bits(src[c + 1], b);
+            }
+#pragma unroll
+            for (int pl = 0; pl < 3; ++pl) {
+                if (rows && u < H)
+                    *reinterpret_cast<unsigned int*>(rows + pl * rplane + ((int64_t)g * H + u) * Kp + c) = (unsigned int)a[pl] | ((unsigned int)b[pl] << 16);
+                tile[pl][cl][ul] = a[pl];
+                tile[pl][cl + 1][ul] = b[pl];
+            }
+        }
+    }
+    __syncthreads();
+    {
+        const int ul = (threadIdx.x % 16) * 2, u = u0 + ul;
+        if (u < Hp)
+            for (int cl = threadIdx.x / 16; cl < W3_TC; cl += 16) {
+                const int64_t o = (int64_t)(c0 + cl) * 4 * Hp + (int64_t)g * Hp + u;
+#pragma unroll
+                for (int pl = 0; pl < 3; ++pl)
+                    *reinterpret_cast<unsigned int*>(wt + pl * tplane + o) = (unsigned int)tile[pl][cl][ul] | ((unsigned int)tile[pl][cl][ul + 1] << 16);
+            }
+    }
+}
+int split3_whh(hipStream_t stream, const float* w_hh, int H, int Kp, int Hp, unsigned short* rows_dst, unsigned short* wt_dst) {
+    S2VT_REQUIRE(w_hh && wt_dst && H > 0 && Kp >= H && Kp % W3_TC == 0 && Hp >= H && Hp % 2 == 0, "split3_whh: bad arguments");
+    hipLaunchKernelGGL(split3_whh_kernel, dim3(Kp / W3_TC, cdiv(Hp, W3_TU), 4), dim3(256), 0, stream, w_hh, H, Kp, Hp, rows_dst, wt_dst);
+    S2VT_LAUNCH_CHECK("split3_whh_kernel");
+    return 0;
+}
+
+}
```

Result: no change. 520,600 frames/s, median of 6 (+0.6%).
